# AliaksandrSiarohin/wc-gan

Hardware: AMD Instinct MI355X
Metric: images/sec G+D step, CIFAR-10 ResNet-SN+WC, batch 64 (higher is better)
Workload: dtype f32; 1 GPU; CIFAR-10 ResNet SN uncond + WC (scripts/cifar10_resnet_sn_uncond.sh), batch 64/GPU, training_ratio 5, generator_batch_multiple 2; parallelism=dp1, wc_statistics=per-replica, launch=hipgraph

## Files before the change

include/wc_hip.h:

```cpp
#ifndef WC_HIP_H
#define WC_HIP_H

#include <stddef.h>
#include <stdint.h>

#ifdef __cplusplus
extern "C" {
#endif

#define WC_ABI_VERSION 8

#define WC_OK                 0
#define WC_ERR_NULL          -1
#define WC_ERR_SHAPE         -2
#define WC_ERR_CHANNELS      -3
#define WC_ERR_WORKSPACE     -4
#define WC_ERR_ARG           -5

typedef void* wc_stream_t;

int         wc_abi_version(void);
const char* wc_error_string(int code);

#define WC_CORE_API "wc_stats_f32 wc_factor_f64 wc_color_f32 wc_group_bias_f32 wc_apply_f32 wc_apply_act_f32 " \
// ... 245 lines not shown
                             float* colsum_partials, int C, wc_stream_t stream);

#define WC_CONV_HIST_FLOATS (4 * 512 + 16)
#define WC_CONV_HIST_REDO (4 * 512)
int wc_conv_split_hist_f32(const float* x, int64_t n, int relu, void* hi, void* lo, float* scale, float* colsum_partials , int C,
                           float* hist, int bootstrap, wc_stream_t stream);

int wc_conv_split_leaky_f32(const float* x, int64_t n, float negative_slope, void* hi, void* lo, float* scale, void* amax_scratch,
                            float* colsum_partials , int C, wc_stream_t stream);
int wc_conv_split_hist_leaky_f32(const float* x, int64_t n, float negative_slope, void* hi, void* lo, float* scale,
                                 float* colsum_partials , int C, float* hist, int bootstrap, wc_stream_t stream);
int wc_conv_leaky_bwd_f32(float* dx, const float* x, int64_t n, float negative_slope, wc_stream_t stream);

size_t wc_conv_weights_bytes(const wc_conv_geom* g);
int wc_conv_weights_f32(const float* w, int64_t stride_k, int64_t stride_n, int64_t stride_r, int64_t stride_s,
                        int64_t n_elems, const wc_conv_geom* g, void* image, float* scale, void* amax_scratch,
                        const float* known_amax, int known_count, wc_stream_t stream);

int wc_conv_weights_pair_f32(const float* w, int64_t stride_r, int64_t stride_s, int64_t n_elems,
                             int64_t a_stride_k, int64_t a_stride_n, const wc_conv_geom* ga, void* image_a,
                             int64_t b_stride_k, int64_t b_stride_n, const wc_conv_geom* gb, void* image_b,
                             float* scale, void* amax_scratch, const float* known_amax, int known_count,
                             wc_stream_t stream);

typedef struct {
    const float* w; int64_t stride_k, stride_n, stride_r, stride_s, n_elems;
    const wc_conv_geom* g; void* image; float* scale;
    const float* amax; int amax_count; int pair_of;
} wc_conv_weights_job;
int wc_conv_weights_batch_f32(const wc_conv_weights_job* jobs, int count, wc_stream_t stream);
int wc_conv_weights_batch_launches(const wc_conv_weights_job* jobs, int count);

#define WC_CONV_ABSMAX_FLOATS 512
typedef struct { const float* x; int64_t n; float* partial; } wc_conv_absmax_job;
int wc_conv_absmax_batch_f32(const wc_conv_absmax_job* jobs, int count, wc_stream_t stream);

size_t wc_conv_workspace_bytes(const wc_conv_geom* g);
int wc_conv_f16x3(const void* xhi, const void* xlo, const float* xscale, const void* wimage, const float* wscale,
                  const float* bias, const void* zero_line, const wc_conv_geom* g, int relu, float* y,
                  void* ws, size_t ws_bytes, wc_stream_t stream);

int wc_conv_res_supported(const wc_conv_geom* g);
int wc_conv_res_f16x3(const void* xhi, const void* xlo, const float* xscale, const void* wimage, const float* wscale,
                      const float* bias, const float* res, const void* zero_line, const wc_conv_geom* g, float* y,
                      void* ws, size_t ws_bytes, wc_stream_t stream);
int wc_conv_block_dx_f32(const float* dx1, const float* x, const float* other, int64_t N, int64_t H, int64_t W, int C, int down,
                         float* out, wc_stream_t stream);

size_t wc_conv_wrw_workspace_bytes(const wc_conv_geom* g);
int wc_conv_wrw_f16x3(const void* xhi, const void* xlo, const float* xscale, const void* ghi, const void* glo,
                      const float* gscale, const void* zero_line, const wc_conv_geom* g, float* dw, int64_t stride_k,
                      int64_t stride_n, int64_t stride_r, int64_t stride_s, void* ws, size_t ws_bytes,
                      wc_stream_t stream);

int    wc_conv_wrw_narrow_supported(int64_t N, int64_t H, int64_t W, int Cin, int Cout, int ksize);
size_t wc_conv_wrw_narrow_workspace_bytes(int64_t N, int64_t H, int64_t W, int Cin, int Cout, int ksize);
int    wc_conv_wrw_narrow_f32(const float* x, const float* gy, int64_t N, int64_t H, int64_t W, int Cin, int Cout, int ksize,
                              float* dw, int64_t stride_k, int64_t stride_n, int64_t stride_r, int64_t stride_s, float* db ,
                              void* ws, size_t ws_bytes, wc_stream_t stream);

int    wc_conv_narrow64_supported(int64_t N, int64_t H, int64_t W, int Cin, int Cout, int ksize);
size_t wc_conv_wrw_narrow64_workspace_bytes(int64_t N, int64_t H, int64_t W, int Cin, int Cout, int ksize);
int    wc_conv_wrw_narrow64_f32(const float* x, const float* gy, int64_t N, int64_t H, int64_t W, int Cin, int Cout, int ksize,
                                float* dw, int64_t stride_k, int64_t stride_n, int64_t stride_r, int64_t stride_s, float* db ,
                                void* ws, size_t ws_bytes, wc_stream_t stream);

int    wc_conv_fwd_narrow_f32(const float* x, const float* w, int64_t stride_k, int64_t stride_n, int64_t stride_r, int64_t stride_s,
                              const float* bias , int64_t N, int64_t H, int64_t W, int Cin, int Cout, int ksize, int relu,
                              float* y, wc_stream_t stream);

int wc_conv_wrw_bias_f16x3(const void* xhi, const void* xlo, const float* xscale, const void* ghi, const void* glo,
                           const float* gscale, const void* zero_line, const wc_conv_geom* g, float* dw, int64_t stride_k,
                           int64_t stride_n, int64_t stride_r, int64_t stride_s, const float* colsum_partials, float* db,
                           void* ws, size_t ws_bytes, wc_stream_t stream);

int    wc_conv_bwd_pair_supported(const wc_conv_geom* gd, const wc_conv_geom* gf);
size_t wc_conv_bwd_pair_workspace_bytes(const wc_conv_geom* gd, const wc_conv_geom* gf);
int    wc_conv_bwd_pair_f16x3(const void* ghi, const void* glo, const float* gscale, const void* wimage, const float* wscale,
                              const void* zero_line, const wc_conv_geom* gd, float* dx, void* ws_dx, size_t ws_dx_bytes,
                              const void* xhi, const void* xlo, const float* xscale, const wc_conv_geom* gf, float* dw,
                              int64_t stride_k, int64_t stride_n, int64_t stride_r, int64_t stride_s,
                              const float* colsum_partials, float* db, void* ws_dw, size_t ws_dw_bytes, wc_stream_t stream);

int wc_stream_copy_f32(const float* src, float* dst, int64_t n, wc_stream_t stream);


size_t wc_std_stats_workspace_bytes(int64_t M, int C, int groups);
int    wc_std_stats_f32(const float* x, int64_t M, int C, int groups, double* sum , double* sqsum ,
                        void* ws, size_t ws_bytes, wc_stream_t stream);

int    wc_std_factor_f64(const double* sum, const double* sqsum, int64_t M, int C, int groups, double eps, double momentum, int ddof,
                         int training, float* moving_mean , float* moving_variance ,
                         const float* gamma , const float* beta , int Kc,
                         float* mu , float* w , float* a , float* b ,
                         wc_stream_t stream);

int    wc_std_apply_f32(const float* x, const float* a, const float* b, const int32_t* slot , int64_t N, int64_t HW,
                        int C, int Kt, int relu, float* y, wc_stream_t stream);

size_t wc_std_bwd_reduce_workspace_bytes(int64_t N, int64_t HW, int C, int Kc);
int    wc_std_bwd_reduce_f32(const float* x, const float* gy, const float* a, const float* b, const int32_t* slot, int64_t N, int64_t HW,
                             int C, int Kc, int relu, double* gsum , double* gxsum ,
                             void* ws, size_t ws_bytes, wc_stream_t stream);

int    wc_std_bwd_factor_f64(const double* gsum, const double* gxsum, const float* mu , const float* w ,
                             const float* gamma , int64_t M, int C, int Kc, int training,
                             float* dgamma , float* dbeta , float* q , float* r , wc_stream_t stream);

int    wc_std_bwd_apply_f32(const float* x, const float* gy, const float* a, const float* b, const float* q, const float* r,
                            const int32_t* slot, int64_t N, int64_t HW, int C, int Kc, int relu, float* dx, wc_stream_t stream);


int    wc_zca_supported(int C);
size_t wc_zca_workspace_bytes(int C, int groups);
size_t wc_zca_status_offset(int C, int groups);
int    wc_zca_f64(const double* L , int C, int groups, double eps,
                  double* U , double* lam , double* W ,
                  void* ws, size_t ws_bytes, wc_stream_t stream);

size_t wc_bwd_factor_zca_workspace_bytes(int C, int Kc);
int    wc_bwd_factor_zca_f64(const double* R, const double* gsum, const double* W, const double* U, const double* lam,
                             const float* gamma, const float* A, int Kc, int C, int64_t M,
                             double eps, int ddof, int training,
                             float* dgamma , float* dbeta ,
                             float* S , float* gmean ,
                             void* ws, size_t ws_bytes, wc_stream_t stream);


int    wc_renorm_supported(int C);
size_t wc_renorm_workspace_bytes(int C);
int    wc_renorm_f64(const float* moving_cov , const double* L , int C, double eps,
                     double* Wm , double* C0 ,
                     void* ws, size_t ws_bytes, wc_stream_t stream);

size_t wc_bwd_factor_renorm_workspace_bytes(int C, int Kc);
int    wc_bwd_factor_renorm_f64(const double* R, const double* gsum, const double* W, const double* Wm, const double* C0,
                                const float* gamma, const float* A, int Kc, int C, int64_t M,
                                double eps, int ddof, int training,
                                float* dgamma , float* dbeta ,
                                float* S , float* gmean ,
                                void* ws, size_t ws_bytes, wc_stream_t stream);


int wc_conv_split_masked_f32(const float* t, const float* a, int64_t n, float slope, void* hi, void* lo, float* scale, void* amax_scratch,
                             float* colsum_partials , int C, wc_stream_t stream);
int wc_conv_split_hist_masked_f32(const float* t, const float* a, int64_t n, float slope, void* hi, void* lo, float* scale,
                                  float* colsum_partials , int C, float* hist, int bootstrap, wc_stream_t stream);

int wc_gp_interp_f32(const float* real, const float* fake, const float* eps, int64_t N, int64_t L, float* x_hat, wc_stream_t stream);

size_t wc_gp_rows_workspace_bytes(int64_t N);
int wc_gp_rows_f32(const float* g, int64_t N, int64_t L, double lambda, double inv_n, float* norms , float* v ,
                   float* penalty , void* ws, size_t ws_bytes, wc_stream_t stream);


int wc_adam_tick(int64_t* counter, float* record , double lr, double beta1, double beta2, int kind, double total, double drop_at,
                 wc_stream_t stream);

#define WC_ADAM_CAPACITY 96
typedef struct {
    float*       param[WC_ADAM_CAPACITY];
    const float* grad[WC_ADAM_CAPACITY];
    int64_t      moment_off[WC_ADAM_CAPACITY];
    int32_t      numel[WC_ADAM_CAPACITY];
    int32_t      chunk_start[WC_ADAM_CAPACITY + 1];
    int32_t      count, chunk;
// ... 31 lines not shown
```

wc_gan_amd/_lib.py:

```python
from __future__ import annotations

import ctypes
import os
from ctypes import c_float, c_char_p, c_double, c_int, c_int64, c_size_t, c_void_p

_HERE = os.path.dirname(os.path.abspath(__file__))
LIB_PATH = os.path.join(_HERE, "libwc_hip.so")

WC_OK = 0
ABI_VERSION = 8
ERRORS = {-1: "WC_ERR_NULL", -2: "WC_ERR_SHAPE", -3: "WC_ERR_CHANNELS", -4: "WC_ERR_WORKSPACE", -5: "WC_ERR_ARG"}

SIGNATURES = {
    "wc_abi_version": (c_int, []),
    "wc_error_string": (c_char_p, [c_int]),
    "wc_stats_workspace_bytes": (c_size_t, [c_int64, c_int, c_int]),
    "wc_factor_workspace_bytes": (c_size_t, [c_int, c_int]),
    "wc_color_workspace_bytes": (c_size_t, [c_int, c_int]),
    "wc_bwd_reduce_workspace_bytes": (c_size_t, [c_int64, c_int64, c_int, c_int, c_int]),
    "wc_bwd_factor_workspace_bytes": (c_size_t, [c_int, c_int]),
    "wc_apply_workspace_bytes": (c_size_t, [c_int64, c_int64, c_int, c_int]),
    "wc_apply_plan_bytes": (c_size_t, [c_int, c_int]),
    "wc_bwd_apply_workspace_bytes": (c_size_t, [c_int64, c_int64, c_int, c_int]),
    "wc_stats_f32": (c_int, [c_void_p, c_int64, c_int, c_int, c_void_p, c_void_p, c_void_p, c_size_t, c_void_p]),
# ... 56 lines not shown
    "wc_apply_split_ex_f16x2": (c_int, [c_void_p, c_void_p, c_void_p, c_void_p, c_void_p, c_void_p, c_void_p, c_int64, c_int64,
                                        c_int, c_int, c_int, c_void_p, c_void_p, c_void_p, c_void_p, c_void_p, c_void_p, c_size_t, c_void_p]),
    "wc_whiten_split_workspace_bytes": (c_size_t, [c_int64, c_int, c_int]),
    "wc_whiten_split_error_offset": (c_size_t, [c_int64, c_int, c_int]),
    "wc_whiten_split_f16x2": (c_int, [c_void_p, c_void_p, c_void_p, c_int64, c_int, c_int, c_double, c_double, c_int, c_void_p, c_void_p,
                                      c_void_p, c_void_p, c_void_p, c_void_p, c_size_t, c_void_p]),
    "wc_resadd_split_supported": (c_int, [c_int64, c_int64, c_int64, c_int]),
    "wc_resadd_f32": (c_int, [c_void_p, c_void_p, c_int64, c_int64, c_int64, c_int, c_int, c_void_p, c_void_p]),
    "wc_resadd_stats_supported": (c_int, [c_int64, c_int64, c_int64, c_int, c_int, c_int]),
    "wc_resadd_stats_workspace_bytes": (c_size_t, [c_int64, c_int64, c_int64, c_int, c_int]),
    "wc_resadd_stats_split_f32": (c_int, [c_void_p, c_void_p, c_int64, c_int64, c_int64, c_int, c_int, c_int, c_void_p, c_void_p, c_void_p, c_void_p,
                                          c_void_p, c_void_p, c_size_t, c_void_p]),
    "wc_whiten_presummed_error_offset": (c_size_t, [c_int64, c_int, c_int]),
    "wc_whiten_presummed_f16x2": (c_int, [c_void_p, c_int64, c_int, c_int, c_double, c_double, c_int, c_void_p, c_void_p, c_void_p, c_void_p,
                                          c_void_p, c_void_p, c_size_t, c_void_p]),
    "wc_stats_presummed_f16x2": (c_int, [c_void_p, c_int64, c_int, c_int, c_void_p, c_void_p, c_void_p, c_size_t, c_void_p]),
    "wc_resadd_split_f32": (c_int, [c_void_p, c_void_p, c_int64, c_int64, c_int64, c_int, c_int, c_void_p, c_void_p, c_void_p, c_void_p,
                                    c_void_p, c_void_p]),
    "wc_patch_sum_f32": (c_int, [c_void_p, c_int64, c_int64, c_int64, c_int, c_void_p, c_void_p]),
    "wc_fold_channel_scale_f32": (c_int, [c_void_p, c_int64, c_int64, c_int, c_int, c_void_p, c_void_p, c_void_p, c_void_p, c_void_p, c_void_p]),
    "wc_unfold_channel_scale_f32": (c_int, [c_void_p, c_void_p, c_int64, c_int64, c_int, c_int, c_void_p, c_void_p, c_void_p, c_void_p]),
    "wc_color_split_f32": (c_int, [c_void_p, c_void_p, c_int, c_int, c_void_p, c_void_p, c_void_p, c_void_p, c_void_p, c_void_p, c_void_p,
                                   c_void_p, c_void_p, c_size_t, c_void_p]),
    "wc_factor_mix_supported": (c_int, [c_int, c_int]),
    "wc_factor_mix_f32": (c_int, [c_void_p, c_void_p, c_void_p, c_void_p, c_int, c_int, c_int, c_int, c_void_p, c_void_p]),
    "wc_factor_mix_bwd_workspace_bytes": (c_size_t, [c_int, c_int]),
    "wc_factor_mix_bwd_f32": (c_int, [c_void_p, c_void_p, c_void_p, c_void_p, c_int, c_int, c_int, c_int, c_void_p, c_void_p, c_void_p,
                                      c_void_p, c_size_t, c_void_p]),
    "wc_group_bias_centered_f32": (c_int, [c_void_p, c_void_p, c_void_p, c_void_p, c_int, c_int, c_int, c_int, c_void_p, c_void_p]),
    "wc_bwd_xsplit_supported": (c_int, [c_int64, c_int64, c_int, c_int]),
    "wc_bwd_reduce_xsplit_f32": (c_int, [c_void_p, c_void_p, c_void_p, c_void_p, c_void_p, c_void_p, c_void_p, c_int64, c_int64, c_int, c_int,
                                         c_void_p, c_void_p, c_void_p, c_void_p, c_size_t, c_void_p]),
    "wc_bwd_apply_xsplit_workspace_bytes": (c_size_t, [c_int, c_int]),
    "wc_bwd_apply_xsplit_f32": (c_int, [c_void_p, c_void_p, c_void_p, c_void_p, c_void_p, c_void_p, c_void_p, c_void_p, c_void_p, c_void_p,
                                        c_int64, c_int64, c_int, c_int, c_void_p, c_void_p, c_void_p, c_size_t, c_void_p]),
    "wc_stream_copy_f32": (c_int, [c_void_p, c_void_p, c_int64, c_void_p]),
    "wc_spectral_norm_workspace_bytes": (c_size_t, [c_int, c_int]),
    "wc_spectral_norm_batched_f32": (c_int, [c_void_p, c_int, c_int, c_float, c_void_p]),
    "wc_spectral_norm_bwd_batched_f32": (c_int, [c_void_p, c_int, c_int, c_void_p]),
    "wc_spectral_norm_f32": (c_int, [c_void_p, c_int, c_int, c_void_p, c_void_p, c_int, c_float, c_void_p, c_void_p,
                                     c_void_p, c_void_p, c_void_p, c_size_t, c_void_p]),
    "wc_spectral_norm_bwd_f32": (c_int, [c_void_p, c_void_p, c_void_p, c_void_p, c_void_p, c_int, c_int, c_int, c_void_p,
                                         c_void_p, c_size_t, c_void_p]),
    "wc_conv_supported": (c_int, [c_void_p]),
    "wc_conv_split_f32": (c_int, [c_void_p, c_int64, c_int, c_void_p, c_void_p, c_void_p, c_void_p, c_void_p]),
    "wc_conv_weights_bytes": (c_size_t, [c_void_p]),
    "wc_conv_weights_f32": (c_int, [c_void_p, c_int64, c_int64, c_int64, c_int64, c_int64, c_void_p, c_void_p, c_void_p,
                                    c_void_p, c_void_p, c_int, c_void_p]),
    "wc_spectral_norm_amax_offset": (c_size_t, [c_int, c_int]),
    "wc_spectral_norm_error_offset": (c_size_t, [c_int, c_int]),
    "wc_conv_split_hist_f32": (c_int, [c_void_p, c_int64, c_int, c_void_p, c_void_p, c_void_p, c_void_p, c_int, c_void_p, c_int, c_void_p]),
    "wc_conv_split_leaky_f32": (c_int, [c_void_p, c_int64, c_float, c_void_p, c_void_p, c_void_p, c_void_p, c_void_p, c_int, c_void_p]),
    "wc_conv_split_hist_leaky_f32": (c_int, [c_void_p, c_int64, c_float, c_void_p, c_void_p, c_void_p, c_void_p, c_int, c_void_p, c_int, c_void_p]),
    "wc_conv_leaky_bwd_f32": (c_int, [c_void_p, c_void_p, c_int64, c_float, c_void_p]),
    "wc_conv_narrow64_supported": (c_int, [c_int64, c_int64, c_int64, c_int, c_int, c_int]),
    "wc_conv_wrw_narrow64_workspace_bytes": (c_size_t, [c_int64, c_int64, c_int64, c_int, c_int, c_int]),
    "wc_conv_wrw_narrow64_f32": (c_int, [c_void_p, c_void_p, c_int64, c_int64, c_int64, c_int, c_int, c_int, c_void_p, c_int64, c_int64, c_int64,
                                         c_int64, c_void_p, c_void_p, c_size_t, c_void_p]),
    "wc_conv_fwd_narrow_f32": (c_int, [c_void_p, c_void_p, c_int64, c_int64, c_int64, c_int64, c_void_p, c_int64, c_int64, c_int64, c_int, c_int, c_int,
                                       c_int, c_void_p, c_void_p]),
    "wc_conv_wrw_narrow_supported": (c_int, [c_int64, c_int64, c_int64, c_int, c_int, c_int]),
    "wc_conv_wrw_narrow_workspace_bytes": (c_size_t, [c_int64, c_int64, c_int64, c_int, c_int, c_int]),
    "wc_conv_wrw_narrow_f32": (c_int, [c_void_p, c_void_p, c_int64, c_int64, c_int64, c_int, c_int, c_int, c_void_p, c_int64, c_int64, c_int64,
                                       c_int64, c_void_p, c_void_p, c_size_t, c_void_p]),
    "wc_conv_split_colsum_f32": (c_int, [c_void_p, c_int64, c_int, c_void_p, c_void_p, c_void_p, c_void_p, c_void_p, c_int, c_void_p]),
    "wc_conv_wrw_bias_f16x3": (c_int, [c_void_p, c_void_p, c_void_p, c_void_p, c_void_p, c_void_p, c_void_p, c_void_p, c_void_p,
                                       c_int64, c_int64, c_int64, c_int64, c_void_p, c_void_p, c_void_p, c_size_t, c_void_p]),
    "wc_conv_weights_pair_f32": (c_int, [c_void_p, c_int64, c_int64, c_int64, c_int64, c_int64, c_void_p, c_void_p,
                                         c_int64, c_int64, c_void_p, c_void_p, c_void_p, c_void_p, c_void_p, c_int, c_void_p]),
    "wc_conv_weights_batch_f32": (c_int, [c_void_p, c_int, c_void_p]),
    "wc_conv_weights_batch_launches": (c_int, [c_void_p, c_int]),
    "wc_conv_absmax_batch_f32": (c_int, [c_void_p, c_int, c_void_p]),
    "wc_conv_wrw_workspace_bytes": (c_size_t, [c_void_p]),
    "wc_conv_wrw_f16x3": (c_int, [c_void_p, c_void_p, c_void_p, c_void_p, c_void_p, c_void_p, c_void_p, c_void_p, c_void_p,
                                  c_int64, c_int64, c_int64, c_int64, c_void_p, c_size_t, c_void_p]),
    "wc_conv_workspace_bytes": (c_size_t, [c_void_p]),
    "wc_conv_f16x3": (c_int, [c_void_p, c_void_p, c_void_p, c_void_p, c_void_p, c_void_p, c_void_p, c_void_p, c_int,
                              c_void_p, c_void_p, c_size_t, c_void_p]),
    "wc_conv_bwd_pair_supported": (c_int, [c_void_p, c_void_p]),
    "wc_conv_bwd_pair_workspace_bytes": (c_size_t, [c_void_p, c_void_p]),
    "wc_conv_bwd_pair_f16x3": (c_int, [c_void_p, c_void_p, c_void_p, c_void_p, c_void_p, c_void_p, c_void_p, c_void_p, c_void_p, c_size_t,
                                       c_void_p, c_void_p, c_void_p, c_void_p, c_void_p, c_int64, c_int64, c_int64, c_int64,
                                       c_void_p, c_void_p, c_void_p, c_size_t, c_void_p]),
    "wc_std_stats_workspace_bytes": (c_size_t, [c_int64, c_int, c_int]),
    "wc_std_stats_f32": (c_int, [c_void_p, c_int64, c_int, c_int, c_void_p, c_void_p, c_void_p, c_size_t, c_void_p]),
    "wc_std_factor_f64": (c_int, [c_void_p, c_void_p, c_int64, c_int, c_int, c_double, c_double, c_int, c_int, c_void_p, c_void_p,
                                  c_void_p, c_void_p, c_int, c_void_p, c_void_p, c_void_p, c_void_p, c_void_p]),
    "wc_std_apply_f32": (c_int, [c_void_p, c_void_p, c_void_p, c_void_p, c_int64, c_int64, c_int, c_int, c_int, c_void_p, c_void_p]),
    "wc_std_bwd_reduce_workspace_bytes": (c_size_t, [c_int64, c_int64, c_int, c_int]),
    "wc_std_bwd_reduce_f32": (c_int, [c_void_p, c_void_p, c_void_p, c_void_p, c_void_p, c_int64, c_int64, c_int, c_int, c_int,
                                      c_void_p, c_void_p, c_void_p, c_size_t, c_void_p]),
    "wc_std_bwd_factor_f64": (c_int, [c_void_p, c_void_p, c_void_p, c_void_p, c_void_p, c_int64, c_int, c_int, c_int,
                                      c_void_p, c_void_p, c_void_p, c_void_p, c_void_p]),
    "wc_std_bwd_apply_f32": (c_int, [c_void_p, c_void_p, c_void_p, c_void_p, c_void_p, c_void_p, c_void_p, c_int64, c_int64, c_int, c_int,
                                     c_int, c_void_p, c_void_p]),
    "wc_zca_supported": (c_int, [c_int]),
    "wc_zca_workspace_bytes": (c_size_t, [c_int, c_int]),
    "wc_zca_status_offset": (c_size_t, [c_int, c_int]),
    "wc_zca_f64": (c_int, [c_void_p, c_int, c_int, c_double, c_void_p, c_void_p, c_void_p, c_void_p, c_size_t, c_void_p]),
    "wc_bwd_factor_zca_workspace_bytes": (c_size_t, [c_int, c_int]),
    "wc_bwd_factor_zca_f64": (c_int, [c_void_p, c_void_p, c_void_p, c_void_p, c_void_p, c_void_p, c_void_p, c_int, c_int, c_int64,
                                      c_double, c_int, c_int, c_void_p, c_void_p, c_void_p, c_void_p,
                                      c_void_p, c_size_t, c_void_p]),
    "wc_renorm_supported": (c_int, [c_int]),
    "wc_renorm_workspace_bytes": (c_size_t, [c_int]),
    "wc_renorm_f64": (c_int, [c_void_p, c_void_p, c_int, c_double, c_void_p, c_void_p, c_void_p, c_size_t, c_void_p]),
    "wc_bwd_factor_renorm_workspace_bytes": (c_size_t, [c_int, c_int]),
    "wc_bwd_factor_renorm_f64": (c_int, [c_void_p, c_void_p, c_void_p, c_void_p, c_void_p, c_void_p, c_void_p, c_int, c_int, c_int64,
                                         c_double, c_int, c_int, c_void_p, c_void_p, c_void_p, c_void_p,
                                         c_void_p, c_size_t, c_void_p]),
    "wc_conv_split_masked_f32": (c_int, [c_void_p, c_void_p, c_int64, c_float, c_void_p, c_void_p, c_void_p, c_void_p, c_void_p, c_int, c_void_p]),
    "wc_conv_split_hist_masked_f32": (c_int, [c_void_p, c_void_p, c_int64, c_float, c_void_p, c_void_p, c_void_p, c_void_p, c_int, c_void_p, c_int,
                                              c_void_p]),
    "wc_conv_res_supported": (c_int, [c_void_p]),
    "wc_conv_res_f16x3": (c_int, [c_void_p, c_void_p, c_void_p, c_void_p, c_void_p, c_void_p, c_void_p, c_void_p, c_void_p,
                                  c_void_p, c_void_p, c_size_t, c_void_p]),
    "wc_conv_block_dx_f32": (c_int, [c_void_p, c_void_p, c_void_p, c_int64, c_int64, c_int64, c_int, c_int, c_void_p, c_void_p]),
    "wc_gp_interp_f32": (c_int, [c_void_p, c_void_p, c_void_p, c_int64, c_int64, c_void_p, c_void_p]),
    "wc_gp_rows_workspace_bytes": (c_size_t, [c_int64]),
    "wc_gp_rows_f32": (c_int, [c_void_p, c_int64, c_int64, c_double, c_double, c_void_p, c_void_p, c_void_p, c_void_p, c_size_t, c_void_p]),
    "wc_adam_capacity": (c_int, []),
    "wc_adam_tick": (c_int, [c_void_p, c_void_p, c_double, c_double, c_double, c_int, c_double, c_double, c_void_p]),
    "wc_adam_update_f32": (c_int, [c_void_p, c_void_p, c_void_p, c_int64, c_void_p, c_double, c_double, c_float, c_void_p]),
    "wc_critic_tail_supported": (c_int, [c_int64, c_int64, c_int, c_int]),
    "wc_critic_tail_fwd_f32": (c_int, [c_void_p, c_void_p, c_void_p, c_void_p, c_void_p, c_void_p, c_int64, c_int64, c_int, c_int, c_int,
                                       c_void_p, c_void_p, c_void_p, c_void_p, c_void_p, c_void_p]),
    "wc_critic_tail_bwd_f32": (c_int, [c_void_p, c_void_p, c_void_p, c_void_p, c_void_p, c_void_p, c_void_p, c_void_p, c_void_p,
                                       c_int64, c_int64, c_int, c_int, c_int, c_void_p, c_void_p, c_void_p]),
    "wc_critic_tail_wgrad_f32": (c_int, [c_void_p, c_void_p, c_void_p, c_int64, c_int, c_int, c_void_p, c_void_p, c_void_p, c_void_p, c_void_p]),
    "wc_critic_proj_supported": (c_int, [c_int64, c_int64, c_int, c_int]),
    "wc_critic_proj_fwd_f32": (c_int, [c_void_p, c_void_p, c_void_p, c_void_p, c_void_p, c_int64, c_int64, c_int, c_int, c_int,
                                       c_void_p, c_void_p, c_void_p]),
    "wc_critic_proj_bwd_f32": (c_int, [c_void_p, c_void_p, c_void_p, c_void_p, c_void_p, c_int64, c_int64, c_int, c_int, c_int, c_void_p, c_void_p]),
    "wc_critic_proj_wgrad_f32": (c_int, [c_void_p, c_void_p, c_void_p, c_int64, c_int, c_int, c_void_p, c_void_p, c_void_p, c_void_p]),
}

ADAM_CAPACITY = 96


class AdamTable(ctypes.Structure):
    _fields_ = [("param", c_void_p * ADAM_CAPACITY), ("grad", c_void_p * ADAM_CAPACITY), ("moment_off", c_int64 * ADAM_CAPACITY),
                ("numel", ctypes.c_int32 * ADAM_CAPACITY), ("chunk_start", ctypes.c_int32 * (ADAM_CAPACITY + 1)),
                ("count", ctypes.c_int32), ("chunk", ctypes.c_int32)]


class SnItem(ctypes.Structure):
    _fields_ = [("W", c_void_p), ("u", c_void_p), ("v", c_void_p), ("w_sn", c_void_p), ("sigma", c_void_p),
                ("u_used", c_void_p), ("v_used", c_void_p), ("ws", c_void_p), ("rows", c_int), ("cols", c_int)]


class SnBwdItem(ctypes.Structure):
    _fields_ = [("g", c_void_p), ("w_sn", c_void_p), ("u", c_void_p), ("v", c_void_p), ("sigma", c_void_p),
                ("dW", c_void_p), ("ws", c_void_p), ("rows", c_int), ("cols", c_int)]


class ConvGeom(ctypes.Structure):
    _fields_ = [("N", c_int), ("H", c_int), ("W", c_int), ("Hin", c_int), ("Win", c_int), ("Cin", c_int),
                ("Hout", c_int), ("Wout", c_int), ("Cout", c_int), ("in_stride", c_int), ("out_stride", c_int),
                ("ntaps", c_int), ("nphase", c_int),
                ("dy", (ctypes.c_byte * 16) * 4), ("dx", (ctypes.c_byte * 16) * 4),
                ("off_y", ctypes.c_byte * 4), ("off_x", ctypes.c_byte * 4),
                ("nsrc", (ctypes.c_byte * 16) * 4),
                ("wr", ((ctypes.c_byte * 4) * 16) * 4), ("ws", ((ctypes.c_byte * 4) * 16) * 4),
                ("wcoef", c_float)]


class ConvWeightsJob(ctypes.Structure):
    _fields_ = [("w", c_void_p), ("stride_k", c_int64), ("stride_n", c_int64), ("stride_r", c_int64), ("stride_s", c_int64),
                ("n_elems", c_int64), ("g", c_void_p), ("image", c_void_p), ("scale", c_void_p), ("amax", c_void_p),
                ("amax_count", c_int), ("pair_of", c_int)]


class ConvAbsmaxJob(ctypes.Structure):
    _fields_ = [("x", c_void_p), ("n", c_int64), ("partial", c_void_p)]


ABSMAX_FLOATS = 512

_lib = None


class WcHipError(RuntimeError):
    pass


def shared_gpu_guard(device_count=None) -> bool:
    if "WC_K2_TWO_LAUNCH" in os.environ:
        if os.environ["WC_K2_TWO_LAUNCH"] == "0":
            del os.environ["WC_K2_TWO_LAUNCH"]
        return False
    try:
        ranks = int(os.environ.get("LOCAL_WORLD_SIZE", "1") or 1)
    except ValueError:
        ranks = 1
    if ranks <= 1:
        return False
    if any(os.environ.get(k) for k in ("HIP_VISIBLE_DEVICES", "CUDA_VISIBLE_DEVICES", "ROCR_VISIBLE_DEVICES")):
        return False
    if device_count is None:
        try:
            import torch
            device_count = torch.cuda.device_count()
        except Exception:
            device_count = 0
    if device_count and ranks > device_count:
        os.environ["WC_K2_TWO_LAUNCH"] = "1"
        return True
    return False


def load() -> ctypes.CDLL:
    global _lib
    if _lib is not None:
        return _lib
    import torch
    shared_gpu_guard()
    if not os.path.exists(LIB_PATH):
        raise WcHipError(
            f"{LIB_PATH} is missing: build it with `python -m wc_gan_amd.build` "
            "(or __graft_entry__.build()); the WC path has no non-HIP fallback")
    lib = ctypes.CDLL(LIB_PATH)
    for name, (res, args) in SIGNATURES.items():
        fn = getattr(lib, name)
        fn.restype = res
        fn.argtypes = args
    if lib.wc_abi_version() != ABI_VERSION:
        raise WcHipError(f"libwc_hip.so ABI version {lib.wc_abi_version()} != {ABI_VERSION}: rebuild it "
                         "(python -m wc_gan_amd.build)")
    _lib = lib
    return lib


def check(code: int, what: str) -> None:
    if code == WC_OK:
        return
    lib = load()
    msg = lib.wc_error_string(code)
    raise WcHipError(f"{what} failed: {ERRORS.get(code, code)} ({msg.decode() if msg else '?'})")
```

wc_gan_amd/build.py:

```python
from __future__ import annotations

import os
import subprocess
import sys
from concurrent.futures import ThreadPoolExecutor

HERE = os.path.dirname(os.path.abspath(__file__))
CSRC = os.path.join(HERE, "csrc")
LIB = os.path.join(HERE, "libwc_hip.so")
SOURCES = ["wc_rows.hip", "wc_fast.hip", "wc_split.hip", "wc_split_xty.hip", "wc_resadd.hip", "wc_fast_xty.hip", "wc_small.hip", "wc_zca.hip", "wc_renorm.hip", "wc_mix.hip", "wc_std.hip", "wc_sn.hip", "wc_conv.hip", "wc_gp.hip", "wc_adam.hip", "wc_tail.hip", "wc_abi.hip"]
HEADERS = ["wc_common.h", os.path.join("..", "..", "include", "wc_hip.h")]
FLAGS = ["--offload-arch=gfx950", "-O3", "-std=c++17", "-fPIC", "-ffp-contract=fast", "-Wall", "-Wno-unused-function"] + \
    os.environ.get("WC_EXTRA_FLAGS", "").split()


def _hipcc() -> str:
    for cand in (os.environ.get("HIPCC"), "/opt/rocm/bin/hipcc", "hipcc"):
        if cand and (os.path.isabs(cand) and os.path.exists(cand) or not os.path.isabs(cand)):
            return cand
    raise RuntimeError("hipcc not found")


def _stale(target: str, deps: list[str]) -> bool:
    if not os.path.exists(target):
        return True
    t = os.path.getmtime(target)
    return any(os.path.getmtime(d) > t for d in deps if os.path.exists(d))


def build(force: bool = False, verbose: bool = True) -> str:
    hipcc = _hipcc()
    objdir = os.path.join(CSRC, "build")
    os.makedirs(objdir, exist_ok=True)
    hdrs = [os.path.join(CSRC, h) for h in HEADERS]
    srcs = [s for s in SOURCES if os.path.exists(os.path.join(CSRC, s))]
    jobs = []
    for s in srcs:
        src = os.path.join(CSRC, s)
        obj = os.path.join(objdir, s.replace(".hip", ".o"))
        if force or _stale(obj, [src] + hdrs):
            jobs.append((src, obj))

    def compile_one(job):
        src, obj = job
        cmd = [hipcc] + FLAGS + ["-c", src, "-o", obj]
        if verbose:
            print(" ".join(cmd), flush=True)
        r = subprocess.run(cmd, capture_output=True, text=True)
        if r.returncode != 0:
            raise RuntimeError(f"hipcc failed for {src}:\n{r.stdout}\n{r.stderr}")
        if verbose and r.stderr.strip():
            print(r.stderr, file=sys.stderr)

    with ThreadPoolExecutor(max_workers=4) as ex:
        list(ex.map(compile_one, jobs))
    objs = [os.path.join(objdir, s.replace(".hip", ".o")) for s in srcs]
    if force or jobs or _stale(LIB, objs):
        cmd = [hipcc, "--offload-arch=gfx950", "-shared", "-fPIC", "-o", LIB] + objs
        if verbose:
            print(" ".join(cmd), flush=True)
        r = subprocess.run(cmd, capture_output=True, text=True)
        if r.returncode != 0:
            raise RuntimeError(f"link failed:\n{r.stdout}\n{r.stderr}")
    return LIB


if __name__ == "__main__":
    print(build(force="--force" in sys.argv))
```

wc_gan_amd/conv.py:

```python
from __future__ import annotations

import ctypes
import os

import torch
import torch.nn.functional as F

from . import _lib, _state
from .ops import _ptr, _stream

_zero_lines = {}


def _zero_line(device):
    z = _zero_lines.get(device)
    if z is None:
        z = _zero_lines[device] = torch.zeros(64, dtype=torch.uint8, device=device)
    return z


def _plain(r, s):
    return [(r, s)], 1.0


def _pooled3(r, s):
    return [(r - a, s - b) for a in (0, 1) for b in (0, 1) if 0 <= r - a <= 2 and 0 <= s - b <= 2], 0.25


_UP_ROWS = ((2,), (1, 2), (0, 1), (0,))


def _upsampled3(r, s):
    return [(r3, s3) for r3 in _UP_ROWS[r] for s3 in _UP_ROWS[s]], 1.0


def _set_sources(g, p, t, r, s, source):
    taps, coef = source(r, s)
    g.nsrc[p][t] = len(taps)
    for m, (r3, s3) in enumerate(taps):
        g.wr[p][t][m], g.ws[p][t][m] = r3, s3
    g.wcoef = coef


def _dense_geom(N, Hin, Win, Cin, Cout, k, stride, source=_plain):
    pad = k // 2 if stride == 1 else 1
    g = _lib.ConvGeom()
    g.N, g.Hin, g.Win, g.Cin, g.Cout = N, Hin, Win, Cin, Cout
    g.H, g.W = Hin // stride, Win // stride
    g.Hout, g.Wout = g.H, g.W
    g.in_stride, g.out_stride, g.ntaps, g.nphase = stride, 1, k * k, 1
    for r in range(k):
        for s in range(k):
            t = r * k + s
            g.dy[0][t], g.dx[0][t] = r - pad, s - pad
            _set_sources(g, 0, t, r, s, source)
    return g


def _phase_geom(N, Hin, Win, Cin, Cout, source=_plain):
    g = _lib.ConvGeom()
    g.N, g.Hin, g.Win, g.Cin, g.Cout = N, Hin, Win, Cin, Cout
    g.H, g.W, g.Hout, g.Wout = Hin, Win, 2 * Hin, 2 * Win
    g.in_stride, g.out_stride, g.ntaps, g.nphase = 1, 2, 4, 4
    for py in range(2):
        for px in range(2):
            p = py * 2 + px
            g.off_y[p], g.off_x[p] = py, px
            t = 0
            for dy in ((-1, 0) if py == 0 else (0, 1)):
                for dx in ((-1, 0) if px == 0 else (0, 1)):
                    g.dy[p][t], g.dx[p][t] = dy, dx
                    _set_sources(g, p, t, py + 1 - 2 * dy, px + 1 - 2 * dx, source)
                    t += 1
    return g


def _supported(g):
    return bool(_lib.load().wc_conv_supported(ctypes.addressof(g)))


def supported(x, w, kind):
    handed = getattr(x, '_wc_planes', None) is not None
    if not (x.is_cuda and x.dtype == torch.float32 and x.dim() == 4 and (handed or x.is_contiguous()) and w.dtype == torch.float32):
        return False
    p = _plan(kind, x, w)
    return bool(p) and p.ok


class _Plan:
    __slots__ = ('ok', 'fwd', 'bwd', 'fwd_ws', 'bwd_ws', 'wrw_ws', 'fwd_ptr', 'bwd_ptr', 'pair', 'res')

    def __init__(self, kind, N, H, W, wshape):
        class _W:
            shape = wshape
        lib = _lib.load()
        (gf, kf, nf), (gb, kb, nb) = _geoms(kind, N, H, W, _W)
        self.fwd, self.bwd = (gf, kf, nf), (gb, kb, nb)
        self.fwd_ptr, self.bwd_ptr = ctypes.addressof(gf), ctypes.addressof(gb)
        self.ok = bool(lib.wc_conv_supported(self.fwd_ptr)) and bool(lib.wc_conv_supported(self.bwd_ptr))
        self.fwd_ws = lib.wc_conv_workspace_bytes(self.fwd_ptr) if self.ok else 0
        self.bwd_ws = lib.wc_conv_workspace_bytes(self.bwd_ptr) if self.ok else 0
        self.wrw_ws = lib.wc_conv_wrw_workspace_bytes(self.fwd_ptr) if self.ok else 0
        self.pair = self.ok and bool(lib.wc_conv_bwd_pair_supported(self.bwd_ptr, self.fwd_ptr))
        self.res = self.ok and bool(lib.wc_conv_res_supported(self.fwd_ptr))


_plans = {}


def _plan(kind, x, w):
    key = (kind, tuple(x.shape), tuple(w.shape))
    p = _plans.get(key)
    if p is None:
        N, H, W, C = x.shape
        good = (kind == 'same' and w.shape[1] == C and w.shape[2] == w.shape[3] and w.shape[2] in (1, 3)) or \
               (kind == 'down' and w.shape[1] == C and tuple(w.shape[2:]) == (4, 4) and H % 2 == 0 and W % 2 == 0) or \
               (kind == 'down3' and w.shape[1] == C and tuple(w.shape[2:]) == (3, 3) and H % 2 == 0 and W % 2 == 0) or \
               (kind == 'up3' and w.shape[1] == C and tuple(w.shape[2:]) == (3, 3)) or \
               (kind == 'up' and w.shape[0] == C and tuple(w.shape[2:]) == (4, 4))
        if kind not in ('same', 'down', 'up', 'down3', 'up3'):
            raise ValueError(kind)
        if good and kind != 'down' and (C % 128 or w.shape[0] % 128 or w.shape[1] % 128):
            good = False
        p = _plans[key] = _Plan(kind, N, H, W, tuple(w.shape)) if good else False
    return p


def _colsum_ok(C):
    return C % 4 == 0 and 256 % (C // 4) == 0


SPLIT_HIST = os.environ.get('WC_SPLIT_HIST', '1') != '0'
HIST_FLOATS = 4 * 512 + 16
HIST_REDO = 4 * 512


_REDO_MODE = os.environ.get('WC_SPLIT_HIST_REDO', '1')


def _guarded(role):
    return _REDO_MODE == '2' or (_REDO_MODE != '0' and role in ('g', 't', 'd'))


def _site_hist(site, role, device):
    if not getattr(site, 'training', True):
        return None
    book = site.__dict__.setdefault('_wc_split_hist', {})
    h = book.get(role)
    if h is not None and h[0].device != device:
        h = None
    if h is None:
        if torch.cuda.is_current_stream_capturing():
            return None
        h = book[role] = [torch.zeros(HIST_FLOATS, dtype=torch.float32, device=device), False]
    return h


def split_planes(x, relu=False, colsum=False, site=None, role='x', leaky=None):
    lib = _lib.load()
    if leaky is not None:
        if relu:
            raise ValueError("relu and leaky are two activations")
        return _split_planes_leaky(lib, x, float(leaky), colsum, site, role)
    both = torch.empty((2,) + tuple(x.shape), dtype=torch.float16, device=x.device)
    hi, lo = both[0], both[1]
    scale = torch.empty(1 + 512, dtype=torch.float32, device=x.device)
    h = _site_hist(site, role, x.device) if (SPLIT_HIST and site is not None) else None
    if h is not None:
        C = x.shape[-1]
        part = torch.empty((512, C), dtype=torch.float32, device=x.device) if colsum else None
        _lib.check(lib.wc_conv_split_hist_f32(_ptr(x), x.numel(), 1 if relu else 0, _ptr(hi), _ptr(lo), _ptr(scale), _ptr(part), C if colsum else 0,
                                              _ptr(h[0]), (0 if h[1] else 1) | (0 if _guarded(role) else 2), _stream()), "wc_conv_split_hist_f32")
        h[1] = True
        return (hi, lo, scale, part) if colsum else (hi, lo, scale)
    if not colsum:
        _lib.check(lib.wc_conv_split_f32(_ptr(x), x.numel(), 1 if relu else 0, _ptr(hi), _ptr(lo), _ptr(scale),
                                         scale.data_ptr() + 4, _stream()), "wc_conv_split_f32")
        return hi, lo, scale
    C = x.shape[-1]
    part = torch.empty((512, C), dtype=torch.float32, device=x.device)
    _lib.check(lib.wc_conv_split_colsum_f32(_ptr(x), x.numel(), 1 if relu else 0, _ptr(hi), _ptr(lo), _ptr(scale),
                                            scale.data_ptr() + 4, _ptr(part), C, _stream()), "wc_conv_split_colsum_f32")
    return hi, lo, scale, part


def _split_planes_leaky(lib, x, slope, colsum, site, role):
    both = torch.empty((2,) + tuple(x.shape), dtype=torch.float16, device=x.device)
# ... 220 lines not shown
                del recs[i]
                return images
    if _recording is not None:
        _recording[2].append((site, tuple(geoms)))
    elif _prepared is not None:
        _prepared[2] = True
    return None


def finish_images(root):
    global _recording, _prepared
    if _recording is not None and _recording[0] is root:
        root._wc_image_logs[_recording[1]] = _recording[2]
    elif _prepared is not None and _prepared[0] is root:
        if _prepared[2] or any(site.__dict__.get('_wc_images') for site in root.__dict__.get('_wc_image_sites', ())):
            root._wc_image_logs.pop(_prepared[1], None)
    _recording = _prepared = None
    _clear_images(root)


def run(planes, image, geom, bias=None, relu=False, nbytes=None, res=None):
    hi, lo, xs = planes
    img, ws = image
    lib = _lib.load()
    y = torch.empty((geom.N, geom.Hout, geom.Wout, geom.Cout), dtype=torch.float32, device=hi.device)
    if nbytes is None:
        nbytes = lib.wc_conv_workspace_bytes(ctypes.addressof(geom))
    work = torch.empty(nbytes, dtype=torch.uint8, device=hi.device) if nbytes else None
    if res is not None:
        if relu or not (res.is_contiguous() and res.shape == y.shape and res.dtype == torch.float32 and res.device == y.device):
            raise ValueError("run: the residual is a dense fp32 tensor of the output's shape (and there is no ReLU behind it)")
        _lib.check(lib.wc_conv_res_f16x3(_ptr(hi), _ptr(lo), _ptr(xs), _ptr(img), _ptr(ws), _ptr(bias) if bias is not None else None,
                                         _ptr(res), _ptr(_zero_line(hi.device)), ctypes.addressof(geom), _ptr(y),
                                         _ptr(work), nbytes, _stream()), "wc_conv_res_f16x3")
        return y
    _lib.check(lib.wc_conv_f16x3(_ptr(hi), _ptr(lo), _ptr(xs), _ptr(img), _ptr(ws), _ptr(bias) if bias is not None else None,
                                 _ptr(_zero_line(hi.device)), ctypes.addressof(geom), 1 if relu else 0, _ptr(y),
                                 _ptr(work), nbytes, _stream()), "wc_conv_f16x3")
    return y


def _geoms(kind, N, H, W, w):
    if kind == 'same':
        co, ci, k = w.shape[0], w.shape[1], w.shape[2]
        fwd = _dense_geom(N, H, W, ci, co, k, 1)
        bwd = _dense_geom(N, H, W, co, ci, k, 1)
        for t in range(k * k):
            bwd.dy[0][t], bwd.dx[0][t] = -bwd.dy[0][t], -bwd.dx[0][t]
        return (fwd, 1, 0), (bwd, 0, 1)
    if kind in ('down', 'down3'):
        co, ci = w.shape[0], w.shape[1]
        src = _pooled3 if kind == 'down3' else _plain
        return (_dense_geom(N, H, W, ci, co, 4, 2, src), 1, 0), (_phase_geom(N, H // 2, W // 2, co, ci, src), 0, 1)
    if kind == 'up3':
        co, ci = w.shape[0], w.shape[1]
        return (_phase_geom(N, H, W, ci, co, _upsampled3), 1, 0), (_dense_geom(N, 2 * H, 2 * W, co, ci, 4, 2, _upsampled3), 0, 1)
    ci, co = w.shape[0], w.shape[1]
    return (_phase_geom(N, H, W, ci, co), 0, 1), (_dense_geom(N, 2 * H, 2 * W, co, ci, 4, 2), 1, 0)


def weight_gradient(x_planes, g_planes, geom, w, k_axis, n_axis, nbytes=None, colsum=None):
    lib = _lib.load()
    xh, xl, xs = x_planes
    gh, gl, gs = g_planes[:3]
    dw = torch.empty_like(w)
    if dw.stride() != w.stride():
        raise ValueError("weight must be dense")
    if nbytes is None:
        nbytes = lib.wc_conv_wrw_workspace_bytes(ctypes.addressof(geom))
    ws = torch.empty(nbytes, dtype=torch.uint8, device=w.device)
    if colsum is not None:
        db = torch.empty(geom.Cout, dtype=torch.float32, device=w.device)
        _lib.check(lib.wc_conv_wrw_bias_f16x3(_ptr(xh), _ptr(xl), _ptr(xs), _ptr(gh), _ptr(gl), _ptr(gs), _ptr(_zero_line(w.device)),
                                              ctypes.addressof(geom), _ptr(dw), w.stride(k_axis), w.stride(n_axis), w.stride(2),
                                              w.stride(3), _ptr(colsum), _ptr(db), _ptr(ws), nbytes, _stream()),
                   "wc_conv_wrw_bias_f16x3")
        return dw, db
    _lib.check(lib.wc_conv_wrw_f16x3(_ptr(xh), _ptr(xl), _ptr(xs), _ptr(gh), _ptr(gl), _ptr(gs), _ptr(_zero_line(w.device)),
                                     ctypes.addressof(geom), _ptr(dw), w.stride(k_axis), w.stride(n_axis), w.stride(2),
                                     w.stride(3), _ptr(ws), nbytes, _stream()), "wc_conv_wrw_f16x3")
    return dw


def backward_pair(g_planes, image, x_planes, plan, w, colsum=None):
    lib = _lib.load()
    gh, gl, gs = g_planes[:3]
    xh, xl, xs = x_planes
    img, ws = image
    gf, kf, nf = plan.fwd
    gb = plan.bwd[0]
    dx = torch.empty((gb.N, gb.Hout, gb.Wout, gb.Cout), dtype=torch.float32, device=gh.device)
    dw = torch.empty_like(w)
    if dw.stride() != w.stride():
        raise ValueError("weight must be dense")
    work_dx = torch.empty(plan.bwd_ws, dtype=torch.uint8, device=gh.device) if plan.bwd_ws else None
    work_dw = torch.empty(plan.wrw_ws, dtype=torch.uint8, device=gh.device)
    db = torch.empty(gf.Cout, dtype=torch.float32, device=w.device) if colsum is not None else None
    zero = _zero_line(gh.device)
    _lib.check(lib.wc_conv_bwd_pair_f16x3(_ptr(gh), _ptr(gl), _ptr(gs), _ptr(img), _ptr(ws), _ptr(zero), plan.bwd_ptr, _ptr(dx),
                                          _ptr(work_dx), plan.bwd_ws,
                                          _ptr(xh), _ptr(xl), _ptr(xs), plan.fwd_ptr, _ptr(dw), w.stride(kf), w.stride(nf), w.stride(2),
                                          w.stride(3), _ptr(colsum), _ptr(db), _ptr(work_dw), plan.wrw_ws, _stream()),
               "wc_conv_bwd_pair_f16x3")
    return dx, dw, db


def takes_planes(shape, wshape, kind):
    class _S:
        pass
    xs, ws = _S(), _S()
    xs.shape, ws.shape = tuple(shape), tuple(wshape)
    p = _plan(kind, xs, ws)
    return bool(p) and p.ok


class _FastConv(torch.autograd.Function):
    @staticmethod
    def forward(ctx, x, w, bias, kind, plan, relu_input=False, handed=None, site=None, leaky=None, residual=None):
        gf, kf, nf = plan.fwd
        planes = handed if handed is not None else split_planes(x, relu=relu_input, site=site, role='x', leaky=leaky)
        ctx.site, ctx.leaky = site, leaky
        if ctx.needs_input_grad[0]:
            img, ctx.bwd_image = weight_image_pair(w, plan.fwd, plan.bwd, site=site)
        else:
            img, ctx.bwd_image = weight_image(w, gf, kf, nf, site=site), None
        if residual is not None and plan.res and FUSED_RESIDUAL:
            y = run(planes, img, gf, bias, nbytes=plan.fwd_ws, res=residual.contiguous())
        else:
            y = run(planes, img, gf, bias, nbytes=plan.fwd_ws)
            if residual is not None:
                y = y + residual
        ctx.save_for_backward(w, *planes, *((x,) if (relu_input or leaky is not None) else ()))
        ctx.kind, ctx.has_bias, ctx.plan, ctx.relu_input = kind, bias is not None, plan, relu_input
        return y

    @staticmethod
    def backward(ctx, gy):
        w, xh, xl, xs = ctx.saved_tensors[:4]
        kind, plan = ctx.kind, ctx.plan
        gy = gy.contiguous()
        want_db = ctx.has_bias and ctx.needs_input_grad[2]
        fused_db = want_db and ctx.needs_input_grad[1] and _colsum_ok(gy.shape[-1])
        g_planes = split_planes(gy, colsum=fused_db, site=ctx.site, role='g')
        dx = dw = db = None
        paired = ctx.needs_input_grad[0] and ctx.needs_input_grad[1] and ctx.bwd_image is not None and plan.pair
        if paired:
            dx, dw, pdb = backward_pair(g_planes, ctx.bwd_image, (xh, xl, xs), plan, w, colsum=g_planes[3] if fused_db else None)
            if fused_db:
                db = pdb
        if ctx.needs_input_grad[0]:
            if not paired:
                gb, kb, nb = plan.bwd
                image = ctx.bwd_image if ctx.bwd_image is not None else weight_image(w, gb, kb, nb)
                dx = run(g_planes[:3], image, gb, nbytes=plan.bwd_ws)
            if ctx.relu_input:
                dx = torch.ops.aten.threshold_backward(dx, ctx.saved_tensors[4], 0)
            elif ctx.leaky is not None:
                dx = leaky_backward_(dx, ctx.saved_tensors[4], ctx.leaky)
        if ctx.needs_input_grad[1] and not paired:
            gf, kf, nf = plan.fwd
            if fused_db:
                dw, db = weight_gradient((xh, xl, xs), g_planes, gf, w, kf, nf, nbytes=plan.wrw_ws, colsum=g_planes[3])
            else:
                dw = weight_gradient((xh, xl, xs), g_planes, gf, w, kf, nf, nbytes=plan.wrw_ws)
        if want_db and not fused_db:
            db = gy.sum((0, 1, 2))
        need = ctx.needs_input_grad
        return dx, dw, db, None, None, None, None, None, None, (gy if len(need) > 9 and need[9] else None)


_ones = {}


def _one(device):
    t = _ones.get(device)
    if t is None:
        t = torch.ones(1, dtype=torch.float32, device=device)
        if not torch.cuda.is_current_stream_capturing():
            _ones[device] = t
    return t

# ... 158 lines not shown

def narrow_in_conv(x, w, bias=None):
    if _storage_extent(w) != w.numel():
        w = w.contiguous()
    return _NarrowInConv.apply(x, w, bias)


def narrow_out_weight_gradient(x, gy, w):
    lib = _lib.load()
    N, H, W, C = x.shape
    O, k = w.shape[0], w.shape[2]
    dw = torch.empty_strided(w.shape, w.stride(), dtype=torch.float32, device=w.device)
    if _storage_extent(dw) != dw.numel():
        raise ValueError("weight must be dense")
    nb = lib.wc_conv_wrw_narrow_workspace_bytes(N, H, W, O, C, k)
    ws = torch.empty(nb, dtype=torch.uint8, device=x.device)
    last = dw.data_ptr() + 4 * ((k - 1) * dw.stride(2) + (k - 1) * dw.stride(3))
    _lib.check(lib.wc_conv_wrw_narrow_f32(_ptr(gy), _ptr(x), N, H, W, O, C, k, ctypes.c_void_p(last), dw.stride(0), dw.stride(1), -dw.stride(2),
                                          -dw.stride(3), None, _ptr(ws), nb, _stream()), "wc_conv_wrw_narrow_f32")
    return dw


def narrow_out_wrw_supported(x, w):
    if not (NARROW_WRW and x.is_cuda and x.dtype == torch.float32 and w.dtype == torch.float32 and x.dim() == 4 and w.dim() == 4):
        return False
    k = w.shape[2]
    if w.shape[3] != k or k not in (1, 3) or w.shape[1] != x.shape[3]:
        return False
    N, H, W, C = x.shape
    return bool(_lib.load().wc_conv_wrw_narrow_supported(N, H, W, w.shape[0], C, k))


def fast_conv(x, w, bias=None, kind='same', residual=None):
    if not supported(x, w, kind):
        raise _lib.WcHipError(f"fast_conv: unsupported call {tuple(x.shape)} x {tuple(w.shape)} ({kind})")
    if residual is None:
        return _FastConv.apply(x, w, bias, kind, _plan(kind, x, w))
    return _FastConv.apply(x, w, bias, kind, _plan(kind, x, w), False, None, None, None, residual)


FUSED_BLOCK = True
FUSED_MASKED_SPLIT = True
FUSED_RESIDUAL = True
FUSED_BLOCK_DX = True


class _Shape:
    def __init__(self, shape):
        self.shape = tuple(shape)


def critic_block_plans(xshape, w1shape, w2shape, wsshape, down):
    if len(xshape) != 4 or len(w1shape) != 4 or len(w2shape) != 4:
        return None
    N, H, W, C = xshape
    F1, F2 = w1shape[0], w2shape[0]
    if tuple(w1shape[1:]) != (C, 3, 3) or tuple(w2shape[1:]) != (F1, 3, 3):
        return None
    if down and (H % 2 or W % 2):
        return None
    if wsshape is None:
        if down or F2 != C:
            return None
    elif tuple(wsshape) != (F2, C, 1, 1):
        return None
    if not (_colsum_ok(F1) and _colsum_ok(F2)):
        return None
    out = (N, H // 2, W // 2) if down else (N, H, W)
    p1 = _plan('same', _Shape(xshape), _Shape(w1shape))
    p2 = _plan('down3' if down else 'same', _Shape((N, H, W, F1)), _Shape(w2shape))
    ps = _plan('same', _Shape(out + (C,)), _Shape(wsshape)) if wsshape is not None else None
    if not (p1 and p1.ok and p2 and p2.ok and (wsshape is None or (ps and ps.ok))):
        return None
    return p1, p2, ps


def _images(w, plan, both, site=None):
    if both:
        return weight_image_pair(w, plan.fwd, plan.bwd, site=site)
    gf, kf, nf = plan.fwd
    return weight_image(w, gf, kf, nf, site=site), None


def _layer_gradients(g_planes, fused_db, x_planes, w, plan, bwd_image, need_dx, need_dw):
    cs = g_planes[3] if fused_db else None
    if need_dx and need_dw and bwd_image is not None and plan.pair:
        return backward_pair(g_planes, bwd_image, x_planes, plan, w, colsum=cs)
    dx = dw = db = None
    if need_dx:
        gb, kb, nb = plan.bwd
        image = bwd_image if bwd_image is not None else weight_image(w, gb, kb, nb)
        dx = run(g_planes[:3], image, gb, nbytes=plan.bwd_ws)
    if need_dw:
        gf, kf, nf = plan.fwd
        if fused_db:
            dw, db = weight_gradient(x_planes, g_planes, gf, w, kf, nf, nbytes=plan.wrw_ws, colsum=cs)
        else:
            dw = weight_gradient(x_planes, g_planes, gf, w, kf, nf, nbytes=plan.wrw_ws)
    return dx, dw, db


def _pool2(x):
    return F.avg_pool2d(x.permute(0, 3, 1, 2), 2).permute(0, 2, 3, 1).contiguous()


class _CriticBlock(torch.autograd.Function):
    @staticmethod
    def forward(ctx, x, w1, b1, w2, b2, ws, bs, sites, plans, down):
        conv1, conv2, shortcut = sites
        p1, p2, ps = plans
        need = ctx.needs_input_grad
        need_h = need[0] or need[1] or need[2]
        x_pl = split_planes(x, relu=True, site=conv1, role='x')
        img1, bimg1 = _images(w1, p1, need[0], conv1)
        h = run(x_pl, img1, p1.fwd[0], b1, nbytes=p1.fwd_ws)
        h_pl = split_planes(h, relu=True, site=conv2, role='x')
        img2, bimg2 = _images(w2, p2, need_h, conv2)
        s, s_pl, bimgs = x, (), None
        if ws is not None:
            s_pl = split_planes(_pool2(x) if down else x, site=shortcut, role='x')
            imgs, bimgs = _images(ws, ps, need[0], shortcut)
            s = run(s_pl, imgs, ps.fwd[0], bs, nbytes=ps.fwd_ws)
        if p2.res and FUSED_RESIDUAL:
            y = run(h_pl, img2, p2.fwd[0], b2, nbytes=p2.fwd_ws, res=s)
        else:
            y = run(h_pl, img2, p2.fwd[0], b2, nbytes=p2.fwd_ws) + s
        ctx.save_for_backward(x, h, w1, w2, *x_pl, *h_pl, *s_pl, *((ws,) if ws is not None else ()))
        ctx.sites, ctx.plans, ctx.down = sites, plans, down
        ctx.images = (bimg1, bimg2, bimgs)
        ctx.has_bias = (b1 is not None, b2 is not None, bs is not None)
        ctx.mark_non_differentiable(h)
        ctx.set_materialize_grads(False)
        return y, h

    @staticmethod
    def backward(ctx, g, _gh):
        saved = ctx.saved_tensors
        x, h, w1, w2 = saved[:4]
        x_pl, h_pl = saved[4:7], saved[7:10]
        conv1, conv2, shortcut = ctx.sites
        p1, p2, ps = ctx.plans
        bimg1, bimg2, bimgs = ctx.images
        need = ctx.needs_input_grad
        need_h = need[0] or need[1] or need[2]
        if g is None:
            return (None,) * 10
        g = g.contiguous()
        dx = dw1 = db1 = dw2 = db2 = dws = dbs = dx1 = None

        def bias_rides(has, need_b, need_w, C):
            return has and need_b and need_w and _colsum_ok(C)

        fused2 = bias_rides(ctx.has_bias[1], need[4], need[3], g.shape[-1])
        g2 = split_planes(g, colsum=fused2, site=conv2, role='g')
        dh, dw2, db2 = _layer_gradients(g2, fused2, h_pl, w2, p2, bimg2, need_h, need[3])
        if ctx.has_bias[1] and need[4] and not fused2:
            db2 = g.sum((0, 1, 2))
        if need_h:
            fused1 = bias_rides(ctx.has_bias[0], need[2], need[1], h.shape[-1])
            if FUSED_MASKED_SPLIT:
                g1 = split_planes_masked(dh, h, site=conv1, role='g', colsum=fused1)
            else:
                g1 = split_planes(torch.ops.aten.threshold_backward(dh, h, 0), colsum=fused1, site=conv1, role='g')
            dx1, dw1, db1 = _layer_gradients(g1, fused1, x_pl, w1, p1, bimg1, need[0], need[1])
            if ctx.has_bias[0] and need[2] and not fused1:
                db1 = torch.ops.aten.threshold_backward(dh, h, 0).sum((0, 1, 2))
        other = g
        if ps is not None:
            ws = saved[13]
            fuseds = bias_rides(ctx.has_bias[2], need[6], need[5], g.shape[-1])
            gs = split_planes(g, colsum=fuseds, site=shortcut, role='g')
            other, dws, dbs = _layer_gradients(gs, fuseds, saved[10:13], ws, ps, bimgs, need[0], need[5])
            if ctx.has_bias[2] and need[6] and not fuseds:
                dbs = g.sum((0, 1, 2))
        if need[0]:
            if FUSED_BLOCK_DX:
                dx = block_input_gradient(dx1, x, other, ctx.down)
            else:
                dx = torch.ops.aten.threshold_backward(dx1, x, 0)
                if ctx.down:
                    other = torch.ops.aten.avg_pool2d_backward(other.permute(0, 3, 1, 2), x.permute(0, 3, 1, 2), [2, 2], [2, 2], [0, 0],
                                                               False, True, None).permute(0, 2, 3, 1)
                dx = dx + other
        return dx, dw1, db1, dw2, db2, dws, dbs, None, None, None


def critic_block(x, w1, b1, w2, b2, ws, bs, sites, plans, down):
    return _CriticBlock.apply(x, w1, b1, w2, b2, ws, bs, sites, plans, down)
```

wc_gan_amd/csrc/wc_conv.hip:

```cpp
#include "wc_common.h"
#include "../../include/wc_hip.h"
#include <stdlib.h>
#include <string.h>


namespace {

constexpr int kMaxTaps = 16, kMaxPhase = 4;

struct ConvArgs {
    const _Float16* xhi; const _Float16* xlo;
    const _Float16* zero;
    const char* wimg;
    const float* xscale; const float* wscale;
    const float* bias;
    float* y;
    int N, H, W, Hin, Win, Cin, Cout, in_stride, ntaps, nphase, Hout, Wout, out_stride, relu;
    unsigned magHW, shHW, magW, shW;
    int ksplit; float* partial;
    signed char dy[kMaxPhase][kMaxTaps], dx[kMaxPhase][kMaxTaps];
    signed char offy[kMaxPhase], offx[kMaxPhase];
};

__device__ __forceinline__ void lds_dma16(const void* g, unsigned lds)
{
    unsigned keep;
    asm volatile("s_mov_b32 %0, m0\n\ts_mov_b32 m0, %2\n\ts_nop 0\n\tglobal_load_lds_dwordx4 %1, off\n\ts_mov_b32 m0, %0"
                 : "=&s"(keep) : "v"(g), "s"(lds) : "memory");
}

template <int MB, int NB, bool KS>
__device__ __forceinline__ void conv_f16x3_body(const ConvArgs& a, const unsigned bx, const unsigned by, const unsigned bz)
{
    extern __shared__ __attribute__((aligned(16))) char smem[];
    constexpr int TM = 64 * MB, TN = 64 * NB;
    constexpr int A_BYTES = 2 * MB * 4 * 1024, B_BYTES = 2 * NB * 4 * 1024, STAGE = A_BYTES + B_BYTES;
    constexpr int AQ = (2 * MB) / 4;
    static_assert(AQ >= 1, "MB >= 2");

    const int tid = threadIdx.x, lane = tid & 63;
    const int wave = __builtin_amdgcn_readfirstlane(tid >> 6);
    const int wm = wave >> 1, wn = wave & 1;
    const int ntn = a.Cout / TN;
    const int phase = by / ntn, nt = by - phase * ntn;
    const unsigned m0 = bx * TM;
    const unsigned HW = a.H * a.W;
    const int koff = (lane >> 5) * 8;

    int gy[AQ], gx[AQ];
    unsigned gpix[AQ];
    #pragma unroll
    for (int q = 0; q < AQ; ++q) {
        const unsigned m = m0 + (wave * AQ + q) * 32 + (lane & 31);
        const unsigned n = __umulhi(m, a.magHW) >> a.shHW, rem = m - n * HW;
        const unsigned yy = __umulhi(rem, a.magW) >> a.shW, xx = rem - yy * a.W;
        gy[q] = yy * a.in_stride; gx[q] = xx * a.in_stride; gpix[q] = n * (a.Hin * a.Win);
    }
    const unsigned lds0 = (unsigned)(size_t)((__attribute__((address_space(3))) char*)smem);
    const int nchunk = a.Cin >> 5;
    const int iters = a.ntaps * nchunk;
    const int nblk_all = a.Cout >> 5;

    auto issue = [&](int it, int stage) {
        const int tap = it / nchunk, ch = it - tap * nchunk;
        const int dy = a.dy[phase][tap], dx = a.dx[phase][tap];
        const unsigned sbase = __builtin_amdgcn_readfirstlane(lds0 + stage * STAGE);
        #pragma unroll
        for (int q = 0; q < AQ; ++q) {
            const int iy = gy[q] + dy, ix = gx[q] + dx;
            const bool ok = (unsigned)iy < (unsigned)a.Hin && (unsigned)ix < (unsigned)a.Win;
            const int64_t e = ((int64_t)(gpix[q] + iy * a.Win + ix)) * a.Cin + ch * 32 + koff;
            #pragma unroll
            for (int s = 0; s < 2; ++s) {
                const _Float16* ph = ok ? a.xhi + e + s * 16 : a.zero + koff;
                const _Float16* pl = ok ? a.xlo + e + s * 16 : a.zero + koff;
                const unsigned l = sbase + (((wave * AQ + q) * 2 + s) * 2) * 1024;
                lds_dma16(ph, l);
                lds_dma16(pl, l + 1024);
            }
        }
        const char* wsrc = a.wimg + ((((int64_t)(phase * a.ntaps + tap) * nchunk + ch) * nblk_all + nt * 2 * NB) << 12);
        #pragma unroll
        for (int c = 0; c < 2 * NB; ++c) {
// ... 49 lines not shown
        const char* sa = smem + stage * STAGE;
        const char* sb = sa + A_BYTES;
        #pragma unroll
        for (int i = 0; i < MB; ++i) {
            const char* p = sa + (((wm * MB + i) * 2 + ks) * 2) * 1024 + lane * 16;
            fa[ks][i][0] = *reinterpret_cast<const f16x8*>(p);
            fa[ks][i][1] = *reinterpret_cast<const f16x8*>(p + 1024);
        }
        #pragma unroll
        for (int j = 0; j < NB; ++j) {
            const char* p = sb + (((wn * NB + j) * 2 + ks) * 2) * 1024 + lane * 16;
            fb[ks][j][0] = *reinterpret_cast<const f16x8*>(p);
            fb[ks][j][1] = *reinterpret_cast<const f16x8*>(p + 1024);
        }
    };
    prep(it0, 0);
    #pragma unroll
    for (int d = 0; d < ND; ++d) dma(d);
    for (int it = it0; it < it1; ++it) {
        const int stage = (it - it0) & 1;
        __builtin_amdgcn_s_waitcnt(0x0F70);
        __syncthreads();
        frags(stage, 0);
        prep(it + 1 < it1 ? it + 1 : it, stage ^ 1);
        __builtin_amdgcn_sched_barrier(0);
        #pragma unroll
        for (int ks = 0; ks < 2; ++ks) {
            #pragma unroll
            for (int g = 0; g < PER; ++g) {
                const int prod = g / (MB * NB), i = (g / NB) % MB, j = g % NB;
                acc[i][j] = __builtin_amdgcn_mfma_f32_32x32x16_f16(fa[ks][i][prod == 0 ? 1 : 0], fb[ks][j][prod == 1 ? 1 : 0], acc[i][j], 0, 0, 0);
                if ((g + 1) % GAP == 0) {
                    dma(ks * HALF + g / GAP);
                    __builtin_amdgcn_sched_barrier(0);
                }
                if (ks == 0 && g == PER / 2) {
                    frags(stage, 1);
                    __builtin_amdgcn_sched_barrier(0);
                }
            }
        }
    }
    __builtin_amdgcn_s_waitcnt(0x0F70);
    const float inv = 1.0f / (a.xscale[0] * a.wscale[0]);
    const int oy0 = a.offy[phase], ox0 = a.offx[phase];
    float bj[NB];
    #pragma unroll
    for (int j = 0; j < NB; ++j) bj[j] = a.bias ? a.bias[nt * TN + (wn * NB + j) * 32 + (lane & 31)] : 0.f;
    #pragma unroll
    for (int i = 0; i < MB; ++i) {
        #pragma unroll
        for (int r = 0; r < 16; ++r) {
            const unsigned row = (r & 3) + 8 * (r >> 2) + 4 * (lane >> 5);
            const unsigned m = m0 + (wm * MB + i) * 32 + row;
            const unsigned n = __umulhi(m, a.magHW) >> a.shHW, rem = m - n * HW;
            const unsigned yy = __umulhi(rem, a.magW) >> a.shW, xx = rem - yy * a.W;
            const int64_t opix = ((int64_t)n * a.Hout + (yy * a.out_stride + oy0)) * a.Wout + (xx * a.out_stride + ox0);
            const int64_t oe = opix * a.Cout + nt * TN + wn * NB * 32 + (lane & 31);
            if (KS) {
                float* o = a.partial + (int64_t)bz * ((int64_t)a.N * a.Hout * a.Wout * a.Cout) + oe;
                #pragma unroll
                for (int j = 0; j < NB; ++j) o[j * 32] = acc[i][j][r];
            } else {
                float* o = a.y + oe;
                #pragma unroll
                for (int j = 0; j < NB; ++j) {
                    float v = acc[i][j][r] * inv + bj[j];
                    if (a.relu) v = fmaxf(v, 0.f);
                    o[j * 32] = v;
                }
            }
        }
    }
}

template <int MB, int NB, bool KS>
__global__ __launch_bounds__(256) void conv_f16x3_kernel(ConvArgs a) { conv_f16x3_body<MB, NB, KS>(a, blockIdx.x, blockIdx.y, blockIdx.z); }

struct KsplitReduceArgs {
    const float* partial; int ksplit; int64_t n4; int cout;
    const float* xscale; const float* wscale; const float* bias; int relu; float* y;
};

__device__ __forceinline__ void conv_ksplit_reduce_body(const float* __restrict__ partial, int ksplit, int64_t n4, int cout,
                                                        const float* __restrict__ xscale, const float* __restrict__ wscale,
                                                        const float* __restrict__ bias, int relu, float* __restrict__ y,
                                                        const unsigned bid, const unsigned nblocks, const float* __restrict__ res = nullptr)
{
    const float inv = 1.0f / (xscale[0] * wscale[0]);
    for (int64_t i = (int64_t)bid * 256 + threadIdx.x; i < n4; i += (int64_t)nblocks * 256) {
        f32x4 v = *reinterpret_cast<const f32x4*>(partial + 4 * i);
        int z = 1;
        for (; z + 3 < ksplit; z += 4) {
            f32x4 t[4];
            #pragma unroll
            for (int u = 0; u < 4; ++u) t[u] = *reinterpret_cast<const f32x4*>(partial + 4 * ((z + u) * n4 + i));
            #pragma unroll
            for (int u = 0; u < 4; ++u) v += t[u];
        }
        for (; z < ksplit; ++z) v += *reinterpret_cast<const f32x4*>(partial + 4 * (z * n4 + i));
        v = v * inv;
        if (bias) v += *reinterpret_cast<const f32x4*>(bias + (4 * i) % cout);
        if (relu) { v[0] = fmaxf(v[0], 0.f); v[1] = fmaxf(v[1], 0.f); v[2] = fmaxf(v[2], 0.f); v[3] = fmaxf(v[3], 0.f); }
        if (res) {
            const f32x4 r = *reinterpret_cast<const f32x4*>(res + 4 * i);
            #pragma unroll
            for (int j = 0; j < 4; ++j) v[j] = __fadd_rn(v[j], r[j]);
        }
        *reinterpret_cast<f32x4*>(y + 4 * i) = v;
    }
}

__global__ __launch_bounds__(256) void conv_ksplit_reduce_kernel(const float* __restrict__ partial, int ksplit, int64_t n4, int cout,
                                                                 const float* __restrict__ xscale, const float* __restrict__ wscale,
                                                                 const float* __restrict__ bias, int relu, float* __restrict__ y)
{
    conv_ksplit_reduce_body(partial, ksplit, n4, cout, xscale, wscale, bias, relu, y, blockIdx.x, gridDim.x);
}

__global__ __launch_bounds__(256) void conv_ksplit_reduce_res_kernel(const float* __restrict__ partial, int ksplit, int64_t n4, int cout,
                                                                     const float* __restrict__ xscale, const float* __restrict__ wscale,
                                                                     const float* __restrict__ bias, const float* __restrict__ res,
                                                                     float* __restrict__ y)
{
    conv_ksplit_reduce_body(partial, ksplit, n4, cout, xscale, wscale, bias, 0, y, blockIdx.x, gridDim.x, res);
}

__device__ __forceinline__ f32x4 split_act(f32x4 v, int relu, float slope)
{
    if (relu == 1) { v[0] = fmaxf(v[0], 0.f); v[1] = fmaxf(v[1], 0.f); v[2] = fmaxf(v[2], 0.f); v[3] = fmaxf(v[3], 0.f); }
    else if (relu == 2) {
        #pragma unroll
        for (int j = 0; j < 4; ++j) v[j] = v[j] > 0.f ? v[j] : slope * v[j];
    }
    return v;
}

constexpr int kAmaxBlocks = 512;

__global__ __launch_bounds__(256) void conv_absmax_kernel(const float* __restrict__ x, int64_t n4, int64_t n, float* __restrict__ partial,
                                                          float* __restrict__ colsum = nullptr, int c4n = 0, float leaky = -1.f)
{
    __shared__ float red[4];
    __shared__ f32x4 red4[256];
    float m = 0.f;
    f32x4 cs = {0.f, 0.f, 0.f, 0.f};
    for (int64_t i = blockIdx.x * 256 + threadIdx.x; i < n4; i += (int64_t)gridDim.x * 256) {
        const f32x4 v = *reinterpret_cast<const f32x4*>(x + 4 * i);
        const f32x4 u = leaky >= 0.f ? split_act(v, 2, leaky) : v;
        m = fmaxf(fmaxf(m, fabsf(u[0])), fmaxf(fabsf(u[1]), fmaxf(fabsf(u[2]), fabsf(u[3]))));
        cs += v;
    }
    if (blockIdx.x == 0 && threadIdx.x == 0) for (int64_t i = 4 * n4; i < n; ++i) m = fmaxf(m, fabsf(x[i]));
    #pragma unroll
    for (int o = 32; o > 0; o >>= 1) m = fmaxf(m, __shfl_xor(m, o));
    if ((threadIdx.x & 63) == 0) red[threadIdx.x >> 6] = m;
    if (colsum) red4[threadIdx.x] = cs;
    __syncthreads();
    if (threadIdx.x == 0) partial[blockIdx.x] = fmaxf(fmaxf(red[0], red[1]), fmaxf(red[2], red[3]));
    if (colsum && (int)threadIdx.x < c4n) {
        f32x4 t = red4[threadIdx.x];
        for (int p = threadIdx.x + c4n; p < 256; p += c4n) t += red4[p];
        *reinterpret_cast<f32x4*>(colsum + (int64_t)blockIdx.x * 4 * c4n + 4 * threadIdx.x) = t;
    }
}

__device__ __forceinline__ float scale_of(const float* __restrict__ partial, float mul = 1.0f, int count = kAmaxBlocks)
{
    float amax = 0.f;
    for (int i = threadIdx.x & 63; i < count; i += 64) amax = fmaxf(amax, partial[i]);
    #pragma unroll
    for (int o = 32; o > 0; o >>= 1) amax = fmaxf(amax, __shfl_xor(amax, o));
    amax *= mul;
    if (!(amax > 0.f) || !(amax < 3.0e38f)) return 1.0f;
    int e;
    (void)frexpf(amax, &e);
    return ldexpf(1.0f, 14 - e);
}

__global__ __launch_bounds__(256) void conv_leaky_bwd_kernel(float* __restrict__ dx, const float* __restrict__ x, int64_t n4, float slope)
{
    for (int64_t i = blockIdx.x * 256 + threadIdx.x; i < n4; i += (int64_t)gridDim.x * 256) {
        f32x4 g = *reinterpret_cast<const f32x4*>(dx + 4 * i);
        const f32x4 v = *reinterpret_cast<const f32x4*>(x + 4 * i);
        #pragma unroll
        for (int j = 0; j < 4; ++j) g[j] = v[j] > 0.f ? g[j] : slope * g[j];
        *reinterpret_cast<f32x4*>(dx + 4 * i) = g;
    }
}

template <bool DOWN>
__global__ __launch_bounds__(256) void conv_block_dx_kernel(const float* __restrict__ dx1, const float* __restrict__ x,
                                                            const float* __restrict__ other, int64_t n4, int c4, int W, int H,
                                                            float* __restrict__ out)
{
    for (int64_t i = (int64_t)blockIdx.x * 256 + threadIdx.x; i < n4; i += (int64_t)gridDim.x * 256) {
        const f32x4 d = *reinterpret_cast<const f32x4*>(dx1 + 4 * i);
        const f32x4 a = *reinterpret_cast<const f32x4*>(x + 4 * i);
        int64_t j = i;
        if (DOWN) {
            const int64_t pix = i / c4;
            const int c = (int)(i - pix * c4);
            const int64_t row = pix / W;
            const int xx = (int)(pix - row * W);
            const int64_t n = row / H;
            const int yy = (int)(row - n * H);
            j = ((n * (H >> 1) + (yy >> 1)) * (W >> 1) + (xx >> 1)) * c4 + c;
        }
        const f32x4 o = *reinterpret_cast<const f32x4*>(other + 4 * j);
        f32x4 r;
        #pragma unroll
        for (int k = 0; k < 4; ++k) {
            const float m = a[k] <= 0.f ? 0.f : d[k];
            r[k] = __fadd_rn(m, DOWN ? __fadd_rn(0.f, __fmul_rn(0.25f, o[k])) : o[k]);
        }
        *reinterpret_cast<f32x4*>(out + 4 * i) = r;
    }
}

__global__ __launch_bounds__(256) void conv_split_kernel(const float* __restrict__ x, int64_t n4, const float* __restrict__ amax,
                                                         int relu, _Float16* __restrict__ hi, _Float16* __restrict__ lo,
                                                         float* __restrict__ scale_out, float slope = 0.f)
{
    const float s = scale_of(amax);
    if (blockIdx.x == 0 && threadIdx.x == 0) scale_out[0] = s;
    for (int64_t i = blockIdx.x * 256 + threadIdx.x; i < n4; i += (int64_t)gridDim.x * 256) {
        f32x4 v = *reinterpret_cast<const f32x4*>(x + 4 * i);
        v = split_act(v, relu, slope);
        v = v * s;
        f16x4 h, l;
        #pragma unroll
        for (int j = 0; j < 4; ++j) { h[j] = (_Float16)v[j]; l[j] = (_Float16)(v[j] - (float)h[j]); }
        *reinterpret_cast<f16x4*>(hi + 4 * i) = h;
        *reinterpret_cast<f16x4*>(lo + 4 * i) = l;
    }
}

constexpr float kHistMargin = 64.0f;
constexpr int kHistArray = 2 * kAmaxBlocks;

__device__ __forceinline__ float scale_for(float amax)
{
    if (!(amax > 0.f) || !(amax < 3.0e38f)) return 1.0f;
    int e;
    (void)frexpf(amax, &e);
    return ldexpf(1.0f, 14 - e);
}

__global__ __launch_bounds__(kAmaxBlocks) void conv_hist_seed_kernel(float* __restrict__ hist)
{
    const float m = hist[threadIdx.x];
    __syncthreads();
    typedef float f32x2h __attribute__((ext_vector_type(2)));
    f32x2h a = {m, __builtin_bit_cast(float, 1u)}, b = {0.f, __builtin_bit_cast(float, 0u)};
    *reinterpret_cast<f32x2h*>(hist + 2 * threadIdx.x) = a;
    *reinterpret_cast<f32x2h*>(hist + kHistArray + 2 * threadIdx.x) = b;
    __shared__ float red[kAmaxBlocks / 64];
    float mm = m;
    #pragma unroll
    for (int o = 32; o > 0; o >>= 1) mm = fmaxf(mm, __shfl_xor(mm, o));
    if ((threadIdx.x & 63) == 0) red[threadIdx.x >> 6] = mm;
    __syncthreads();
    if (threadIdx.x == 0) {
        float t = 0.f;
        for (int i = 0; i < kAmaxBlocks / 64; ++i) t = fmaxf(t, red[i]);
        hist[2 * kHistArray + 2] = t; hist[2 * kHistArray + 3] = t;
    }
}

__global__ __launch_bounds__(256) void conv_split_hist_kernel(const float* __restrict__ x, int64_t n4, int relu, _Float16* __restrict__ hi,
                                                              _Float16* __restrict__ lo, float* __restrict__ scale_out,
                                                              float* __restrict__ hist, float* __restrict__ colsum, int c4n,
                                                              float slope = 0.f)
{
    __shared__ float red[4];
    __shared__ f32x4 red4[256];
    typedef float f32x2h __attribute__((ext_vector_type(2)));
    typedef int i32x2h __attribute__((ext_vector_type(2)));
    float mx[2] = {0.f, 0.f};
    int tlo[2] = {0x7fffffff, 0x7fffffff}, thi[2] = {0, 0};
    #pragma unroll
    for (int arr = 0; arr < 2; ++arr)
        #pragma unroll
        for (int i = 0; i < kAmaxBlocks / 64; ++i) {
            const i32x2h p = *reinterpret_cast<const i32x2h*>(hist + arr * kHistArray + 2 * ((threadIdx.x & 63) + 64 * i));
            mx[arr] = fmaxf(mx[arr], __builtin_bit_cast(float, p[0]));
            tlo[arr] = min(tlo[arr], p[1]);
            thi[arr] = max(thi[arr], p[1]);
        }
    #pragma unroll
    for (int o = 32; o > 0; o >>= 1)
        #pragma unroll
        for (int arr = 0; arr < 2; ++arr) {
            mx[arr] = fmaxf(mx[arr], __shfl_xor(mx[arr], o));
            tlo[arr] = min(tlo[arr], __shfl_xor(tlo[arr], o));
            thi[arr] = max(thi[arr], __shfl_xor(thi[arr], o));
        }
    const bool ok0 = tlo[0] == thi[0], ok1 = tlo[1] == thi[1];
    const int src = (ok1 && (!ok0 || thi[1] > thi[0])) ? 1 : 0;
    const int tag = (src ? thi[1] : thi[0]) + 1;
    const float prev = src ? mx[1] : mx[0];
    const float assumed = prev > 0.f ? prev : hist[2 * kHistArray + 2 + src];
    const float s = scale_for(assumed * kHistMargin);
    if (blockIdx.x == 0 && threadIdx.x == 0) { scale_out[0] = s; hist[2 * kHistArray + 2 + (1 - src)] = assumed; }
    float m = 0.f;
    f32x4 cs = {0.f, 0.f, 0.f, 0.f};
    for (int64_t i = blockIdx.x * 256 + threadIdx.x; i < n4; i += (int64_t)gridDim.x * 256) {
        f32x4 v = *reinterpret_cast<const f32x4*>(x + 4 * i);
        cs += v;
        v = split_act(v, relu, slope);
        m = fmaxf(fmaxf(m, fabsf(v[0])), fmaxf(fabsf(v[1]), fmaxf(fabsf(v[2]), fabsf(v[3]))));
        v = v * s;
        f16x4 h, l;
        #pragma unroll
        for (int j = 0; j < 4; ++j) { h[j] = (_Float16)v[j]; l[j] = (_Float16)(v[j] - (float)h[j]); }
        *reinterpret_cast<f16x4*>(hi + 4 * i) = h;
        *reinterpret_cast<f16x4*>(lo + 4 * i) = l;
    }
    #pragma unroll
    for (int o = 32; o > 0; o >>= 1) m = fmaxf(m, __shfl_xor(m, o));
    if ((threadIdx.x & 63) == 0) red[threadIdx.x >> 6] = m;
    if (colsum) red4[threadIdx.x] = cs;
    __syncthreads();
    if (threadIdx.x == 0) {
        const f32x2h p = {fmaxf(fmaxf(red[0], red[1]), fmaxf(red[2], red[3])), __builtin_bit_cast(float, tag)};
        *reinterpret_cast<f32x2h*>(hist + (1 - src) * kHistArray + 2 * blockIdx.x) = p;
    }
    if (colsum && (int)threadIdx.x < c4n) {
        f32x4 t = red4[threadIdx.x];
        for (int p = threadIdx.x + c4n; p < 256; p += c4n) t += red4[p];
        *reinterpret_cast<f32x4*>(colsum + (int64_t)blockIdx.x * 4 * c4n + 4 * threadIdx.x) = t;
    }
}

constexpr int kHistRedoWord = 2 * kHistArray;
__global__ __launch_bounds__(256) void conv_split_redo_kernel(const float* __restrict__ x, int64_t n4, int relu, _Float16* __restrict__ hi,
                                                              _Float16* __restrict__ lo, float* __restrict__ scale_out,
                                                              float* __restrict__ hist, float slope = 0.f)
{
    typedef int i32x2h __attribute__((ext_vector_type(2)));
    float mx[2] = {0.f, 0.f};
    int tg[2] = {0, 0};
    #pragma unroll
    for (int arr = 0; arr < 2; ++arr)
        #pragma unroll
        for (int i = 0; i < kAmaxBlocks / 64; ++i) {
            const i32x2h p = *reinterpret_cast<const i32x2h*>(hist + arr * kHistArray + 2 * ((threadIdx.x & 63) + 64 * i));
            mx[arr] = fmaxf(mx[arr], __builtin_bit_cast(float, p[0]));
            tg[arr] = max(tg[arr], p[1]);
        }
    #pragma unroll
    for (int o = 32; o > 0; o >>= 1)
        #pragma unroll
        for (int arr = 0; arr < 2; ++arr) {
            mx[arr] = fmaxf(mx[arr], __shfl_xor(mx[arr], o));
            tg[arr] = max(tg[arr], __shfl_xor(tg[arr], o));
        }
    const int now = tg[1] > tg[0] ? 1 : 0;
    const float own = mx[now], assumed = hist[2 * kHistArray + 2 + now];
    const float s_used = scale_for(assumed * kHistMargin);
    const float top = own * s_used;
    const bool fine = !(own > 0.f) || !(own < 3.0e38f) || (top >= 0.03125f && top < 65504.0f);
    if (fine) return;
    const float s = scale_for(own);
    if (blockIdx.x == 0 && threadIdx.x == 0) {
        scale_out[0] = s;
        reinterpret_cast<unsigned*>(hist)[kHistRedoWord] += 1u;
    }
    for (int64_t i = blockIdx.x * 256 + threadIdx.x; i < n4; i += (int64_t)gridDim.x * 256) {
        f32x4 v = *reinterpret_cast<const f32x4*>(x + 4 * i);
        v = split_act(v, relu, slope);
        v = v * s;
        f16x4 h, l;
        #pragma unroll
        for (int j = 0; j < 4; ++j) { h[j] = (_Float16)v[j]; l[j] = (_Float16)(v[j] - (float)h[j]); }
        *reinterpret_cast<f16x4*>(hi + 4 * i) = h;
        *reinterpret_cast<f16x4*>(lo + 4 * i) = l;
    }
}

struct WeightArgs {
    const float* w; int64_t sk, sn, sr, ss;
    const float* amax; float* scale_out; char* img;
    int K, Nn, ntaps, nphase;
    int64_t n4;
    float coef, bound_mul;
    int amax_count;
    signed char nsrc[kMaxPhase][kMaxTaps];
    signed char r[kMaxPhase][kMaxTaps][4], s[kMaxPhase][kMaxTaps][4];
};

__device__ __forceinline__ void conv_weights_body(const WeightArgs& a, const int bid, const int nblocks)
{
    float sc;
    if (a.amax) sc = scale_of(a.amax, a.bound_mul, a.amax_count);
    else {
        __shared__ float red[4];
        float m = 0.f;
        for (int64_t i = threadIdx.x; i < a.n4; i += 256) {
            const f32x4 v = *reinterpret_cast<const f32x4*>(a.w + 4 * i);
            m = fmaxf(fmaxf(m, fabsf(v[0])), fmaxf(fabsf(v[1]), fmaxf(fabsf(v[2]), fabsf(v[3]))));
        }
        #pragma unroll
        for (int o = 32; o > 0; o >>= 1) m = fmaxf(m, __shfl_xor(m, o));
        if ((threadIdx.x & 63) == 0) red[threadIdx.x >> 6] = m;
        __syncthreads();
        m = fmaxf(fmaxf(red[0], red[1]), fmaxf(red[2], red[3])) * a.bound_mul;
        sc = 1.0f;
        if (m > 0.f && m < 3.0e38f) { int e; (void)frexpf(m, &e); sc = ldexpf(1.0f, 14 - e); }
    }
    if (bid == 0 && threadIdx.x == 0) a.scale_out[0] = sc;
    const int nchunk = a.K >> 5, nblk = a.Nn >> 5;
    const int64_t groups = (int64_t)a.nphase * a.ntaps * nchunk * nblk * 2 * 64;
    for (int64_t g = (int64_t)bid * 256 + threadIdx.x; g < groups; g += (int64_t)nblocks * 256) {
        const int lane = g & 63;
        int64_t t = g >> 6;
// ... 306 lines not shown
            for (int j = 0; j < NB; ++j) o[j * 32] = acc[i][j][r];
        }
}

template <int MB, int NB>
__global__ __launch_bounds__(256) void conv_wrw_kernel(WrwArgs a) { conv_wrw_body<MB, NB>(a, blockIdx.x, blockIdx.y); }

struct WrwReduceArgs {
    const float* partial; int splits, nslice, Ca, Cb;
    const float* xscale; const float* gscale;
    float* dw; int64_t sa, sb, sr, ss;
    float coef;
    const float* colsum; float* db; int c4n, main_blocks;
    int nout;
    signed char r[kMaxTaps], s[kMaxTaps], cnt[kMaxTaps], slice[kMaxTaps][4];
};

__device__ __forceinline__ void conv_wrw_reduce_body(const WrwReduceArgs& a, const unsigned bid)
{
    if ((int)bid >= a.main_blocks) {
        const int u = ((int)bid - a.main_blocks) * 256 + threadIdx.x, cg = u >> 6, lane = u & 63;
        if (cg >= a.c4n) return;
        f32x4 v = {0.f, 0.f, 0.f, 0.f};
        for (int b = lane; b < kAmaxBlocks; b += 64) v += *reinterpret_cast<const f32x4*>(a.colsum + (int64_t)b * 4 * a.c4n + 4 * cg);
        #pragma unroll
        for (int j = 0; j < 4; ++j)
            #pragma unroll
            for (int o = 1; o < 64; o <<= 1) v[j] += __shfl_xor(v[j], o);
        if (lane == 0) *reinterpret_cast<f32x4*>(a.db + 4 * cg) = v;
        return;
    }
    const int64_t plane = (int64_t)a.Ca * a.Cb, per = (int64_t)a.nslice * plane, total4 = (int64_t)a.nout * plane >> 2;
    const float inv = a.coef / (a.xscale[0] * a.gscale[0]);
    const int part = threadIdx.x & 3;
    for (int64_t e4 = ((int64_t)bid * 256 + threadIdx.x) >> 2; e4 < total4; e4 += (int64_t)a.main_blocks * 64) {
        const int64_t e = e4 * 4;
        const int o = e / plane; const int64_t w = e - o * plane;
        f32x4 v = {0.f, 0.f, 0.f, 0.f};
        for (int i = 0; i < a.cnt[o]; ++i) {
            const float* src = a.partial + a.slice[o][i] * plane + w;
            int sp = part;
            for (; sp + 28 < a.splits; sp += 32) {
                f32x4 t[8];
                #pragma unroll
                for (int u = 0; u < 8; ++u) t[u] = *reinterpret_cast<const f32x4*>(src + (int64_t)(sp + 4 * u) * per);
                #pragma unroll
                for (int u = 0; u < 8; ++u) v += t[u];
            }
            for (; sp < a.splits; sp += 4) v += *reinterpret_cast<const f32x4*>(src + sp * per);
        }
        #pragma unroll
        for (int j = 0; j < 4; ++j) { v[j] += __shfl_xor(v[j], 1); v[j] += __shfl_xor(v[j], 2); }
        if (part != 0) continue;
        v = v * inv;
        const int cb = w % a.Cb, ca = w / a.Cb;
        float* out = a.dw + ca * a.sa + cb * a.sb + a.r[o] * a.sr + a.s[o] * a.ss;
        if (a.sb == 1 && ((uintptr_t)out & 15) == 0) *reinterpret_cast<f32x4*>(out) = v;
        else { out[0] = v[0]; out[a.sb] = v[1]; out[2 * a.sb] = v[2]; out[3 * a.sb] = v[3]; }
    }
}

__global__ __launch_bounds__(256) void conv_wrw_reduce_kernel(WrwReduceArgs a) { conv_wrw_reduce_body(a, blockIdx.x); }

template <bool KS>
__global__ __launch_bounds__(256) void conv_bwd_pair_kernel(ConvArgs d, WrwArgs w, int conv_blocks, int wrw_off, int wrw_splits, int gx, int gy)
{
    const int b = blockIdx.x;
    if (b < conv_blocks) {
        const int t = b / gx, z = t / gy;
        conv_f16x3_body<2, 2, KS>(d, (unsigned)(b - t * gx), (unsigned)(t - z * gy), (unsigned)z);
    } else if (b >= wrw_off) {
        const int e = b - wrw_off, tile = e / wrw_splits;
        conv_wrw_body<2, 2>(w, (unsigned)(e - tile * wrw_splits), (unsigned)tile);
    }
}

__global__ __launch_bounds__(256) void conv_pair_reduce_kernel(WrwReduceArgs r, KsplitReduceArgs k, int wrw_blocks)
{
    if ((int)blockIdx.x < wrw_blocks) conv_wrw_reduce_body(r, blockIdx.x);
    else conv_ksplit_reduce_body(k.partial, k.ksplit, k.n4, k.cout, k.xscale, k.wscale, k.bias, k.relu, k.y,
                                 blockIdx.x - wrw_blocks, gridDim.x - wrw_blocks);
}

struct NarrowWrwArgs {
    const float* x; const float* gy; float* partial;
    int N, H, W, Cin, Cout, ks, nrow;
    unsigned magHW, shHW, magW, shW;
    int64_t M; int64_t pix_per_wave;
};

__global__ __launch_bounds__(512, 1) void conv_wrw_narrow_kernel(NarrowWrwArgs a)
{
    extern __shared__ __attribute__((aligned(16))) float nw_part[];
    const int tid = threadIdx.x, lane = tid & 63;
    const int wave = __builtin_amdgcn_readfirstlane(tid >> 6);
    const int i = lane & 31, k = lane >> 5;
    const int grp = blockIdx.y;
    const bool is_tap = i < a.nrow, is_one = i == a.nrow;
    int dy = 0, dx = 0, c = 0;
    if (is_tap) {
        const int tap = i / a.Cin;
        c = i - tap * a.Cin;
        dy = tap / a.ks - a.ks / 2; dx = tap % a.ks - a.ks / 2;
    }
    const unsigned HW = (unsigned)(a.H * a.W);
    f32x16 acc[4];
#pragma unroll
    for (int q = 0; q < 4; ++q)
#pragma unroll
        for (int r = 0; r < 16; ++r) acc[q][r] = 0.f;
    const int64_t p0 = ((int64_t)blockIdx.x * 8 + wave) * a.pix_per_wave;
    int64_t p1 = p0 + a.pix_per_wave;
    if (p1 > a.M) p1 = a.M;
    const float* gyc = a.gy + grp * 128 + (grp * 128 + 4 * i < a.Cout ? 4 * i : 0);
    constexpr int U = 8;
    for (int64_t p = p0; p < p1; p += 2 * U) {
        float av[U]; f32x4 bv[U];
#pragma unroll
        for (int u = 0; u < U; ++u) {
            const int64_t pp = p + 2 * u + k;
            const bool ok = pp < p1;
            const unsigned pc = (unsigned)(ok ? pp : a.M - 1);
            const unsigned n = __umulhi(pc, a.magHW) >> a.shHW, rem = pc - n * HW;
            const unsigned yy = __umulhi(rem, a.magW) >> a.shW, xx = rem - yy * a.W;
            const int iy = (int)yy + dy, ix = (int)xx + dx;
            const bool inb = ok && is_tap && (unsigned)iy < (unsigned)a.H && (unsigned)ix < (unsigned)a.W;
            const float xv = a.x[inb ? ((int64_t)(n * a.H + iy) * a.W + ix) * a.Cin + c : 0];
            av[u] = inb ? xv : ((ok && is_one) ? 1.f : 0.f);
            bv[u] = *reinterpret_cast<const f32x4*>(gyc + (int64_t)pc * a.Cout);
        }
#pragma unroll
        for (int u = 0; u < U; ++u)
#pragma unroll
            for (int q = 0; q < 4; ++q) acc[q] = __builtin_amdgcn_mfma_f32_32x32x2f32(av[u], bv[u][q], acc[q], 0, 0, 0);
    }
#pragma unroll
    for (int q = 0; q < 4; ++q)
#pragma unroll
        for (int r = 0; r < 16; ++r) nw_part[((wave * 4 + q) * 16 + r) * 64 + lane] = acc[q][r];
    __syncthreads();
    float* out = a.partial + ((int64_t)blockIdx.y * gridDim.x + blockIdx.x) * 4096;
#pragma unroll
    for (int m = 0; m < 8; ++m) {
        const int e = tid + 512 * m;
        float sum = nw_part[e];
#pragma unroll
        for (int w = 1; w < 8; ++w) sum += nw_part[w * 4096 + e];
        out[e] = sum;
    }
}

__global__ __launch_bounds__(256) void conv_wrw_narrow_reduce_kernel(const float* __restrict__ partial, int nparts, int Cin, int ks, int nrow,
                                                                     float* __restrict__ dw, int64_t sk, int64_t sn, int64_t sr, int64_t ss,
                                                                     float* __restrict__ db, int Cout)
{
    __shared__ float red[8][32];
    const int el = threadIdx.x & 31, pg = threadIdx.x >> 5;
    const int e = blockIdx.x * 32 + el;
    const float* p = partial + (int64_t)blockIdx.y * nparts * 4096 + e;
    float sum = 0.f;
    int z = pg;
    for (; z + 8 * 15 < nparts; z += 8 * 16) {
        float v[16];
#pragma unroll
        for (int u = 0; u < 16; ++u) v[u] = p[(int64_t)(z + 8 * u) * 4096];
#pragma unroll
// ... 421 lines not shown
    return k < 1 ? 1 : (k > 8 ? 8 : k);
}

size_t wc_conv_workspace_bytes(const wc_conv_geom* g)
{
    if (!g) return 0;
    const int k = conv_ksplit(g);
    return k > 1 ? (size_t)k * g->N * g->Hout * g->Wout * g->Cout * 4 : 0;
}

static bool conv_big_tile(const wc_conv_geom* g, int ksplit)
{
    const int64_t M = (int64_t)g->N * g->H * g->W;
    const bool wide = (g->Cout % 256) == 0;
    const int64_t wgs_big = (M / 256) * g->nphase * (g->Cout / (wide ? 256 : 128));
    return ksplit == 1 && (M % 256) == 0 && wgs_big >= 256;
}

static int conv_prepare(ConvArgs& a, const void* xhi, const void* xlo, const float* xscale, const void* wimage, const float* wscale,
                        const float* bias, const void* zero_line, const wc_conv_geom* g, int relu, float* y, void* ws, size_t ws_bytes)
{
    if (!xhi || !xlo || !xscale || !wimage || !wscale || !zero_line || !g || !y) return WC_ERR_ARG;
    if (!wc_conv_supported(g)) return WC_ERR_SHAPE;
    a.xhi = (const _Float16*)xhi; a.xlo = (const _Float16*)xlo; a.zero = (const _Float16*)zero_line;
    a.wimg = (const char*)wimage; a.xscale = xscale; a.wscale = wscale; a.bias = bias; a.y = y;
    a.N = g->N; a.H = g->H; a.W = g->W; a.Hin = g->Hin; a.Win = g->Win; a.Cin = g->Cin; a.Cout = g->Cout;
    a.in_stride = g->in_stride; a.ntaps = g->ntaps; a.nphase = g->nphase; a.Hout = g->Hout; a.Wout = g->Wout;
    a.out_stride = g->out_stride; a.relu = relu;
    a.ksplit = conv_ksplit(g); a.partial = (float*)ws;
    magic_u31((unsigned)(g->H * g->W), &a.magHW, &a.shHW);
    magic_u31((unsigned)g->W, &a.magW, &a.shW);
    if (a.ksplit > 1 && (!ws || ws_bytes < wc_conv_workspace_bytes(g))) return WC_ERR_WORKSPACE;
    for (int p = 0; p < kMaxPhase; ++p) {
        a.offy[p] = g->off_y[p]; a.offx[p] = g->off_x[p];
        for (int t = 0; t < kMaxTaps; ++t) { a.dy[p][t] = g->dy[p][t]; a.dx[p][t] = g->dx[p][t]; }
    }
    return WC_OK;
}

int wc_conv_f16x3(const void* xhi, const void* xlo, const float* xscale, const void* wimage, const float* wscale,
                  const float* bias, const void* zero_line, const wc_conv_geom* g, int relu, float* y,
                  void* ws, size_t ws_bytes, wc_stream_t stream)
{
    hipStream_t st = (hipStream_t)stream;
    ConvArgs a;
    const int rc = conv_prepare(a, xhi, xlo, xscale, wimage, wscale, bias, zero_line, g, relu, y, ws, ws_bytes);
    if (rc != WC_OK) return rc;
    const bool wide = (g->Cout % 256) == 0;
    hipError_t e;
    if (g->Cout % 128)                                      e = a.ksplit > 1 ? launch_conv<2, 1, true>(a, st) : launch_conv<2, 1>(a, st);
    else if (conv_big_tile(g, a.ksplit))                    e = wide ? launch_conv<4, 4>(a, st) : launch_conv<4, 2>(a, st);
    else if (a.ksplit > 1)                                  e = wide ? launch_conv<2, 4, true>(a, st) : launch_conv<2, 2, true>(a, st);
    else                                                    e = wide ? launch_conv<2, 4>(a, st) : launch_conv<2, 2>(a, st);
    if (e != hipSuccess) return (int)e;
    if (a.ksplit > 1) {
        const int64_t n4 = (int64_t)g->N * g->Hout * g->Wout * g->Cout / 4;
        hipLaunchKernelGGL(conv_ksplit_reduce_kernel, dim3(grid_for(n4)), dim3(256), 0, st, (const float*)ws, a.ksplit, n4, g->Cout,
                           xscale, wscale, bias, relu, y);
    }
    return (int)hipGetLastError();
}

int wc_conv_res_supported(const wc_conv_geom* g)
{
    return g && wc_conv_supported(g) && (g->Cout % 128) == 0 && conv_ksplit(g) > 1;
}

int wc_conv_res_f16x3(const void* xhi, const void* xlo, const float* xscale, const void* wimage, const float* wscale,
                      const float* bias, const float* res, const void* zero_line, const wc_conv_geom* g, float* y,
                      void* ws, size_t ws_bytes, wc_stream_t stream)
{
    hipStream_t st = (hipStream_t)stream;
    if (!res) return WC_ERR_ARG;
    ConvArgs a;
    const int rc = conv_prepare(a, xhi, xlo, xscale, wimage, wscale, bias, zero_line, g, 0, y, ws, ws_bytes);
    if (rc != WC_OK) return rc;
    if (!wc_conv_res_supported(g)) return WC_ERR_SHAPE;
    const hipError_t e = (g->Cout % 256) == 0 ? launch_conv<2, 4, true>(a, st) : launch_conv<2, 2, true>(a, st);
    if (e != hipSuccess) return (int)e;
    const int64_t n4 = (int64_t)g->N * g->Hout * g->Wout * g->Cout / 4;
    hipLaunchKernelGGL(conv_ksplit_reduce_res_kernel, dim3(grid_for(n4)), dim3(256), 0, st, (const float*)ws, a.ksplit, n4, g->Cout,
                       xscale, wscale, bias, res, y);
    return (int)hipGetLastError();
}

int wc_conv_block_dx_f32(const float* dx1, const float* x, const float* other, int64_t N, int64_t H, int64_t W, int C, int down,
                         float* out, wc_stream_t stream)
{
    if (!dx1 || !x || !other || !out) return WC_ERR_NULL;
    if (N <= 0 || H <= 0 || W <= 0 || C <= 0 || (C & 3) || H > 0x7fffffff || W > 0x7fffffff) return WC_ERR_SHAPE;
    if (down && ((H & 1) || (W & 1))) return WC_ERR_SHAPE;
    const int64_t n4 = N * H * W * (C >> 2);
    hipStream_t st = (hipStream_t)stream;
    if (down) hipLaunchKernelGGL(conv_block_dx_kernel<true>, dim3(grid_for(n4)), dim3(256), 0, st, dx1, x, other, n4, C >> 2, (int)W, (int)H, out);
    else      hipLaunchKernelGGL(conv_block_dx_kernel<false>, dim3(grid_for(n4)), dim3(256), 0, st, dx1, x, other, n4, C >> 2, (int)W, (int)H, out);
    return (int)hipGetLastError();
}

static int wrw_splits(const wc_conv_geom* g, int* tile)
{
    const bool wide = (g->Cin % 256 == 0) && (g->Cout % 256 == 0) && g->nphase * g->ntaps * (g->Cin / 256) * (g->Cout / 256) >= 4;
    *tile = wide ? 256 : ((g->Cin % 128) || (g->Cout % 128)) ? 64 : 128;
    const int tiles = g->nphase * g->ntaps * (g->Cin / *tile) * (g->Cout / *tile);
    const int64_t nchunks = (int64_t)g->N * g->H * g->W / 32;
    int splits = kWrwTargetWgs / tiles / 8 * 8;
    if (splits < 8) splits = 8;
    if (splits > 64) splits = 64;
    if (splits > nchunks) splits = (int)nchunks;
    return splits < 1 ? 1 : splits;
}

int wc_conv_wrw_narrow_supported(int64_t N, int64_t H, int64_t W, int Cin, int Cout, int ksize);
int wc_conv_narrow64_supported(int64_t N, int64_t H, int64_t W, int Cin, int Cout, int ksize);

int wc_conv_fwd_narrow_f32(const float* x, const float* w, int64_t stride_k, int64_t stride_n, int64_t stride_r, int64_t stride_s,
                           const float* bias, int64_t N, int64_t H, int64_t W, int Cin, int Cout, int ksize, int relu, float* y, wc_stream_t stream)
{
    if (!x || !w || !y) return WC_ERR_ARG;
    if (!wc_conv_narrow64_supported(N, H, W, Cin, Cout, ksize) || N * H * W * Cin >= ((int64_t)1 << 31)) return WC_ERR_SHAPE;
    hipStream_t st = (hipStream_t)stream;
    NarrowFwdArgs a = {};
    a.x = x; a.w = w; a.bias = bias; a.y = y;
    a.N = (int)N; a.H = (int)H; a.W = (int)W; a.Cin = Cin; a.Cout = Cout; a.ks = ksize; a.nrow = ksize * ksize * Cin; a.relu = relu;
    a.sk = stride_k; a.sn = stride_n; a.sr = stride_r; a.ss = stride_s;
    magic_u31((unsigned)(H * W), &a.magHW, &a.shHW);
    magic_u31((unsigned)W, &a.magW, &a.shW);
    for (int m = 0; m < 32; ++m) {
        const int tap = m < a.nrow ? m / Cin : 0, c = m < a.nrow ? m % Cin : 0;
        a.tr[m] = (signed char)(tap / ksize); a.ts[m] = (signed char)(tap % ksize); a.tch[m] = (signed char)c;
        a.tdy[m] = (signed char)(tap / ksize - ksize / 2); a.tdx[m] = (signed char)(tap % ksize - ksize / 2);
    }
    a.M = N * H * W;
    a.ntiles = (int)((a.M + 31) / 32);
    a.tiles_per_wave = (a.ntiles + 1023) / 1024;
    if (a.tiles_per_wave < 1) a.tiles_per_wave = 1;
    const int nwg = (a.ntiles + 4 * a.tiles_per_wave - 1) / (4 * a.tiles_per_wave);
    const int ks2 = (a.nrow + 2) / 2;
    dim3 grid(nwg, Cout / (32 * kNarrowNQ));
    if (ks2 <= 2) hipLaunchKernelGGL(conv_fwd_narrow_kernel<2>, grid, dim3(256), 0, st, a);
    else if (ks2 <= 5) hipLaunchKernelGGL(conv_fwd_narrow_kernel<5>, grid, dim3(256), 0, st, a);
    else if (ks2 <= 10) hipLaunchKernelGGL(conv_fwd_narrow_kernel<10>, grid, dim3(256), 0, st, a);
    else if (ks2 <= 14) hipLaunchKernelGGL(conv_fwd_narrow_kernel<14>, grid, dim3(256), 0, st, a);
    else hipLaunchKernelGGL(conv_fwd_narrow_kernel<16>, grid, dim3(256), 0, st, a);
    return (int)hipGetLastError();
}

static int64_t narrow_wrw_parts(int64_t M, int64_t* pix_per_wave)
{
    int64_t ppw = (M + 256 * 8 - 1) / (256 * 8);
    if (ppw < 16) ppw = 16;
    ppw = (ppw + 1) & ~(int64_t)1;
    *pix_per_wave = ppw;
    return (M + 8 * ppw - 1) / (8 * ppw);
}

int wc_conv_narrow64_supported(int64_t N, int64_t H, int64_t W, int Cin, int Cout, int ksize)
{
    if (N <= 0 || H <= 0 || W <= 0 || Cin <= 0 || Cout <= 0 || (ksize != 1 && ksize != 3)) return 0;
    if (ksize * ksize * Cin >= 32 || (Cout & 63)) return 0;
    return N * H * W < ((int64_t)1 << 31) ? 1 : 0;
}

int wc_conv_wrw_narrow_supported(int64_t N, int64_t H, int64_t W, int Cin, int Cout, int ksize)
{
    return ((Cout & 127) == 0 && wc_conv_narrow64_supported(N, H, W, Cin, Cout, ksize)) ? 1 : 0;
}
// ... 89 lines not shown
            if (ph >= g->nphase || t >= g->ntaps) continue;
            if (g->nsrc[ph][t] < 1 || g->nsrc[ph][t] > 4) return WC_ERR_ARG;
            for (int m = 0; m < g->nsrc[ph][t]; ++m) {
                int o = 0;
                while (o < r.nout && (r.r[o] != g->wr[ph][t][m] || r.s[o] != g->ws[ph][t][m])) ++o;
                if (o == r.nout) {
                    if (r.nout == kMaxTaps) return WC_ERR_ARG;
                    r.r[o] = g->wr[ph][t][m]; r.s[o] = g->ws[ph][t][m]; r.cnt[o] = 0; ++r.nout;
                }
                if (r.cnt[o] == 4) return WC_ERR_ARG;
                r.slice[o][r.cnt[o]++] = (signed char)(ph * g->ntaps + t);
            }
        }
    const bool x_cols = stride_k == 1;
    a.A = x_cols ? G : X; a.B = x_cols ? X : G;
    a.zero = (const _Float16*)zero_line; a.partial = (float*)ws;
    a.N = g->N; a.H = g->H; a.W = g->W; a.ntaps = g->ntaps; a.nphase = g->nphase;
    magic_u31((unsigned)(g->H * g->W), &a.magHW, &a.shHW);
    magic_u31((unsigned)g->W, &a.magW, &a.shW);
    a.nchunks = nchunks; a.cps = (nchunks + splits - 1) / splits;
    splits = (nchunks + a.cps - 1) / a.cps;
    r.partial = (const float*)ws; r.splits = splits; r.nslice = nslice; r.Ca = a.A.C; r.Cb = a.B.C;
    r.xscale = xscale; r.gscale = gscale; r.dw = dw;
    r.sa = x_cols ? stride_n : stride_k; r.sb = x_cols ? stride_k : stride_n; r.sr = stride_r; r.ss = stride_s;
    r.colsum = colsum_partials; r.db = db; r.c4n = db ? g->Cout >> 2 : 0;
    r.main_blocks = grid_for((int64_t)r.nout * g->Cin * g->Cout);
    p.T = T; p.splits = splits; p.tiles = tiles; p.extra = db ? (r.c4n * 64 + 255) / 256 : 0;
    return WC_OK;
}

int wc_conv_wrw_bias_f16x3(const void* xhi, const void* xlo, const float* xscale, const void* ghi, const void* glo, const float* gscale,
                           const void* zero_line, const wc_conv_geom* g, float* dw, int64_t stride_k, int64_t stride_n,
                           int64_t stride_r, int64_t stride_s, const float* colsum_partials, float* db,
                           void* ws, size_t ws_bytes, wc_stream_t stream)
{
    hipStream_t st = (hipStream_t)stream;
    WrwPlan p;
    const int rc = wrw_prepare(p, xhi, xlo, xscale, ghi, glo, gscale, zero_line, g, dw, stride_k, stride_n, stride_r, stride_s,
                               colsum_partials, db, ws, ws_bytes);
    if (rc != WC_OK) return rc;
    const WrwArgs& a = p.a;
    const WrwReduceArgs& r = p.r;
    const int T = p.T;
    dim3 grid((unsigned)p.splits, (unsigned)p.tiles);
    hipError_t e = hipSuccess;
    if (T == 256) {
        constexpr int LDS = 2 * (2 * 4 * 4 * 1024 + 2 * 4 * 4 * 1024);
        e = wc_set_max_lds(reinterpret_cast<const void*>(conv_wrw_kernel<4, 4>), LDS);
        if (e != hipSuccess) return (int)e;
        hipLaunchKernelGGL((conv_wrw_kernel<4, 4>), grid, dim3(256), LDS, st, a);
    } else if (T == 64) {
        constexpr int LDS = 2 * (2 * 1 * 4 * 1024 + 2 * 1 * 4 * 1024);
        e = wc_set_max_lds(reinterpret_cast<const void*>(conv_wrw_kernel<1, 1>), LDS);
        if (e != hipSuccess) return (int)e;
        hipLaunchKernelGGL((conv_wrw_kernel<1, 1>), grid, dim3(256), LDS, st, a);
    } else {
        constexpr int LDS = 2 * (2 * 2 * 4 * 1024 + 2 * 2 * 4 * 1024);
        e = wc_set_max_lds(reinterpret_cast<const void*>(conv_wrw_kernel<2, 2>), LDS);
        if (e != hipSuccess) return (int)e;
        hipLaunchKernelGGL((conv_wrw_kernel<2, 2>), grid, dim3(256), LDS, st, a);
    }
    hipLaunchKernelGGL(conv_wrw_reduce_kernel, dim3(r.main_blocks + p.extra), dim3(256), 0, st, r);
    return (int)hipGetLastError();
}

int wc_conv_bwd_pair_supported(const wc_conv_geom* gd, const wc_conv_geom* gf)
{
    if (!gd || !gf || !wc_conv_supported(gd) || !wc_conv_supported(gf) || (gf->Cin & 63) || gf->H * gf->W < 2) return 0;
    if (gd->N != gf->N || gd->Cin != gf->Cout || gd->Cout != gf->Cin) return 0;
    if (gd->Hin != gf->Hout || gd->Win != gf->Wout || gd->Hout != gf->Hin || gd->Wout != gf->Win) return 0;
    if (gf->nphase != 1 || gd->in_stride != 1) return 0;
    if ((gd->Cout % 128) != 0 || (gd->Cout % 256) == 0 || conv_big_tile(gd, conv_ksplit(gd))) return 0;
    int tile;
    (void)wrw_splits(gf, &tile);
    return tile == 128 ? 1 : 0;
}

size_t wc_conv_bwd_pair_workspace_bytes(const wc_conv_geom* gd, const wc_conv_geom* gf)
{
    if (!gd || !gf) return 0;
    return wc_conv_workspace_bytes(gd) + wc_conv_wrw_workspace_bytes(gf);
}

int wc_conv_bwd_pair_f16x3(const void* ghi, const void* glo, const float* gscale, const void* wimage, const float* wscale,
                           const void* zero_line, const wc_conv_geom* gd, float* dx, void* ws_dx, size_t ws_dx_bytes,
                           const void* xhi, const void* xlo, const float* xscale, const wc_conv_geom* gf, float* dw,
                           int64_t stride_k, int64_t stride_n, int64_t stride_r, int64_t stride_s,
                           const float* colsum_partials, float* db, void* ws_dw, size_t ws_dw_bytes, wc_stream_t stream)
{
    hipStream_t st = (hipStream_t)stream;
    ConvArgs d;
    int rc = conv_prepare(d, ghi, glo, gscale, wimage, wscale, nullptr, zero_line, gd, 0, dx, ws_dx, ws_dx_bytes);
    if (rc != WC_OK) return rc;
    WrwPlan p;
    rc = wrw_prepare(p, xhi, xlo, xscale, ghi, glo, gscale, zero_line, gf, dw, stride_k, stride_n, stride_r, stride_s,
                     colsum_partials, db, ws_dw, ws_dw_bytes);
    if (rc != WC_OK) return rc;
    if (!wc_conv_bwd_pair_supported(gd, gf) || p.T != 128) return WC_ERR_SHAPE;
    constexpr int LDS = 2 * (2 * 2 * 4 * 1024 + 2 * 2 * 4 * 1024);
    const int64_t M = (int64_t)gd->N * gd->H * gd->W;
    const int gx = (int)(M / 128), gy = gd->nphase * (gd->Cout / 128);
    const int64_t conv_blocks = (int64_t)gx * gy * d.ksplit, wrw_off = (conv_blocks + 7) & ~(int64_t)7;
    const int64_t blocks = wrw_off + (int64_t)p.splits * p.tiles;
    if (blocks > 0x7fffffff) return WC_ERR_SHAPE;
    hipError_t e;
    if (d.ksplit > 1) {
        e = wc_set_max_lds(reinterpret_cast<const void*>(conv_bwd_pair_kernel<true>), LDS);
        if (e != hipSuccess) return (int)e;
        hipLaunchKernelGGL((conv_bwd_pair_kernel<true>), dim3((unsigned)blocks), dim3(256), LDS, st, d, p.a,
                           (int)conv_blocks, (int)wrw_off, p.splits, gx, gy);
    } else {
        e = wc_set_max_lds(reinterpret_cast<const void*>(conv_bwd_pair_kernel<false>), LDS);
        if (e != hipSuccess) return (int)e;
        hipLaunchKernelGGL((conv_bwd_pair_kernel<false>), dim3((unsigned)blocks), dim3(256), LDS, st, d, p.a,
                           (int)conv_blocks, (int)wrw_off, p.splits, gx, gy);
    }
    e = hipGetLastError();
    if (e != hipSuccess) return (int)e;
    const int reduce_blocks = p.r.main_blocks + p.extra;
    if (d.ksplit > 1) {
        KsplitReduceArgs k;
        k.n4 = (int64_t)gd->N * gd->Hout * gd->Wout * gd->Cout / 4;
        k.partial = (const float*)ws_dx; k.ksplit = d.ksplit; k.cout = gd->Cout;
        k.xscale = gscale; k.wscale = wscale; k.bias = nullptr; k.relu = 0; k.y = dx;
        hipLaunchKernelGGL(conv_pair_reduce_kernel, dim3(reduce_blocks + grid_for(k.n4)), dim3(256), 0, st, p.r, k, reduce_blocks);
    } else {
        hipLaunchKernelGGL(conv_wrw_reduce_kernel, dim3(reduce_blocks), dim3(256), 0, st, p.r);
    }
    return (int)hipGetLastError();
}

}
```

wc_gan_amd/csrc/wc_gp.hip:

```cpp
#include "wc_common.h"
#include "../../include/wc_hip.h"

namespace {

constexpr int kAmaxBlocks = 512;
constexpr float kHistMargin = 64.0f;
constexpr int kHistArray = 2 * kAmaxBlocks;
constexpr int kHistRedoWord = 2 * kHistArray;

__device__ __forceinline__ f32x4 masked_load(const float* __restrict__ t, const float* __restrict__ a, int64_t i, float slope)
{
    f32x4 v = *reinterpret_cast<const f32x4*>(t + 4 * i);
    const f32x4 p = *reinterpret_cast<const f32x4*>(a + 4 * i);
    #pragma unroll
    for (int j = 0; j < 4; ++j) v[j] = v[j] * (p[j] > 0.f ? 1.0f : slope);
    return v;
}

__device__ __forceinline__ float absmax4(float m, f32x4 v)
{
    return fmaxf(fmaxf(m, fabsf(v[0])), fmaxf(fabsf(v[1]), fmaxf(fabsf(v[2]), fabsf(v[3]))));
}

__device__ __forceinline__ void store_split(f32x4 v, float s, _Float16* __restrict__ hi, _Float16* __restrict__ lo, int64_t i)
{
    v = v * s;
    f16x4 h, l;
    #pragma unroll
    for (int j = 0; j < 4; ++j) { h[j] = (_Float16)v[j]; l[j] = (_Float16)(v[j] - (float)h[j]); }
    *reinterpret_cast<f16x4*>(hi + 4 * i) = h;
    *reinterpret_cast<f16x4*>(lo + 4 * i) = l;
}

__device__ __forceinline__ float scale_for(float amax)
{
    if (!(amax > 0.f) || !(amax < 3.0e38f)) return 1.0f;
    int e;
    (void)frexpf(amax, &e);
    return ldexpf(1.0f, 14 - e);
}

__device__ __forceinline__ float wave_max(float m)
{
    #pragma unroll
    for (int o = 32; o > 0; o >>= 1) m = fmaxf(m, __shfl_xor(m, o));
    return m;
}

__device__ __forceinline__ f32x4 colsum_add(f32x4 cs, f32x4 v)
{
    #pragma unroll
    for (int j = 0; j < 4; ++j) cs[j] = __fadd_rn(cs[j], v[j]);
    return cs;
}

__device__ __forceinline__ void colsum_fold(f32x4* red4, float* __restrict__ colsum, int c4n)
{
    if (colsum && (int)threadIdx.x < c4n) {
        f32x4 s = red4[threadIdx.x];
        for (int p = threadIdx.x + c4n; p < 256; p += c4n) s += red4[p];
        *reinterpret_cast<f32x4*>(colsum + (int64_t)blockIdx.x * 4 * c4n + 4 * threadIdx.x) = s;
    }
}

__global__ __launch_bounds__(256) void gp_absmax_kernel(const float* __restrict__ t, const float* __restrict__ a, int64_t n4, float slope,
                                                        float* __restrict__ partial, float* __restrict__ colsum = nullptr, int c4n = 0)
{
    __shared__ float red[4];
    __shared__ f32x4 red4[256];
    float m = 0.f;
    f32x4 cs = {0.f, 0.f, 0.f, 0.f};
    for (int64_t i = blockIdx.x * 256 + threadIdx.x; i < n4; i += (int64_t)gridDim.x * 256) {
        const f32x4 v = masked_load(t, a, i, slope);
        m = absmax4(m, v);
        cs = colsum_add(cs, v);
    }
    m = wave_max(m);
    if ((threadIdx.x & 63) == 0) red[threadIdx.x >> 6] = m;
    if (colsum) red4[threadIdx.x] = cs;
    __syncthreads();
    if (threadIdx.x == 0) partial[blockIdx.x] = fmaxf(fmaxf(red[0], red[1]), fmaxf(red[2], red[3]));
    colsum_fold(red4, colsum, c4n);
}

__global__ __launch_bounds__(256) void gp_split_kernel(const float* __restrict__ t, const float* __restrict__ a, int64_t n4, float slope,
                                                       const float* __restrict__ amax, _Float16* __restrict__ hi, _Float16* __restrict__ lo,
                                                       float* __restrict__ scale_out)
{
    float m = 0.f;
    for (int i = threadIdx.x & 63; i < kAmaxBlocks; i += 64) m = fmaxf(m, amax[i]);
    const float s = scale_for(wave_max(m));
    if (blockIdx.x == 0 && threadIdx.x == 0) scale_out[0] = s;
    for (int64_t i = blockIdx.x * 256 + threadIdx.x; i < n4; i += (int64_t)gridDim.x * 256) store_split(masked_load(t, a, i, slope), s, hi, lo, i);
}

typedef float f32x2h __attribute__((ext_vector_type(2)));
typedef int i32x2h __attribute__((ext_vector_type(2)));

__global__ __launch_bounds__(kAmaxBlocks) void gp_hist_seed_kernel(float* __restrict__ hist)
{
    const float m = hist[threadIdx.x];
    __syncthreads();
    const f32x2h a = {m, __builtin_bit_cast(float, 1u)}, b = {0.f, __builtin_bit_cast(float, 0u)};
    *reinterpret_cast<f32x2h*>(hist + 2 * threadIdx.x) = a;
    *reinterpret_cast<f32x2h*>(hist + kHistArray + 2 * threadIdx.x) = b;
    __shared__ float red[kAmaxBlocks / 64];
    const float mm = wave_max(m);
    if ((threadIdx.x & 63) == 0) red[threadIdx.x >> 6] = mm;
    __syncthreads();
    if (threadIdx.x == 0) {
        float top = 0.f;
        for (int i = 0; i < kAmaxBlocks / 64; ++i) top = fmaxf(top, red[i]);
        hist[2 * kHistArray + 2] = top; hist[2 * kHistArray + 3] = top;
    }
}

__global__ __launch_bounds__(256) void gp_split_hist_kernel(const float* __restrict__ t, const float* __restrict__ a, int64_t n4, float slope,
                                                            _Float16* __restrict__ hi, _Float16* __restrict__ lo, float* __restrict__ scale_out,
                                                            float* __restrict__ hist, float* __restrict__ colsum, int c4n)
{
    __shared__ float red[4];
    __shared__ f32x4 red4[256];
    float mx[2] = {0.f, 0.f};
    int tlo[2] = {0x7fffffff, 0x7fffffff}, thi[2] = {0, 0};
    #pragma unroll
    for (int arr = 0; arr < 2; ++arr)
        #pragma unroll
        for (int i = 0; i < kAmaxBlocks / 64; ++i) {
            const i32x2h p = *reinterpret_cast<const i32x2h*>(hist + arr * kHistArray + 2 * ((threadIdx.x & 63) + 64 * i));
            mx[arr] = fmaxf(mx[arr], __builtin_bit_cast(float, p[0]));
            tlo[arr] = min(tlo[arr], p[1]);
            thi[arr] = max(thi[arr], p[1]);
        }
    #pragma unroll
    for (int o = 32; o > 0; o >>= 1)
        #pragma unroll
// ... 71 lines not shown
__global__ __launch_bounds__(256) void gp_interp_kernel(const float* __restrict__ real, const float* __restrict__ fake, const float* __restrict__ eps,
                                                        int64_t total, int64_t L, float* __restrict__ out)
{
    for (int64_t i = (int64_t)blockIdx.x * 256 + threadIdx.x; i < total; i += (int64_t)gridDim.x * 256) {
        const double e = (double)eps[i / L];
        out[i] = (float)(e * (double)real[i] + (1.0 - e) * (double)fake[i]);
    }
}

__global__ __launch_bounds__(256) void gp_rows_kernel(const float* __restrict__ g, int64_t L, double two_lambda_over_n, float* __restrict__ norms,
                                                      float* __restrict__ v, double* __restrict__ terms)
{
    __shared__ double red[4];
    const float* row = g + (int64_t)blockIdx.x * L;
    float* out = v + (int64_t)blockIdx.x * L;
    double ss = 0.0;
    for (int64_t i = threadIdx.x; i < L; i += 256) { const double x = (double)row[i]; ss += x * x; }
    #pragma unroll
    for (int o = 32; o > 0; o >>= 1) ss += __shfl_xor(ss, o);
    if ((threadIdx.x & 63) == 0) red[threadIdx.x >> 6] = ss;
    __syncthreads();
    const double norm = sqrt((red[0] + red[1]) + (red[2] + red[3]));
    const double coef = norm > 0.0 ? two_lambda_over_n * (1.0 - 1.0 / norm) : 0.0;
    if (threadIdx.x == 0) { norms[blockIdx.x] = (float)norm; terms[blockIdx.x] = (norm - 1.0) * (norm - 1.0); }
    for (int64_t i = threadIdx.x; i < L; i += 256) out[i] = (float)(coef * (double)row[i]);
}

__global__ __launch_bounds__(64) void gp_finish_kernel(const double* __restrict__ terms, int64_t N, double lambda_over_n, float* __restrict__ penalty)
{
    double s = 0.0;
    for (int64_t i = threadIdx.x; i < N; i += 64) s += terms[i];
    #pragma unroll
    for (int o = 32; o > 0; o >>= 1) s += __shfl_xor(s, o);
    if (threadIdx.x == 0) penalty[0] = (float)(lambda_over_n * s);
}

}

extern "C" {

static bool colsum_args_ok(const float* colsum_partials, int C, int64_t n)
{
    return !colsum_partials || (C > 0 && !(C & 3) && 256 % (C >> 2) == 0 && n % C == 0);
}

int wc_conv_split_masked_f32(const float* t, const float* a, int64_t n, float slope, void* hi, void* lo, float* scale, void* amax_scratch,
                             float* colsum_partials, int C, wc_stream_t stream)
{
    if (!t || !a || !hi || !lo || !scale || !amax_scratch || n <= 0 || (n & 3)) return WC_ERR_ARG;
    if (!(slope >= 0.f && slope <= 1.f)) return WC_ERR_ARG;
    if (!colsum_args_ok(colsum_partials, C, n)) return WC_ERR_SHAPE;
    hipStream_t st = (hipStream_t)stream;
    hipLaunchKernelGGL(gp_absmax_kernel, dim3(kAmaxBlocks), dim3(256), 0, st, t, a, n / 4, slope, (float*)amax_scratch,
                       colsum_partials, colsum_partials ? C >> 2 : 0);
    hipLaunchKernelGGL(gp_split_kernel, dim3(grid_for(n / 4)), dim3(256), 0, st, t, a, n / 4, slope, (const float*)amax_scratch,
                       (_Float16*)hi, (_Float16*)lo, scale);
    return (int)hipGetLastError();
}

int wc_conv_split_hist_masked_f32(const float* t, const float* a, int64_t n, float slope, void* hi, void* lo, float* scale,
                                  float* colsum_partials, int C, float* hist, int bootstrap, wc_stream_t stream)
{
    if (!t || !a || !hi || !lo || !scale || !hist || n <= 0 || (n & 3)) return WC_ERR_ARG;
    if (!(slope >= 0.f && slope <= 1.f)) return WC_ERR_ARG;
    if (!colsum_args_ok(colsum_partials, C, n)) return WC_ERR_SHAPE;
    hipStream_t st = (hipStream_t)stream;
    const int c4n = colsum_partials ? C >> 2 : 0;
    if (bootstrap & 1) {
        hipLaunchKernelGGL(gp_absmax_kernel, dim3(kAmaxBlocks), dim3(256), 0, st, t, a, n / 4, slope, hist, colsum_partials, c4n);
        hipLaunchKernelGGL(gp_split_kernel, dim3(grid_for(n / 4)), dim3(256), 0, st, t, a, n / 4, slope, (const float*)hist, (_Float16*)hi,
                           (_Float16*)lo, scale);
        hipLaunchKernelGGL(gp_hist_seed_kernel, dim3(1), dim3(kAmaxBlocks), 0, st, hist);
        return (int)hipGetLastError();
    }
    hipLaunchKernelGGL(gp_split_hist_kernel, dim3(kAmaxBlocks), dim3(256), 0, st, t, a, n / 4, slope, (_Float16*)hi, (_Float16*)lo, scale, hist,
                       colsum_partials, c4n);
    if (!(bootstrap & 2)) {
        const unsigned g2 = grid_for(n / 4) < 64 ? grid_for(n / 4) : 64u;
        hipLaunchKernelGGL(gp_split_redo_kernel, dim3(g2), dim3(256), 0, st, t, a, n / 4, slope, (_Float16*)hi, (_Float16*)lo, scale, hist);
    }
    return (int)hipGetLastError();
}

int wc_gp_interp_f32(const float* real, const float* fake, const float* eps, int64_t N, int64_t L, float* x_hat, wc_stream_t stream)
{
    if (!real || !fake || !eps || !x_hat) return WC_ERR_NULL;
    if (N <= 0 || L <= 0) return WC_ERR_SHAPE;
    hipLaunchKernelGGL(gp_interp_kernel, dim3(grid_for(N * L)), dim3(256), 0, (hipStream_t)stream, real, fake, eps, N * L, L, x_hat);
    return (int)hipGetLastError();
}

size_t wc_gp_rows_workspace_bytes(int64_t N) { return N > 0 ? (size_t)N * sizeof(double) : 0; }

int wc_gp_rows_f32(const float* g, int64_t N, int64_t L, double lambda, double inv_n, float* norms, float* v, float* penalty,
                   void* ws, size_t ws_bytes, wc_stream_t stream)
{
    if (!g || !norms || !v || !penalty || !ws) return WC_ERR_NULL;
    if (N <= 0 || L <= 0 || N >= ((int64_t)1 << 31)) return WC_ERR_SHAPE;
    if (ws_bytes < wc_gp_rows_workspace_bytes(N)) return WC_ERR_WORKSPACE;
    hipStream_t st = (hipStream_t)stream;
    hipLaunchKernelGGL(gp_rows_kernel, dim3((unsigned)N), dim3(256), 0, st, g, L, 2.0 * lambda * inv_n, norms, v, (double*)ws);
    hipLaunchKernelGGL(gp_finish_kernel, dim3(1), dim3(64), 0, st, (const double*)ws, N, lambda * inv_n, penalty);
    return (int)hipGetLastError();
}

}
```

wc_gan_amd/discriminator.py:

```python
from __future__ import annotations

from functools import partial

import torch
import torch.nn as nn
import torch.nn.functional as F

from .generator import Conv2D, create_norm, to_nchw_view, to_nhwc


def downsample2x(x):
    return to_nhwc(F.avg_pool2d(to_nchw_view(x), 2))


class ResBlockDown(nn.Module):
    def __init__(self, in_ch, nfilters, resample, name, norm, conv_layer, is_first):
        super().__init__()
        assert resample in ('DOWN', 'SAME')
        self.resample, self.is_first = resample, is_first
        self.bn1 = norm(axis=-1, name=name + '.bn1', channels=in_ch)
        self.conv1 = conv_layer(in_ch, nfilters, (3, 3), name=name + '.conv1')
        self.bn2 = norm(axis=-1, name=name + '.bn2', channels=nfilters)
        self.conv2 = conv_layer(nfilters, nfilters, (3, 3), name=name + '.conv2')
        self.has_shortcut = (in_ch != nfilters) or resample == 'DOWN'
        if self.has_shortcut:
            self.shortcut = conv_layer(in_ch, nfilters, (1, 1), name=name + '.shortcut')

    def _fusable(self):
        from . import conv as fc, generator as _g
        if self.is_first or not (fc.FUSED_BLOCK and _g.FAST_CONV):
            return False
        if not all(isinstance(bn, _g._UnfusedStack) and bn.norm_layer is None and len(bn.branches) == 0 for bn in (self.bn1, self.bn2)):
            return False
        convs = [self.conv1, self.conv2] + ([self.shortcut] if self.has_shortcut else [])
        return all(isinstance(c, Conv2D) and c.kind == 'same' and c.conv.weight.dtype == torch.float32 for c in convs)

    def _fused_plans(self, x):
        from . import conv as fc, generator as _g
        if not self._fusable():
            return None
        if not (torch.is_tensor(x) and x.is_cuda and x.dtype == torch.float32 and x.dim() == 4 and x.is_contiguous()
                and getattr(x, '_wc_planes', None) is None and _g.split_of(x) is None):
            return None
        return fc.critic_block_plans(tuple(x.shape), tuple(self.conv1.conv.weight.shape), tuple(self.conv2.conv.weight.shape),
                                     tuple(self.shortcut.conv.weight.shape) if self.has_shortcut else None, self.resample == 'DOWN')

    def forward(self, x, cls):
        plans = self._fused_plans(x)
        if plans is not None:
            from . import conv as fc
            w1, w2 = self.conv1._weight(), self.conv2._weight()
            ws = self.shortcut._weight() if self.has_shortcut else None
            x = self.bn1(x, cls)
            y, h = fc.critic_block(x, w1, self.conv1.conv.bias, w2, self.conv2.conv.bias, ws, self.shortcut.conv.bias if self.has_shortcut else None,
                                   (self.conv1, self.conv2, self.shortcut if self.has_shortcut else None), plans, self.resample == 'DOWN')
            self.bn2(h, cls)
            return y
        h = self.conv1(x) if self.is_first else self.conv1.forward_relu(self.bn1(x, cls))
        h = self.bn2(h, cls)
        s = x
        if self.resample == 'DOWN':
            from . import generator as _g
            if h.shape[1] * h.shape[2] >= 1024 or (_g.FAST_CONV and h.is_cuda):
                h = self.conv2.forward_pooled(h, relu_input=True)
            else:
                h = downsample2x(self.conv2.forward_relu(h))
            s = downsample2x(s)
        else:
            h = self.conv2.forward_relu(h)
        if self.has_shortcut:
            s = self.shortcut(s)
        return h + s


LEAKY_SLOPE = 0.3


class DCBlockDown(nn.Module):

    def __init__(self, in_ch, nfilters, resample, name, norm, conv_layer, is_first):
        super().__init__()
        assert resample in ('DOWN', 'SAME')
        self.resample, self.is_first = resample, is_first
        self.bn = norm(axis=-1, name=name + '.bn', channels=in_ch)
        if resample == 'DOWN':
            self.conv = conv_layer(in_ch, nfilters, (4, 4), name=name + '.conv', stride=2)
        else:
            self.conv = conv_layer(in_ch, nfilters, (3, 3), name=name + '.conv')

    def forward(self, x, cls):
        if self.is_first:
            return self.conv(x)
        return self.conv.forward_leaky(self.bn(x, cls), LEAKY_SLOPE)


class Discriminator(nn.Module):
    def __init__(self, in_ch, block_sizes, resamples, norm_layer, conv_layer, dense, emb, number_of_classes, type,
                 sum_pool, dropout, arch='res', input_hw=None, fused_tail=False, fused_projection=False):
        super().__init__()
        self.fused_tail = bool(fused_tail)
        self.fused_projection = bool(fused_projection)
        blocks = []
        ch = in_ch
        self.arch = arch
        block = ResBlockDown if arch == 'res' else DCBlockDown
        for i, (bs, rs) in enumerate(zip(block_sizes, resamples)):
            bs = int(bs)
            blocks.append(block(ch, bs, rs, 'Discriminator.' + str(i), norm_layer, conv_layer, is_first=(i == 0)))
            ch = bs
        self.blocks = nn.ModuleList(blocks)
        self.sum_pool, self.type = sum_pool, type
        self.dropout = nn.Dropout(dropout) if dropout else None
        emb_dim = ch
        if arch == 'dcgan':
            h, w = (int(v) for v in input_hw)
            for rs in resamples:
                if rs == 'DOWN':
                    if h % 2 or w % 2:
                        raise ValueError(f"arch='dcgan': a DOWN block halves a {h} x {w} grid")
                    h, w = h // 2, w // 2
            if type == 'PROJECTIVE' and h * w != 1:
                raise ValueError(f"arch='dcgan' with type='PROJECTIVE' needs a 1 x 1 final grid (the embedding has block_sizes[-1] = {ch} "
                                 f"dimensions, the flattened features {h} x {w} x {ch}); no shipped recipe combines them")
            ch = h * w * ch
        self.out = dense(ch, 1)
        if type == 'AC_GAN':
            self.cls_out = nn.Linear(ch, number_of_classes)
            nn.init.xavier_uniform_(self.cls_out.weight); nn.init.zeros_(self.cls_out.bias)
        elif type == 'PROJECTIVE':
            self.emb = emb(number_of_classes, emb_dim)

    def _tail_is_fused(self):
        return self.fused_tail and self.arch == 'res' and self.dropout is None and self.type in (None, 'AC_GAN')

    def _projection_is_fused(self):
        return self.fused_projection and self.arch == 'res' and self.dropout is None and self.type == 'PROJECTIVE'

    def forward(self, x, cls=None, labels=None):
        if labels is not None and self.type != 'AC_GAN':
            raise ValueError("Discriminator.forward: labels are the AC_GAN class head's; this critic has type " + repr(self.type))
        from .spectral import prepare_spectral
        prepare_spectral(self)
        from . import conv as fc
        batch = torch.is_tensor(x) and x.is_cuda
        if batch:
            fc.prepare_images(self, fc.pass_key(self, x))
        try:
            y = x
            for blk in self.blocks:
                y = blk(y, cls)
        finally:
            if batch:
                fc.finish_images(self)
        if self._tail_is_fused():
            from .tail import critic_tail
            w_out = self.out.normalized_weight() if hasattr(self.out, 'normalized_weight') else self.out.weight
            ac = self.type == 'AC_GAN'
            out, logits, ce = critic_tail(y, w_out, self.out.bias, self.cls_out.weight if ac else None, self.cls_out.bias if ac else None,
                                          labels, self.sum_pool)
            if not ac:
                return out
            return (out, logits) if labels is None else (out, logits, ce)
        if self._projection_is_fused():
            from .tail import projection_tail
            w_out = self.out.normalized_weight() if hasattr(self.out, 'normalized_weight') else self.out.weight
            table = self.emb.normalized_weight() if hasattr(self.emb, 'normalized_weight') else self.emb.weight
            return projection_tail(y, w_out, self.out.bias, table, cls, self.sum_pool)
        if self.arch == 'dcgan':
            y = F.leaky_relu(y, LEAKY_SLOPE).flatten(1)
        else:
            y = F.relu(y)
            y = y.sum(dim=(1, 2)) if self.sum_pool else y.mean(dim=(1, 2))
        if self.dropout is not None:
            y = self.dropout(y)
        out = self.out(y)
        if self.type == 'AC_GAN':
            logits = self.cls_out(y)
            if labels is None:
                return out, logits
            return out, logits, F.cross_entropy(logits, labels.reshape(-1).long(), reduction='none')
        if self.type == 'PROJECTIVE':
            out = out + (self.emb(cls.reshape(-1).long()) * y).sum(dim=1, keepdim=True)
        return out


def make_discriminator(input_image_shape=(32, 32, 3), input_cls_shape=(1,), block_sizes=(128, 128, 128, 128),
                       resamples=('DOWN', 'DOWN', 'SAME', 'SAME'), number_of_classes=10,
                       type='AC_GAN', norm='n', after_norm='n', spectral=False,
                       fully_diff_spectral=False, spectral_iterations=1, conv_singular=True,
                       sum_pool=False, dropout=False, arch='res', filters_emb=10, fused_tail=False, fused_projection=False):
    assert arch in ('res', 'dcgan')
    assert type in [None, 'AC_GAN', 'PROJECTIVE']
    if spectral and conv_singular:
        import warnings
        warnings.warn("conv_singular=True is not built: spectral normalisation uses the reshaped-kernel singular value",
                      stacklevel=2)
    sn_kw = dict(spectral_iterations=spectral_iterations, fully_diff_spectral=fully_diff_spectral)
    conv_layer = partial(Conv2D, spectral=bool(spectral), conv_singular=conv_singular, **sn_kw)

    def dense(i, o):
        if spectral:
            from .spectral import SNLinear
            lin = SNLinear(i, o, **sn_kw)
            with torch.no_grad():
                nn.init.xavier_uniform_(lin.weight); nn.init.zeros_(lin.bias)
                lin._sn_init(**sn_kw)
            return lin
        lin = nn.Linear(i, o)
        nn.init.xavier_uniform_(lin.weight); nn.init.zeros_(lin.bias)
        return lin

    def emb(k, d):
        if spectral:
            from .spectral import SNEmbedding
            return SNEmbedding(k, d, **sn_kw)
        return nn.Embedding(k, d)

    norm_layer = create_norm(norm, after_norm, number_of_classes=number_of_classes, filters_emb=filters_emb)
    return Discriminator(int(input_image_shape[-1]), block_sizes, resamples, norm_layer, conv_layer, dense, emb,
                         number_of_classes, type, sum_pool, dropout, arch=arch, input_hw=input_image_shape[:2], fused_tail=fused_tail,
                         fused_projection=fused_projection)
```

Baseline: 3805 images/sec.

## Fuse fp16 plane splitting into conv epilogues across critic blocks

Adds conv tail epilogues that write the hi/lo fp16 split planes of the conv output straight from the forward conv kernel. It also adds masked-gradient split and dx-combine tails to the backward pair kernel. Adjacent critic blocks hand their split planes forward, so the next block skips its own split pass. The aim is to remove separate split and mask kernels and the extra activation reads they cost. In exchange the conv kernels grow more complex, and a guarded redo path may relaunch the split when the scale history is off.

```diff
diff --git a/include/wc_hip.h b/include/wc_hip.h
--- a/include/wc_hip.h
+++ b/include/wc_hip.h
@@ -351,6 +351,32 @@
                               int64_t stride_k, int64_t stride_n, int64_t stride_r, int64_t stride_s,
                               const float* colsum_partials, float* db, void* ws_dw, size_t ws_dw_bytes, wc_stream_t stream);
 
+#define WC_CONV_TAIL_SPLIT 1
+#define WC_CONV_TAIL_MASKED 2
+#define WC_CONV_TAIL_DX 3
+typedef struct wc_conv_tail {
+    int kind;
+    int redo;
+    const float* res;
+    const float* mask;
+    const float* other;
+    float* out;
+    void* hi; void* lo; float* scale; float* hist;
+    float* colsum_partials; int C;
+} wc_conv_tail;
+int wc_conv_tail_supported(const wc_conv_geom* g);
+int wc_conv_tail_f16x3(const void* xhi, const void* xlo, const float* xscale, const void* wimage, const float* wscale,
+                       const float* bias, const void* zero_line, const wc_conv_geom* g, float* y,
+                       void* ws, size_t ws_bytes, const wc_conv_tail* tail, wc_stream_t stream);
+int wc_conv_bwd_pair_tail_f16x3(const void* ghi, const void* glo, const float* gscale, const void* wimage, const float* wscale,
+                                const void* zero_line, const wc_conv_geom* gd, float* dx, void* ws_dx, size_t ws_dx_bytes,
+                                const void* xhi, const void* xlo, const float* xscale, const wc_conv_geom* gf, float* dw,
+                                int64_t stride_k, int64_t stride_n, int64_t stride_r, int64_t stride_s,
+                                const float* colsum_partials, float* db, void* ws_dw, size_t ws_dw_bytes,
+                                const wc_conv_tail* tail, wc_stream_t stream);
+int wc_conv_split_redo_masked_f32(const float* t, const float* a, int64_t n, float slope, void* hi, void* lo, float* scale, float* hist,
+                                  wc_stream_t stream);
+
 int wc_stream_copy_f32(const float* src, float* dst, int64_t n, wc_stream_t stream);
 
 
diff --git a/wc_gan_amd/_lib.py b/wc_gan_amd/_lib.py
--- a/wc_gan_amd/_lib.py
+++ b/wc_gan_amd/_lib.py
@@ -162,6 +162,13 @@
     "wc_conv_bwd_pair_f16x3": (c_int, [c_void_p, c_void_p, c_void_p, c_void_p, c_void_p, c_void_p, c_void_p, c_void_p, c_void_p, c_size_t,
                                        c_void_p, c_void_p, c_void_p, c_void_p, c_void_p, c_int64, c_int64, c_int64, c_int64,
                                        c_void_p, c_void_p, c_void_p, c_size_t, c_void_p]),
+    "wc_conv_tail_supported": (c_int, [c_void_p]),
+    "wc_conv_tail_f16x3": (c_int, [c_void_p, c_void_p, c_void_p, c_void_p, c_void_p, c_void_p, c_void_p, c_void_p, c_void_p,
+                                   c_void_p, c_size_t, c_void_p, c_void_p]),
+    "wc_conv_bwd_pair_tail_f16x3": (c_int, [c_void_p, c_void_p, c_void_p, c_void_p, c_void_p, c_void_p, c_void_p, c_void_p, c_void_p, c_size_t,
+                                            c_void_p, c_void_p, c_void_p, c_void_p, c_void_p, c_int64, c_int64, c_int64, c_int64,
+                                            c_void_p, c_void_p, c_void_p, c_size_t, c_void_p, c_void_p]),
+    "wc_conv_split_redo_masked_f32": (c_int, [c_void_p, c_void_p, c_int64, c_float, c_void_p, c_void_p, c_void_p, c_void_p, c_void_p]),
     "wc_std_stats_workspace_bytes": (c_size_t, [c_int64, c_int, c_int]),
     "wc_std_stats_f32": (c_int, [c_void_p, c_int64, c_int, c_int, c_void_p, c_void_p, c_void_p, c_size_t, c_void_p]),
     "wc_std_factor_f64": (c_int, [c_void_p, c_void_p, c_int64, c_int, c_int, c_double, c_double, c_int, c_int, c_void_p, c_void_p,
@@ -251,6 +258,14 @@
                 ("amax_count", c_int), ("pair_of", c_int)]
 
 
+TAIL_SPLIT, TAIL_MASKED, TAIL_DX = 1, 2, 3
+
+
+class ConvTail(ctypes.Structure):
+    _fields_ = [("kind", c_int), ("redo", c_int), ("res", c_void_p), ("mask", c_void_p), ("other", c_void_p), ("out", c_void_p),
+                ("hi", c_void_p), ("lo", c_void_p), ("scale", c_void_p), ("hist", c_void_p), ("colsum_partials", c_void_p), ("C", c_int)]
+
+
 class ConvAbsmaxJob(ctypes.Structure):
     _fields_ = [("x", c_void_p), ("n", c_int64), ("partial", c_void_p)]
 
diff --git a/wc_gan_amd/build.py b/wc_gan_amd/build.py
--- a/wc_gan_amd/build.py
+++ b/wc_gan_amd/build.py
@@ -9,7 +9,7 @@
 CSRC = os.path.join(HERE, "csrc")
 LIB = os.path.join(HERE, "libwc_hip.so")
 SOURCES = ["wc_rows.hip", "wc_fast.hip", "wc_split.hip", "wc_split_xty.hip", "wc_resadd.hip", "wc_fast_xty.hip", "wc_small.hip", "wc_zca.hip", "wc_renorm.hip", "wc_mix.hip", "wc_std.hip", "wc_sn.hip", "wc_conv.hip", "wc_gp.hip", "wc_adam.hip", "wc_tail.hip", "wc_abi.hip"]
-HEADERS = ["wc_common.h", os.path.join("..", "..", "include", "wc_hip.h")]
+HEADERS = ["wc_common.h", "wc_mask.h", os.path.join("..", "..", "include", "wc_hip.h")]
 FLAGS = ["--offload-arch=gfx950", "-O3", "-std=c++17", "-fPIC", "-ffp-contract=fast", "-Wall", "-Wno-unused-function"] + \
     os.environ.get("WC_EXTRA_FLAGS", "").split()
 
diff --git a/wc_gan_amd/conv.py b/wc_gan_amd/conv.py
--- a/wc_gan_amd/conv.py
+++ b/wc_gan_amd/conv.py
@@ -88,7 +88,7 @@
 
 
 class _Plan:
-    __slots__ = ('ok', 'fwd', 'bwd', 'fwd_ws', 'bwd_ws', 'wrw_ws', 'fwd_ptr', 'bwd_ptr', 'pair', 'res')
+    __slots__ = ('ok', 'fwd', 'bwd', 'fwd_ws', 'bwd_ws', 'wrw_ws', 'fwd_ptr', 'bwd_ptr', 'pair', 'res', 'tail', 'bwd_tail')
 
     def __init__(self, kind, N, H, W, wshape):
         class _W:
@@ -103,6 +103,8 @@
         self.wrw_ws = lib.wc_conv_wrw_workspace_bytes(self.fwd_ptr) if self.ok else 0
         self.pair = self.ok and bool(lib.wc_conv_bwd_pair_supported(self.bwd_ptr, self.fwd_ptr))
         self.res = self.ok and bool(lib.wc_conv_res_supported(self.fwd_ptr))
+        self.tail = self.ok and bool(lib.wc_conv_tail_supported(self.fwd_ptr))
+        self.bwd_tail = self.ok and bool(lib.wc_conv_tail_supported(self.bwd_ptr))
 
 
 _plans = {}
@@ -489,14 +491,71 @@
     return dw
 
 
-def backward_pair(g_planes, image, x_planes, plan, w, colsum=None):
+def _reader_record(site, role, device):
+    if not (SPLIT_HIST and site is not None and getattr(site, 'training', True)):
+        return None
+    h = site.__dict__.get('_wc_split_hist', {}).get(role)
+    if h is None or not h[1] or h[0].device != device:
+        return None
+    return h
+
+
+class _Tail:
+
+    def __init__(self, kind, shape, device, record=None, role='x', res=None, mask=None, other=None, colsum=False):
+        t = self.c = _lib.ConvTail()
+        t.kind = kind
+        self.keep = (res, mask, other, record)
+        self.planes = self.out = None
+        if kind == _lib.TAIL_DX:
+            self.out = torch.empty(shape, dtype=torch.float32, device=device)
+            t.mask, t.other, t.out = _ptr(mask), _ptr(other), _ptr(self.out)
+            return
+        both = torch.empty((2,) + tuple(shape), dtype=torch.float16, device=device)
+        scale = torch.empty(1 + 512, dtype=torch.float32, device=device)
+        t.hi, t.lo, t.scale, t.hist = _ptr(both[0]), _ptr(both[1]), _ptr(scale), _ptr(record[0])
+        t.redo = 1 if _guarded(role) else 0
+        self.planes = (both[0], both[1], scale)
+        if kind == _lib.TAIL_SPLIT:
+            t.res = _ptr(res) if res is not None else None
+            return
+        t.mask = _ptr(mask)
+        if colsum:
+            part = torch.empty((512, shape[-1]), dtype=torch.float32, device=device)
+            t.colsum_partials, t.C = _ptr(part), shape[-1]
+            self.planes += (part,)
+
+
+def _dense32(t, shape):
+    return t.is_contiguous() and tuple(t.shape) == tuple(shape) and t.dtype == torch.float32
+
+
+def run_tail(planes, image, geom, tail, bias=None, nbytes=None):
+    hi, lo, xs = planes
+    img, ws = image
+    lib = _lib.load()
+    y = None
+    if tail.c.kind != _lib.TAIL_DX:
+        y = torch.empty((geom.N, geom.Hout, geom.Wout, geom.Cout), dtype=torch.float32, device=hi.device)
+    if nbytes is None:
+        nbytes = lib.wc_conv_workspace_bytes(ctypes.addressof(geom))
+    work = torch.empty(nbytes, dtype=torch.uint8, device=hi.device) if nbytes else None
+    _lib.check(lib.wc_conv_tail_f16x3(_ptr(hi), _ptr(lo), _ptr(xs), _ptr(img), _ptr(ws), _ptr(bias) if bias is not None else None,
+                                      _ptr(_zero_line(hi.device)), ctypes.addressof(geom), _ptr(y), _ptr(work), nbytes,
+                                      ctypes.addressof(tail.c), _stream()), "wc_conv_tail_f16x3")
+    return y
+
+
+def backward_pair(g_planes, image, x_planes, plan, w, colsum=None, tail=None):
     lib = _lib.load()
     gh, gl, gs = g_planes[:3]
     xh, xl, xs = x_planes
     img, ws = image
     gf, kf, nf = plan.fwd
     gb = plan.bwd[0]
-    dx = torch.empty((gb.N, gb.Hout, gb.Wout, gb.Cout), dtype=torch.float32, device=gh.device)
+    dx = None
+    if tail is None or tail.c.kind != _lib.TAIL_DX:
+        dx = torch.empty((gb.N, gb.Hout, gb.Wout, gb.Cout), dtype=torch.float32, device=gh.device)
     dw = torch.empty_like(w)
     if dw.stride() != w.stride():
         raise ValueError("weight must be dense")
@@ -504,6 +563,13 @@
     work_dw = torch.empty(plan.wrw_ws, dtype=torch.uint8, device=gh.device)
     db = torch.empty(gf.Cout, dtype=torch.float32, device=w.device) if colsum is not None else None
     zero = _zero_line(gh.device)
+    if tail is not None:
+        _lib.check(lib.wc_conv_bwd_pair_tail_f16x3(_ptr(gh), _ptr(gl), _ptr(gs), _ptr(img), _ptr(ws), _ptr(zero), plan.bwd_ptr, _ptr(dx),
+                                                   _ptr(work_dx), plan.bwd_ws,
+                                                   _ptr(xh), _ptr(xl), _ptr(xs), plan.fwd_ptr, _ptr(dw), w.stride(kf), w.stride(nf),
+                                                   w.stride(2), w.stride(3), _ptr(colsum), _ptr(db), _ptr(work_dw), plan.wrw_ws,
+                                                   ctypes.addressof(tail.c), _stream()), "wc_conv_bwd_pair_tail_f16x3")
+        return dx, dw, db
     _lib.check(lib.wc_conv_bwd_pair_f16x3(_ptr(gh), _ptr(gl), _ptr(gs), _ptr(img), _ptr(ws), _ptr(zero), plan.bwd_ptr, _ptr(dx),
                                           _ptr(work_dx), plan.bwd_ws,
                                           _ptr(xh), _ptr(xl), _ptr(xs), plan.fwd_ptr, _ptr(dw), w.stride(kf), w.stride(nf), w.stride(2),
@@ -828,15 +894,18 @@
     return weight_image(w, gf, kf, nf, site=site), None
 
 
-def _layer_gradients(g_planes, fused_db, x_planes, w, plan, bwd_image, need_dx, need_dw):
+def _layer_gradients(g_planes, fused_db, x_planes, w, plan, bwd_image, need_dx, need_dw, tail=None):
     cs = g_planes[3] if fused_db else None
     if need_dx and need_dw and bwd_image is not None and plan.pair:
-        return backward_pair(g_planes, bwd_image, x_planes, plan, w, colsum=cs)
+        return backward_pair(g_planes, bwd_image, x_planes, plan, w, colsum=cs, tail=tail)
     dx = dw = db = None
     if need_dx:
         gb, kb, nb = plan.bwd
         image = bwd_image if bwd_image is not None else weight_image(w, gb, kb, nb)
-        dx = run(g_planes[:3], image, gb, nbytes=plan.bwd_ws)
+        if tail is not None:
+            dx = run_tail(g_planes[:3], image, gb, tail, nbytes=plan.bwd_ws)
+        else:
+            dx = run(g_planes[:3], image, gb, nbytes=plan.bwd_ws)
     if need_dw:
         gf, kf, nf = plan.fwd
         if fused_db:
@@ -850,37 +919,60 @@
     return F.avg_pool2d(x.permute(0, 3, 1, 2), 2).permute(0, 2, 3, 1).contiguous()
 
 
+FUSED_FINISH = True
+FUSED_FINISH_F1 = True
+FUSED_FINISH_F2 = True
+FUSED_FINISH_B1 = True
+FUSED_FINISH_B2 = True
+
+
 class _CriticBlock(torch.autograd.Function):
     @staticmethod
-    def forward(ctx, x, w1, b1, w2, b2, ws, bs, sites, plans, down):
+    def forward(ctx, x, w1, b1, w2, b2, ws, bs, sites, plans, down, next_site=None, xh=None, xl=None, xs=None, backward_tails=False):
         conv1, conv2, shortcut = sites
         p1, p2, ps = plans
         need = ctx.needs_input_grad
         need_h = need[0] or need[1] or need[2]
-        x_pl = split_planes(x, relu=True, site=conv1, role='x')
+        x_pl = (xh, xl, xs) if xh is not None else split_planes(x, relu=True, site=conv1, role='x')
         img1, bimg1 = _images(w1, p1, need[0], conv1)
-        h = run(x_pl, img1, p1.fwd[0], b1, nbytes=p1.fwd_ws)
-        h_pl = split_planes(h, relu=True, site=conv2, role='x')
+        rec = _reader_record(conv2, 'x', x.device) if (FUSED_FINISH and FUSED_FINISH_F1 and p1.tail) else None
+        if rec is not None:
+            t1 = _Tail(_lib.TAIL_SPLIT, (p1.fwd[0].N, p1.fwd[0].Hout, p1.fwd[0].Wout, p1.fwd[0].Cout), x.device, record=rec, role='x')
+            h = run_tail(x_pl, img1, p1.fwd[0], t1, bias=b1, nbytes=p1.fwd_ws)
+            h_pl = t1.planes
+        else:
+            h = run(x_pl, img1, p1.fwd[0], b1, nbytes=p1.fwd_ws)
+            h_pl = split_planes(h, relu=True, site=conv2, role='x')
         img2, bimg2 = _images(w2, p2, need_h, conv2)
         s, s_pl, bimgs = x, (), None
         if ws is not None:
             s_pl = split_planes(_pool2(x) if down else x, site=shortcut, role='x')
             imgs, bimgs = _images(ws, ps, need[0], shortcut)
             s = run(s_pl, imgs, ps.fwd[0], bs, nbytes=ps.fwd_ws)
-        if p2.res and FUSED_RESIDUAL:
-            y = run(h_pl, img2, p2.fwd[0], b2, nbytes=p2.fwd_ws, res=s)
+        n_pl = ()
+        g2 = p2.fwd[0]
+        rec = None
+        if next_site is not None and FUSED_FINISH and FUSED_FINISH_F2 and FUSED_RESIDUAL and p2.tail and _dense32(s, (g2.N, g2.Hout, g2.Wout, g2.Cout)):
+            rec = _reader_record(next_site, 'x', x.device)
+        if rec is not None:
+            t2 = _Tail(_lib.TAIL_SPLIT, (g2.N, g2.Hout, g2.Wout, g2.Cout), x.device, record=rec, role='x', res=s)
+            y = run_tail(h_pl, img2, g2, t2, bias=b2, nbytes=p2.fwd_ws)
+            n_pl = t2.planes
+        elif p2.res and FUSED_RESIDUAL:
+            y = run(h_pl, img2, g2, b2, nbytes=p2.fwd_ws, res=s)
         else:
-            y = run(h_pl, img2, p2.fwd[0], b2, nbytes=p2.fwd_ws) + s
+            y = run(h_pl, img2, g2, b2, nbytes=p2.fwd_ws) + s
         ctx.save_for_backward(x, h, w1, w2, *x_pl, *h_pl, *s_pl, *((ws,) if ws is not None else ()))
         ctx.sites, ctx.plans, ctx.down = sites, plans, down
+        ctx.backward_tails = bool(backward_tails)
         ctx.images = (bimg1, bimg2, bimgs)
         ctx.has_bias = (b1 is not None, b2 is not None, bs is not None)
-        ctx.mark_non_differentiable(h)
+        ctx.mark_non_differentiable(h, *n_pl)
         ctx.set_materialize_grads(False)
-        return y, h
+        return (y, h) + tuple(n_pl)
 
     @staticmethod
-    def backward(ctx, g, _gh):
+    def backward(ctx, g, _gh, *_gp):
         saved = ctx.saved_tensors
         x, h, w1, w2 = saved[:4]
         x_pl, h_pl = saved[4:7], saved[7:10]
@@ -890,7 +982,7 @@
         need = ctx.needs_input_grad
         need_h = need[0] or need[1] or need[2]
         if g is None:
-            return (None,) * 10
+            return (None,) * 15
         g = g.contiguous()
         dx = dw1 = db1 = dw2 = db2 = dws = dbs = dx1 = None
 
@@ -899,18 +991,14 @@
 
         fused2 = bias_rides(ctx.has_bias[1], need[4], need[3], g.shape[-1])
         g2 = split_planes(g, colsum=fused2, site=conv2, role='g')
-        dh, dw2, db2 = _layer_gradients(g2, fused2, h_pl, w2, p2, bimg2, need_h, need[3])
+        fused1 = need_h and bias_rides(ctx.has_bias[0], need[2], need[1], h.shape[-1])
+        rec = None
+        if need_h and ctx.backward_tails and FUSED_FINISH and FUSED_FINISH_B1 and FUSED_MASKED_SPLIT and p2.bwd_tail:
+            rec = _reader_record(conv1, 'g', g.device)
+        tb1 = _Tail(_lib.TAIL_MASKED, tuple(h.shape), g.device, record=rec, role='g', mask=h, colsum=fused1) if rec is not None else None
+        dh, dw2, db2 = _layer_gradients(g2, fused2, h_pl, w2, p2, bimg2, need_h, need[3], tail=tb1)
         if ctx.has_bias[1] and need[4] and not fused2:
             db2 = g.sum((0, 1, 2))
-        if need_h:
-            fused1 = bias_rides(ctx.has_bias[0], need[2], need[1], h.shape[-1])
-            if FUSED_MASKED_SPLIT:
-                g1 = split_planes_masked(dh, h, site=conv1, role='g', colsum=fused1)
-            else:
-                g1 = split_planes(torch.ops.aten.threshold_backward(dh, h, 0), colsum=fused1, site=conv1, role='g')
-            dx1, dw1, db1 = _layer_gradients(g1, fused1, x_pl, w1, p1, bimg1, need[0], need[1])
-            if ctx.has_bias[0] and need[2] and not fused1:
-                db1 = torch.ops.aten.threshold_backward(dh, h, 0).sum((0, 1, 2))
         other = g
         if ps is not None:
             ws = saved[13]
@@ -919,7 +1007,23 @@
             other, dws, dbs = _layer_gradients(gs, fuseds, saved[10:13], ws, ps, bimgs, need[0], need[5])
             if ctx.has_bias[2] and need[6] and not fuseds:
                 dbs = g.sum((0, 1, 2))
-        if need[0]:
+        if need_h:
+            if tb1 is not None:
+                g1 = tb1.planes
+            elif FUSED_MASKED_SPLIT:
+                g1 = split_planes_masked(dh, h, site=conv1, role='g', colsum=fused1)
+            else:
+                g1 = split_planes(torch.ops.aten.threshold_backward(dh, h, 0), colsum=fused1, site=conv1, role='g')
+            tb2 = None
+            if (need[0] and ctx.backward_tails and FUSED_FINISH and FUSED_FINISH_B2 and FUSED_BLOCK_DX and not ctx.down and p1.bwd_tail
+                    and _dense32(other, x.shape)):
+                tb2 = _Tail(_lib.TAIL_DX, tuple(x.shape), g.device, mask=x, other=other)
+            dx1, dw1, db1 = _layer_gradients(g1, fused1, x_pl, w1, p1, bimg1, need[0], need[1], tail=tb2)
+            if tb2 is not None:
+                dx = tb2.out
+            if ctx.has_bias[0] and need[2] and not fused1:
+                db1 = torch.ops.aten.threshold_backward(dh, h, 0).sum((0, 1, 2))
+        if need[0] and dx is None:
             if FUSED_BLOCK_DX:
                 dx = block_input_gradient(dx1, x, other, ctx.down)
             else:
@@ -928,8 +1032,9 @@
                     other = torch.ops.aten.avg_pool2d_backward(other.permute(0, 3, 1, 2), x.permute(0, 3, 1, 2), [2, 2], [2, 2], [0, 0],
                                                                False, True, None).permute(0, 2, 3, 1)
                 dx = dx + other
-        return dx, dw1, db1, dw2, db2, dws, dbs, None, None, None
-
-
-def critic_block(x, w1, b1, w2, b2, ws, bs, sites, plans, down):
-    return _CriticBlock.apply(x, w1, b1, w2, b2, ws, bs, sites, plans, down)
+        return dx, dw1, db1, dw2, db2, dws, dbs, None, None, None, None, None, None, None, None
+
+
+def critic_block(x, w1, b1, w2, b2, ws, bs, sites, plans, down, next_site=None, x_planes=None, backward_tails=False):
+    out = _CriticBlock.apply(x, w1, b1, w2, b2, ws, bs, sites, plans, down, next_site, *(x_planes if x_planes is not None else (None, None, None)), backward_tails)
+    return out[0], out[1], (tuple(out[2:5]) if len(out) > 2 else None)
diff --git a/wc_gan_amd/csrc/wc_conv.hip b/wc_gan_amd/csrc/wc_conv.hip
--- a/wc_gan_amd/csrc/wc_conv.hip
+++ b/wc_gan_amd/csrc/wc_conv.hip
@@ -1,4 +1,5 @@
 #include "wc_common.h"
+#include "wc_mask.h"
 #include "../../include/wc_hip.h"
 #include <stdlib.h>
 #include <string.h>
@@ -214,33 +215,38 @@
     const float* xscale; const float* wscale; const float* bias; int relu; float* y;
 };
 
+__device__ __forceinline__ f32x4 conv_ksplit_finish_elem(const float* __restrict__ partial, int ksplit, int64_t n4, int cout, const float inv,
+                                                         const float* __restrict__ bias, int relu, const float* __restrict__ res, const int64_t i)
+{
+    f32x4 v = *reinterpret_cast<const f32x4*>(partial + 4 * i);
+    int z = 1;
+    for (; z + 3 < ksplit; z += 4) {
+        f32x4 t[4];
+        #pragma unroll
+        for (int u = 0; u < 4; ++u) t[u] = *reinterpret_cast<const f32x4*>(partial + 4 * ((z + u) * n4 + i));
+        #pragma unroll
+        for (int u = 0; u < 4; ++u) v += t[u];
+    }
+    for (; z < ksplit; ++z) v += *reinterpret_cast<const f32x4*>(partial + 4 * (z * n4 + i));
+    v = v * inv;
+    if (bias) v += *reinterpret_cast<const f32x4*>(bias + (4 * i) % cout);
+    if (relu) { v[0] = fmaxf(v[0], 0.f); v[1] = fmaxf(v[1], 0.f); v[2] = fmaxf(v[2], 0.f); v[3] = fmaxf(v[3], 0.f); }
+    if (res) {
+        const f32x4 r = *reinterpret_cast<const f32x4*>(res + 4 * i);
+        #pragma unroll
+        for (int j = 0; j < 4; ++j) v[j] = __fadd_rn(v[j], r[j]);
+    }
+    return v;
+}
+
 __device__ __forceinline__ void conv_ksplit_reduce_body(const float* __restrict__ partial, int ksplit, int64_t n4, int cout,
                                                         const float* __restrict__ xscale, const float* __restrict__ wscale,
                                                         const float* __restrict__ bias, int relu, float* __restrict__ y,
                                                         const unsigned bid, const unsigned nblocks, const float* __restrict__ res = nullptr)
 {
     const float inv = 1.0f / (xscale[0] * wscale[0]);
-    for (int64_t i = (int64_t)bid * 256 + threadIdx.x; i < n4; i += (int64_t)nblocks * 256) {
-        f32x4 v = *reinterpret_cast<const f32x4*>(partial + 4 * i);
-        int z = 1;
-        for (; z + 3 < ksplit; z += 4) {
-            f32x4 t[4];
-            #pragma unroll
-            for (int u = 0; u < 4; ++u) t[u] = *reinterpret_cast<const f32x4*>(partial + 4 * ((z + u) * n4 + i));
-            #pragma unroll
-            for (int u = 0; u < 4; ++u) v += t[u];
-        }
-        for (; z < ksplit; ++z) v += *reinterpret_cast<const f32x4*>(partial + 4 * (z * n4 + i));
-        v = v * inv;
-        if (bias) v += *reinterpret_cast<const f32x4*>(bias + (4 * i) % cout);
-        if (relu) { v[0] = fmaxf(v[0], 0.f); v[1] = fmaxf(v[1], 0.f); v[2] = fmaxf(v[2], 0.f); v[3] = fmaxf(v[3], 0.f); }
-        if (res) {
-            const f32x4 r = *reinterpret_cast<const f32x4*>(res + 4 * i);
-            #pragma unroll
-            for (int j = 0; j < 4; ++j) v[j] = __fadd_rn(v[j], r[j]);
-        }
-        *reinterpret_cast<f32x4*>(y + 4 * i) = v;
-    }
+    for (int64_t i = (int64_t)bid * 256 + threadIdx.x; i < n4; i += (int64_t)nblocks * 256)
+        *reinterpret_cast<f32x4*>(y + 4 * i) = conv_ksplit_finish_elem(partial, ksplit, n4, cout, inv, bias, relu, res, i);
 }
 
 __global__ __launch_bounds__(256) void conv_ksplit_reduce_kernel(const float* __restrict__ partial, int ksplit, int64_t n4, int cout,
@@ -319,6 +325,18 @@
         for (int j = 0; j < 4; ++j) g[j] = v[j] > 0.f ? g[j] : slope * g[j];
         *reinterpret_cast<f32x4*>(dx + 4 * i) = g;
     }
+}
+
+template <bool DOWN>
+__device__ __forceinline__ f32x4 conv_block_dx_elem(const f32x4 d, const f32x4 a, const f32x4 o)
+{
+    f32x4 r;
+    #pragma unroll
+    for (int k = 0; k < 4; ++k) {
+        const float m = a[k] <= 0.f ? 0.f : d[k];
+        r[k] = __fadd_rn(m, DOWN ? __fadd_rn(0.f, __fmul_rn(0.25f, o[k])) : o[k]);
+    }
+    return r;
 }
 
 template <bool DOWN>
@@ -340,13 +358,7 @@
             j = ((n * (H >> 1) + (yy >> 1)) * (W >> 1) + (xx >> 1)) * c4 + c;
         }
         const f32x4 o = *reinterpret_cast<const f32x4*>(other + 4 * j);
-        f32x4 r;
-        #pragma unroll
-        for (int k = 0; k < 4; ++k) {
-            const float m = a[k] <= 0.f ? 0.f : d[k];
-            r[k] = __fadd_rn(m, DOWN ? __fadd_rn(0.f, __fmul_rn(0.25f, o[k])) : o[k]);
-        }
-        *reinterpret_cast<f32x4*>(out + 4 * i) = r;
+        *reinterpret_cast<f32x4*>(out + 4 * i) = conv_block_dx_elem<DOWN>(d, a, o);
     }
 }
 
@@ -400,14 +412,10 @@
     }
 }
 
-__global__ __launch_bounds__(256) void conv_split_hist_kernel(const float* __restrict__ x, int64_t n4, int relu, _Float16* __restrict__ hi,
-                                                              _Float16* __restrict__ lo, float* __restrict__ scale_out,
-                                                              float* __restrict__ hist, float* __restrict__ colsum, int c4n,
-                                                              float slope = 0.f)
-{
-    __shared__ float red[4];
-    __shared__ f32x4 red4[256];
-    typedef float f32x2h __attribute__((ext_vector_type(2)));
+struct HistPick { int src, tag; float s; };
+
+__device__ __forceinline__ HistPick conv_hist_pick(float* __restrict__ hist, float* __restrict__ scale_out, const unsigned bid)
+{
     typedef int i32x2h __attribute__((ext_vector_type(2)));
     float mx[2] = {0.f, 0.f};
     int tlo[2] = {0x7fffffff, 0x7fffffff}, thi[2] = {0, 0};
@@ -434,36 +442,115 @@
     const float prev = src ? mx[1] : mx[0];
     const float assumed = prev > 0.f ? prev : hist[2 * kHistArray + 2 + src];
     const float s = scale_for(assumed * kHistMargin);
-    if (blockIdx.x == 0 && threadIdx.x == 0) { scale_out[0] = s; hist[2 * kHistArray + 2 + (1 - src)] = assumed; }
+    if (bid == 0 && threadIdx.x == 0) { scale_out[0] = s; hist[2 * kHistArray + 2 + (1 - src)] = assumed; }
+    return HistPick{src, tag, s};
+}
+
+__device__ __forceinline__ float conv_split_elem(f32x4 v, float m, const float s, _Float16* __restrict__ hi, _Float16* __restrict__ lo, const int64_t i)
+{
+    m = fmaxf(fmaxf(m, fabsf(v[0])), fmaxf(fabsf(v[1]), fmaxf(fabsf(v[2]), fabsf(v[3]))));
+    v = v * s;
+    f16x4 h, l;
+    #pragma unroll
+    for (int j = 0; j < 4; ++j) { h[j] = (_Float16)v[j]; l[j] = (_Float16)(v[j] - (float)h[j]); }
+    *reinterpret_cast<f16x4*>(hi + 4 * i) = h;
+    *reinterpret_cast<f16x4*>(lo + 4 * i) = l;
+    return m;
+}
+
+__device__ __forceinline__ void conv_hist_publish(float m, const f32x4 cs, const HistPick pk, float* __restrict__ hist, float* __restrict__ colsum,
+                                                  int c4n, const unsigned bid, float* red, f32x4* red4)
+{
+    typedef float f32x2h __attribute__((ext_vector_type(2)));
+    #pragma unroll
+    for (int o = 32; o > 0; o >>= 1) m = fmaxf(m, __shfl_xor(m, o));
+    if ((threadIdx.x & 63) == 0) red[threadIdx.x >> 6] = m;
+    if (colsum) red4[threadIdx.x] = cs;
+    __syncthreads();
+    if (threadIdx.x == 0) {
+        const f32x2h p = {fmaxf(fmaxf(red[0], red[1]), fmaxf(red[2], red[3])), __builtin_bit_cast(float, pk.tag)};
+        *reinterpret_cast<f32x2h*>(hist + (1 - pk.src) * kHistArray + 2 * bid) = p;
+    }
+    if (colsum && (int)threadIdx.x < c4n) {
+        f32x4 t = red4[threadIdx.x];
+        for (int p = threadIdx.x + c4n; p < 256; p += c4n) t += red4[p];
+        *reinterpret_cast<f32x4*>(colsum + (int64_t)bid * 4 * c4n + 4 * threadIdx.x) = t;
+    }
+}
+
+__global__ __launch_bounds__(256) void conv_split_hist_kernel(const float* __restrict__ x, int64_t n4, int relu, _Float16* __restrict__ hi,
+                                                              _Float16* __restrict__ lo, float* __restrict__ scale_out,
+                                                              float* __restrict__ hist, float* __restrict__ colsum, int c4n,
+                                                              float slope = 0.f)
+{
+    __shared__ float red[4];
+    __shared__ f32x4 red4[256];
+    const HistPick pk = conv_hist_pick(hist, scale_out, blockIdx.x);
     float m = 0.f;
     f32x4 cs = {0.f, 0.f, 0.f, 0.f};
     for (int64_t i = blockIdx.x * 256 + threadIdx.x; i < n4; i += (int64_t)gridDim.x * 256) {
         f32x4 v = *reinterpret_cast<const f32x4*>(x + 4 * i);
         cs += v;
         v = split_act(v, relu, slope);
-        m = fmaxf(fmaxf(m, fabsf(v[0])), fmaxf(fabsf(v[1]), fmaxf(fabsf(v[2]), fabsf(v[3]))));
-        v = v * s;
-        f16x4 h, l;
-        #pragma unroll
-        for (int j = 0; j < 4; ++j) { h[j] = (_Float16)v[j]; l[j] = (_Float16)(v[j] - (float)h[j]); }
-        *reinterpret_cast<f16x4*>(hi + 4 * i) = h;
-        *reinterpret_cast<f16x4*>(lo + 4 * i) = l;
-    }
-    #pragma unroll
-    for (int o = 32; o > 0; o >>= 1) m = fmaxf(m, __shfl_xor(m, o));
-    if ((threadIdx.x & 63) == 0) red[threadIdx.x >> 6] = m;
-    if (colsum) red4[threadIdx.x] = cs;
-    __syncthreads();
-    if (threadIdx.x == 0) {
-        const f32x2h p = {fmaxf(fmaxf(red[0], red[1]), fmaxf(red[2], red[3])), __builtin_bit_cast(float, tag)};
-        *reinterpret_cast<f32x2h*>(hist + (1 - src) * kHistArray + 2 * blockIdx.x) = p;
-    }
-    if (colsum && (int)threadIdx.x < c4n) {
-        f32x4 t = red4[threadIdx.x];
-        for (int p = threadIdx.x + c4n; p < 256; p += c4n) t += red4[p];
-        *reinterpret_cast<f32x4*>(colsum + (int64_t)blockIdx.x * 4 * c4n + 4 * threadIdx.x) = t;
-    }
-}
+        m = conv_split_elem(v, m, pk.s, hi, lo, i);
+    }
+    conv_hist_publish(m, cs, pk, hist, colsum, c4n, blockIdx.x, red, red4);
+}
+
+enum { kTailSplit = 1, kTailMasked = 2, kTailDx = 3 };
+struct FinishTailArgs {
+    KsplitReduceArgs k;
+    const float* res;
+    const float* mask;
+    const float* other;
+    float* out;
+    _Float16* hi; _Float16* lo; float* scale_out; float* hist;
+    float* colsum; int c4n;
+};
+
+template <bool MASKED>
+__device__ __forceinline__ void conv_finish_split_body(const FinishTailArgs& a, const unsigned bid)
+{
+    __shared__ float red[4];
+    __shared__ f32x4 red4[256];
+    const HistPick pk = conv_hist_pick(a.hist, a.scale_out, bid);
+    const float inv = 1.0f / (a.k.xscale[0] * a.k.wscale[0]);
+    float m = 0.f;
+    f32x4 cs = {0.f, 0.f, 0.f, 0.f};
+    for (int64_t i = bid * 256 + threadIdx.x; i < a.k.n4; i += (int64_t)kAmaxBlocks * 256) {
+        f32x4 v = conv_ksplit_finish_elem(a.k.partial, a.k.ksplit, a.k.n4, a.k.cout, inv, a.k.bias, a.k.relu, a.res, i);
+        *reinterpret_cast<f32x4*>(a.k.y + 4 * i) = v;
+        if (MASKED) {
+            v = wc_mask_apply(v, *reinterpret_cast<const f32x4*>(a.mask + 4 * i), 0.f);
+            cs = wc_colsum_add(cs, v);
+        } else {
+            v = split_act(v, 1, 0.f);
+        }
+        m = conv_split_elem(v, m, pk.s, a.hi, a.lo, i);
+    }
+    conv_hist_publish(m, cs, pk, a.hist, MASKED ? a.colsum : nullptr, a.c4n, bid, red, red4);
+}
+
+__device__ __forceinline__ void conv_finish_dx_body(const FinishTailArgs& a, const unsigned bid, const unsigned nblocks)
+{
+    const float inv = 1.0f / (a.k.xscale[0] * a.k.wscale[0]);
+    for (int64_t i = (int64_t)bid * 256 + threadIdx.x; i < a.k.n4; i += (int64_t)nblocks * 256) {
+        const f32x4 d = conv_ksplit_finish_elem(a.k.partial, a.k.ksplit, a.k.n4, a.k.cout, inv, a.k.bias, a.k.relu, nullptr, i);
+        const f32x4 x = *reinterpret_cast<const f32x4*>(a.mask + 4 * i);
+        const f32x4 o = *reinterpret_cast<const f32x4*>(a.other + 4 * i);
+        *reinterpret_cast<f32x4*>(a.out + 4 * i) = conv_block_dx_elem<false>(d, x, o);
+    }
+}
+
+template <int KIND>
+__device__ __forceinline__ void conv_finish_tail_body(const FinishTailArgs& a, const unsigned bid, const unsigned nblocks)
+{
+    if (KIND == kTailDx) conv_finish_dx_body(a, bid, nblocks);
+    else conv_finish_split_body<KIND == kTailMasked>(a, bid);
+}
+
+template <int KIND>
+__global__ __launch_bounds__(256) void conv_finish_tail_kernel(FinishTailArgs a) { conv_finish_tail_body<KIND>(a, blockIdx.x, gridDim.x); }
 
 constexpr int kHistRedoWord = 2 * kHistArray;
 __global__ __launch_bounds__(256) void conv_split_redo_kernel(const float* __restrict__ x, int64_t n4, int relu, _Float16* __restrict__ hi,
@@ -936,6 +1023,13 @@
                                  blockIdx.x - wrw_blocks, gridDim.x - wrw_blocks);
 }
 
+template <int KIND>
+__global__ __launch_bounds__(256) void conv_pair_reduce_tail_kernel(WrwReduceArgs r, FinishTailArgs a, int wrw_blocks)
+{
+    if ((int)blockIdx.x < wrw_blocks) conv_wrw_reduce_body(r, blockIdx.x);
+    else conv_finish_tail_body<KIND>(a, blockIdx.x - wrw_blocks, gridDim.x - wrw_blocks);
+}
+
 struct NarrowWrwArgs {
     const float* x; const float* gy; float* partial;
     int N, H, W, Cin, Cout, ks, nrow;
@@ -1523,6 +1617,74 @@
     hipLaunchKernelGGL(conv_ksplit_reduce_res_kernel, dim3(grid_for(n4)), dim3(256), 0, st, (const float*)ws, a.ksplit, n4, g->Cout,
                        xscale, wscale, bias, res, y);
     return (int)hipGetLastError();
+}
+
+int wc_conv_tail_supported(const wc_conv_geom* g)
+{
+    return wc_conv_res_supported(g);
+}
+
+static int tail_prepare(FinishTailArgs& f, const wc_conv_tail* t, const ConvArgs& a, const wc_conv_geom* g, const float* xscale,
+                        const float* wscale, const float* bias, float* y, const void* ws)
+{
+    if (!t) return WC_ERR_NULL;
+    if (!wc_conv_tail_supported(g)) return WC_ERR_SHAPE;
+    memset(&f, 0, sizeof(f));
+    f.k.n4 = (int64_t)g->N * g->Hout * g->Wout * g->Cout / 4;
+    f.k.partial = (const float*)ws; f.k.ksplit = a.ksplit; f.k.cout = g->Cout;
+    f.k.xscale = xscale; f.k.wscale = wscale; f.k.bias = bias; f.k.relu = 0; f.k.y = y;
+    if (t->kind == WC_CONV_TAIL_DX) {
+        if (!t->mask || !t->other || !t->out) return WC_ERR_NULL;
+        if (t->out == t->mask || t->out == t->other) return WC_ERR_ARG;
+        f.mask = t->mask; f.other = t->other; f.out = t->out;
+        return WC_OK;
+    }
+    if (t->kind != WC_CONV_TAIL_SPLIT && t->kind != WC_CONV_TAIL_MASKED) return WC_ERR_ARG;
+    if (!y || !t->hi || !t->lo || !t->scale || !t->hist) return WC_ERR_NULL;
+    f.hi = (_Float16*)t->hi; f.lo = (_Float16*)t->lo; f.scale_out = t->scale; f.hist = t->hist;
+    if (t->kind == WC_CONV_TAIL_SPLIT) { f.res = t->res; return WC_OK; }
+    if (!t->mask) return WC_ERR_NULL;
+    f.mask = t->mask;
+    if (t->colsum_partials) {
+        if (t->C != g->Cout || (t->C & 3) || 256 % (t->C >> 2) != 0) return WC_ERR_SHAPE;
+        f.colsum = t->colsum_partials; f.c4n = t->C >> 2;
+    }
+    return WC_OK;
+}
+
+static int tail_redo(const wc_conv_tail* t, const FinishTailArgs& f, hipStream_t st)
+{
+    if (t->kind == WC_CONV_TAIL_DX || !t->redo) return WC_OK;
+    const int64_t n4 = f.k.n4;
+    if (t->kind == WC_CONV_TAIL_MASKED)
+        return wc_conv_split_redo_masked_f32(f.k.y, f.mask, 4 * n4, 0.f, t->hi, t->lo, t->scale, t->hist, (wc_stream_t)st);
+    const unsigned g2 = grid_for(n4) < 64u ? grid_for(n4) : 64u;
+    hipLaunchKernelGGL(conv_split_redo_kernel, dim3(g2), dim3(256), 0, st, (const float*)f.k.y, n4, 1, f.hi, f.lo, f.scale_out, f.hist, 0.f);
+    return (int)hipGetLastError();
+}
+
+int wc_conv_tail_f16x3(const void* xhi, const void* xlo, const float* xscale, const void* wimage, const float* wscale,
+                       const float* bias, const void* zero_line, const wc_conv_geom* g, float* y,
+                       void* ws, size_t ws_bytes, const wc_conv_tail* tail, wc_stream_t stream)
+{
+    hipStream_t st = (hipStream_t)stream;
+    if (!tail) return WC_ERR_NULL;
+    ConvArgs a;
+    if (tail->kind == WC_CONV_TAIL_DX && !tail->out) return WC_ERR_NULL;
+    float* y_or_out = tail->kind == WC_CONV_TAIL_DX ? tail->out : y;
+    const int rc = conv_prepare(a, xhi, xlo, xscale, wimage, wscale, bias, zero_line, g, 0, y_or_out, ws, ws_bytes);
+    if (rc != WC_OK) return rc;
+    FinishTailArgs f;
+    const int rt = tail_prepare(f, tail, a, g, xscale, wscale, bias, y, ws);
+    if (rt != WC_OK) return rt;
+    const hipError_t e = (g->Cout % 256) == 0 ? launch_conv<2, 4, true>(a, st) : launch_conv<2, 2, true>(a, st);
+    if (e != hipSuccess) return (int)e;
+    if (tail->kind == WC_CONV_TAIL_SPLIT) hipLaunchKernelGGL((conv_finish_tail_kernel<kTailSplit>), dim3(kAmaxBlocks), dim3(256), 0, st, f);
+    else if (tail->kind == WC_CONV_TAIL_MASKED) hipLaunchKernelGGL((conv_finish_tail_kernel<kTailMasked>), dim3(kAmaxBlocks), dim3(256), 0, st, f);
+    else hipLaunchKernelGGL((conv_finish_tail_kernel<kTailDx>), dim3(grid_for(f.k.n4)), dim3(256), 0, st, f);
+    const hipError_t e2 = hipGetLastError();
+    if (e2 != hipSuccess) return (int)e2;
+    return tail_redo(tail, f, st);
 }
 
 int wc_conv_block_dx_f32(const float* dx1, const float* x, const float* other, int64_t N, int64_t H, int64_t W, int C, int down,
@@ -1778,16 +1940,23 @@
     return wc_conv_workspace_bytes(gd) + wc_conv_wrw_workspace_bytes(gf);
 }
 
-int wc_conv_bwd_pair_f16x3(const void* ghi, const void* glo, const float* gscale, const void* wimage, const float* wscale,
-                           const void* zero_line, const wc_conv_geom* gd, float* dx, void* ws_dx, size_t ws_dx_bytes,
-                           const void* xhi, const void* xlo, const float* xscale, const wc_conv_geom* gf, float* dw,
-                           int64_t stride_k, int64_t stride_n, int64_t stride_r, int64_t stride_s,
-                           const float* colsum_partials, float* db, void* ws_dw, size_t ws_dw_bytes, wc_stream_t stream)
-{
-    hipStream_t st = (hipStream_t)stream;
+static int bwd_pair(const void* ghi, const void* glo, const float* gscale, const void* wimage, const float* wscale,
+                    const void* zero_line, const wc_conv_geom* gd, float* dx, void* ws_dx, size_t ws_dx_bytes,
+                    const void* xhi, const void* xlo, const float* xscale, const wc_conv_geom* gf, float* dw,
+                    int64_t stride_k, int64_t stride_n, int64_t stride_r, int64_t stride_s,
+                    const float* colsum_partials, float* db, void* ws_dw, size_t ws_dw_bytes, const wc_conv_tail* tail, hipStream_t st)
+{
     ConvArgs d;
-    int rc = conv_prepare(d, ghi, glo, gscale, wimage, wscale, nullptr, zero_line, gd, 0, dx, ws_dx, ws_dx_bytes);
+    if (tail && tail->kind == WC_CONV_TAIL_DX && !tail->out) return WC_ERR_NULL;
+    float* dx_or_out = (tail && tail->kind == WC_CONV_TAIL_DX) ? tail->out : dx;
+    int rc = conv_prepare(d, ghi, glo, gscale, wimage, wscale, nullptr, zero_line, gd, 0, dx_or_out, ws_dx, ws_dx_bytes);
     if (rc != WC_OK) return rc;
+    FinishTailArgs f;
+    if (tail) {
+        if (tail->kind != WC_CONV_TAIL_MASKED && tail->kind != WC_CONV_TAIL_DX) return WC_ERR_ARG;
+        rc = tail_prepare(f, tail, d, gd, gscale, wscale, nullptr, dx, ws_dx);
+        if (rc != WC_OK) return rc;
+    }
     WrwPlan p;
     rc = wrw_prepare(p, xhi, xlo, xscale, ghi, glo, gscale, zero_line, gf, dw, stride_k, stride_n, stride_r, stride_s,
                      colsum_partials, db, ws_dw, ws_dw_bytes);
@@ -1814,6 +1983,15 @@
     e = hipGetLastError();
     if (e != hipSuccess) return (int)e;
     const int reduce_blocks = p.r.main_blocks + p.extra;
+    if (tail) {
+        if (tail->kind == WC_CONV_TAIL_MASKED)
+            hipLaunchKernelGGL((conv_pair_reduce_tail_kernel<kTailMasked>), dim3(reduce_blocks + kAmaxBlocks), dim3(256), 0, st, p.r, f, reduce_blocks);
+        else
+            hipLaunchKernelGGL((conv_pair_reduce_tail_kernel<kTailDx>), dim3(reduce_blocks + grid_for(f.k.n4)), dim3(256), 0, st, p.r, f, reduce_blocks);
+        e = hipGetLastError();
+        if (e != hipSuccess) return (int)e;
+        return tail_redo(tail, f, st);
+    }
     if (d.ksplit > 1) {
         KsplitReduceArgs k;
         k.n4 = (int64_t)gd->N * gd->Hout * gd->Wout * gd->Cout / 4;
@@ -1826,4 +2004,26 @@
     return (int)hipGetLastError();
 }
 
-}
+int wc_conv_bwd_pair_f16x3(const void* ghi, const void* glo, const float* gscale, const void* wimage, const float* wscale,
+                           const void* zero_line, const wc_conv_geom* gd, float* dx, void* ws_dx, size_t ws_dx_bytes,
+                           const void* xhi, const void* xlo, const float* xscale, const wc_conv_geom* gf, float* dw,
+                           int64_t stride_k, int64_t stride_n, int64_t stride_r, int64_t stride_s,
+                           const float* colsum_partials, float* db, void* ws_dw, size_t ws_dw_bytes, wc_stream_t stream)
+{
+    return bwd_pair(ghi, glo, gscale, wimage, wscale, zero_line, gd, dx, ws_dx, ws_dx_bytes, xhi, xlo, xscale, gf, dw,
+                    stride_k, stride_n, stride_r, stride_s, colsum_partials, db, ws_dw, ws_dw_bytes, nullptr, (hipStream_t)stream);
+}
+
+int wc_conv_bwd_pair_tail_f16x3(const void* ghi, const void* glo, const float* gscale, const void* wimage, const float* wscale,
+                                const void* zero_line, const wc_conv_geom* gd, float* dx, void* ws_dx, size_t ws_dx_bytes,
+                                const void* xhi, const void* xlo, const float* xscale, const wc_conv_geom* gf, float* dw,
+                                int64_t stride_k, int64_t stride_n, int64_t stride_r, int64_t stride_s,
+                                const float* colsum_partials, float* db, void* ws_dw, size_t ws_dw_bytes,
+                                const wc_conv_tail* tail, wc_stream_t stream)
+{
+    if (!tail) return WC_ERR_NULL;
+    return bwd_pair(ghi, glo, gscale, wimage, wscale, zero_line, gd, dx, ws_dx, ws_dx_bytes, xhi, xlo, xscale, gf, dw,
+                    stride_k, stride_n, stride_r, stride_s, colsum_partials, db, ws_dw, ws_dw_bytes, tail, (hipStream_t)stream);
+}
+
+}
diff --git a/wc_gan_amd/csrc/wc_gp.hip b/wc_gan_amd/csrc/wc_gp.hip
--- a/wc_gan_amd/csrc/wc_gp.hip
+++ b/wc_gan_amd/csrc/wc_gp.hip
@@ -1,4 +1,5 @@
 #include "wc_common.h"
+#include "wc_mask.h"
 #include "../../include/wc_hip.h"
 
 namespace {
@@ -10,11 +11,9 @@
 
 __device__ __forceinline__ f32x4 masked_load(const float* __restrict__ t, const float* __restrict__ a, int64_t i, float slope)
 {
-    f32x4 v = *reinterpret_cast<const f32x4*>(t + 4 * i);
+    const f32x4 v = *reinterpret_cast<const f32x4*>(t + 4 * i);
     const f32x4 p = *reinterpret_cast<const f32x4*>(a + 4 * i);
-    #pragma unroll
-    for (int j = 0; j < 4; ++j) v[j] = v[j] * (p[j] > 0.f ? 1.0f : slope);
-    return v;
+    return wc_mask_apply(v, p, slope);
 }
 
 __device__ __forceinline__ float absmax4(float m, f32x4 v)
@@ -49,9 +48,7 @@
 
 __device__ __forceinline__ f32x4 colsum_add(f32x4 cs, f32x4 v)
 {
-    #pragma unroll
-    for (int j = 0; j < 4; ++j) cs[j] = __fadd_rn(cs[j], v[j]);
-    return cs;
+    return wc_colsum_add(cs, v);
 }
 
 __device__ __forceinline__ void colsum_fold(f32x4* red4, float* __restrict__ colsum, int c4n)
@@ -289,6 +286,16 @@
     return (int)hipGetLastError();
 }
 
+int wc_conv_split_redo_masked_f32(const float* t, const float* a, int64_t n, float slope, void* hi, void* lo, float* scale, float* hist,
+                                  wc_stream_t stream)
+{
+    if (!t || !a || !hi || !lo || !scale || !hist || n <= 0 || (n & 3)) return WC_ERR_ARG;
+    if (!(slope >= 0.f && slope <= 1.f)) return WC_ERR_ARG;
+    const unsigned g2 = grid_for(n / 4) < 64 ? grid_for(n / 4) : 64u;
+    hipLaunchKernelGGL(gp_split_redo_kernel, dim3(g2), dim3(256), 0, (hipStream_t)stream, t, a, n / 4, slope, (_Float16*)hi, (_Float16*)lo, scale, hist);
+    return (int)hipGetLastError();
+}
+
 int wc_gp_interp_f32(const float* real, const float* fake, const float* eps, int64_t N, int64_t L, float* x_hat, wc_stream_t stream)
 {
     if (!real || !fake || !eps || !x_hat) return WC_ERR_NULL;
diff --git a/wc_gan_amd/csrc/wc_mask.h b/wc_gan_amd/csrc/wc_mask.h
--- /dev/null
+++ b/wc_gan_amd/csrc/wc_mask.h
@@ -0,0 +1,16 @@
+#pragma once
+#include "wc_common.h"
+
+__device__ __forceinline__ f32x4 wc_mask_apply(f32x4 v, const f32x4 p, float slope)
+{
+    #pragma unroll
+    for (int j = 0; j < 4; ++j) v[j] = v[j] * (p[j] > 0.f ? 1.0f : slope);
+    return v;
+}
+
+__device__ __forceinline__ f32x4 wc_colsum_add(f32x4 cs, f32x4 v)
+{
+    #pragma unroll
+    for (int j = 0; j < 4; ++j) cs[j] = __fadd_rn(cs[j], v[j]);
+    return cs;
+}
diff --git a/wc_gan_amd/discriminator.py b/wc_gan_amd/discriminator.py
--- a/wc_gan_amd/discriminator.py
+++ b/wc_gan_amd/discriminator.py
@@ -36,26 +36,45 @@
         return all(isinstance(c, Conv2D) and c.kind == 'same' and c.conv.weight.dtype == torch.float32 for c in convs)
 
     def _fused_plans(self, x):
-        from . import conv as fc, generator as _g
+        from . import generator as _g
         if not self._fusable():
             return None
         if not (torch.is_tensor(x) and x.is_cuda and x.dtype == torch.float32 and x.dim() == 4 and x.is_contiguous()
                 and getattr(x, '_wc_planes', None) is None and _g.split_of(x) is None):
             return None
-        return fc.critic_block_plans(tuple(x.shape), tuple(self.conv1.conv.weight.shape), tuple(self.conv2.conv.weight.shape),
+        return self._plans_of(tuple(x.shape))
+
+    def _plans_of(self, xshape):
+        from . import conv as fc
+        return fc.critic_block_plans(xshape, tuple(self.conv1.conv.weight.shape), tuple(self.conv2.conv.weight.shape),
                                      tuple(self.shortcut.conv.weight.shape) if self.has_shortcut else None, self.resample == 'DOWN')
 
-    def forward(self, x, cls):
+    def takes_input_planes(self, xshape):
+        return self._fusable() and self._plans_of(tuple(xshape)) is not None
+
+    def forward(self, x, cls, x_planes=None, handover=None):
+        if handover is not None:
+            handover['planes'] = None
         plans = self._fused_plans(x)
         if plans is not None:
             from . import conv as fc
             w1, w2 = self.conv1._weight(), self.conv2._weight()
             ws = self.shortcut._weight() if self.has_shortcut else None
             x = self.bn1(x, cls)
-            y, h = fc.critic_block(x, w1, self.conv1.conv.bias, w2, self.conv2.conv.bias, ws, self.shortcut.conv.bias if self.has_shortcut else None,
-                                   (self.conv1, self.conv2, self.shortcut if self.has_shortcut else None), plans, self.resample == 'DOWN')
+            nxt = handover.get('next') if handover is not None else None
+            g2 = plans[1].fwd[0]
+            next_site = None
+            if isinstance(nxt, ResBlockDown) and nxt.takes_input_planes((g2.N, g2.Hout, g2.Wout, g2.Cout)):
+                next_site = nxt.conv1
+            y, h, planes = fc.critic_block(x, w1, self.conv1.conv.bias, w2, self.conv2.conv.bias, ws, self.shortcut.conv.bias if self.has_shortcut else None,
+                                           (self.conv1, self.conv2, self.shortcut if self.has_shortcut else None), plans, self.resample == 'DOWN',
+                                           next_site=next_site, x_planes=x_planes, backward_tails=handover is not None)
+            if handover is not None:
+                handover['planes'] = planes
             self.bn2(h, cls)
             return y
+        if x_planes is not None:
+            raise RuntimeError("ResBlockDown: planes handed to a block that does not run as the fused node")
         h = self.conv1(x) if self.is_first else self.conv1.forward_relu(self.bn1(x, cls))
         h = self.bn2(h, cls)
         s = x
@@ -146,9 +165,14 @@
         if batch:
             fc.prepare_images(self, fc.pass_key(self, x))
         try:
-            y = x
-            for blk in self.blocks:
-                y = blk(y, cls)
+            y, planes = x, None
+            for i, blk in enumerate(self.blocks):
+                if isinstance(blk, ResBlockDown):
+                    box = {'next': self.blocks[i + 1] if i + 1 < len(self.blocks) else None}
+                    y = blk(y, cls, x_planes=planes, handover=box)
+                    planes = box['planes']
+                else:
+                    y = blk(y, cls)
         finally:
             if batch:
                 fc.finish_images(self)
```

Measured after the change: 3848 images/sec, median of 6. 1.1% higher.
